# ina-foss/inaSpeechSegmenter

Measured on AMD Instinct MI355X. Metric: hours-of-audio segmented/sec (smn+gender, 16 kHz mono), higher is better.
Workload: dtype f32 (f16x3 split-operand MFMA, f32 accumulate; f64 FFT)

## Files before the change

inaspeechsegmenter_amd/_native.py:

```python
import ctypes as C
import os

import numpy as np

_HERE = os.path.dirname(os.path.abspath(__file__))
LIB_PATH = os.environ.get('ISS_LIB') or os.path.join(_HERE, 'libiss_hip.so')

PROG_COLS = 32
OP_CONV, OP_POOL, OP_SOFTMAX, OP_STATPOOL, OP_ACT, OP_ELT = 1, 2, 3, 4, 5, 6
(ELT_COPY, ELT_ADD, ELT_SUB, ELT_MUL, ELT_MAX, ELT_MIN, ELT_AVG, ELT_ZERO, ELT_PERMUTE) = range(9)
(C_OP, C_IN, C_OUT, C_RES, C_H, C_W, C_CIN, C_HO, C_WO, C_COUT, C_KH, C_KW, C_SH, C_SW, C_PT, C_PL,
 C_ACT, C_WOFF, C_BOFF, C_PSOFF, C_PTOFF, C_INMODE, C_POOLKIND, C_ORDER, C_FPOOLH, C_FPOOLW, C_DUALW, C_DUALB, C_ACTPARAM, C_ACTPARAM2, C_ACTPARAM3) = range(31)
PREC_BF16X3, PREC_F32, PREC_F16X3 = 0, 1, 2
K_ALIGN = 32
BUF_INPUT = -2
MAX_NETS = 8
RS_JOB = np.dtype([('src_offset', '<i8'), ('frames_in', '<i8'), ('channels', '<i4'), ('format', '<i4'), ('filter', '<i4'),
                   ('reserved', '<i4'), ('dst_offset', '<i8'), ('frames_out', '<i8')])
RS_FORMAT = {np.dtype(np.uint8): 0, np.dtype('<i2'): 1, np.dtype('<i4'): 2, np.dtype('<f4'): 3, np.dtype('<f8'): 4}
RS_I8, RS_ULAW, RS_ALAW, RS_SWAP = 8, 9, 10, 0x100
ADPCM_JOB = np.dtype([('src_offset', '<i8'), ('block_begin', '<i8'), ('nblocks', '<i8'), ('frames_total', '<i8'), ('channels', '<i4'),
                      ('block_align', '<i4'), ('output', '<i4'), ('filter', '<i4'), ('dst_offset', '<i8'), ('frames_out', '<i8')])
ADPCM_TO_SIGNAL, ADPCM_TO_STAGE = 0, 1
ADPCM_STATUS = {1: 'step index above 88', 2: 'predictor index above 6'}
# ... 66 lines not shown
    global _lib
    if _lib is not None:
        return _lib
    if not os.path.exists(LIB_PATH):
        raise NativeError(
            f"{LIB_PATH} is missing: the HIP extension has not been built. "
            "Run `python -c 'import __graft_entry__ as g; g.build()'` (needs hipcc). "
            "There is no CPU fallback for the feature/CNN path.")
    try:
        import torch
    except ImportError:
        pass
    L = C.CDLL(LIB_PATH)
    vp, i32, i64, u64 = C.c_void_p, C.c_int32, C.c_int64, C.c_uint64
    pf, pd, pi32, pi64, pu8, pi16 = (C.POINTER(C.c_float), C.POINTER(C.c_double), C.POINTER(C.c_int32),
                                     C.POINTER(C.c_int64), C.POINTER(C.c_uint8), C.POINTER(C.c_int16))
    sig = {
        'iss_create': (C.c_int, [C.c_int, C.POINTER(vp)]),
        'iss_destroy': (None, [vp]),
        'iss_last_error': (C.c_char_p, [vp]),
        'iss_version': (C.c_char_p, []),
        'iss_set_workspace_limit': (C.c_int, [vp, u64]),
        'iss_synchronize': (C.c_int, [vp]),
        'iss_sidekit_tables': (C.c_int, [vp, pd, pf]),
        'iss_signal_pcm16': (C.c_int, [vp, pi16, i64]),
        'iss_signal_f32': (C.c_int, [vp, pf, i64]),
        'iss_signal_pcm16_device': (C.c_int, [vp, vp, i64]),
        'iss_signal_pcm16_device_stream': (C.c_int, [vp, vp, i64, vp]),
        'iss_resample_filter': (C.c_int, [vp, i32, i32, pd, i64, pi32]),
        'iss_resample_pcm16': (C.c_int, [vp, vp, i64, vp, i32, i64]),
        'iss_resample_pcm16_windows': (C.c_int, [vp, vp, i64, vp, vp, i32, i64]),
        'iss_flac_decode_windows': (C.c_int, [vp, vp, i64, vp, i64, vp, vp, i32, i64, pi32]),
        'iss_adpcm_decode_windows': (C.c_int, [vp, vp, i64, vp, vp, i32, i64, i64, pi32]),
        'iss_msadpcm_decode_windows': (C.c_int, [vp, vp, i64, vp, vp, i32, i64, i64, pi32]),
        'iss_resample_pcm16_split': (C.c_int, [vp, vp, i64, vp, i32, i64, vp, vp, i64]),
        'iss_flac_decode_split': (C.c_int, [vp, vp, i64, vp, i64, vp, i32, i64, pi32, vp, vp, i64]),
        'iss_adpcm_decode_split': (C.c_int, [vp, vp, i64, vp, i32, i64, i64, pi32, vp, vp, i64]),
        'iss_msadpcm_decode_split': (C.c_int, [vp, vp, i64, vp, i32, i64, i64, pi32, vp, vp, i64]),
        'iss_resample_pcm16_windows_split': (C.c_int, [vp, vp, i64, vp, vp, i32, i64, vp, vp, i64]),
        'iss_flac_decode_windows_split': (C.c_int, [vp, vp, i64, vp, i64, vp, vp, i32, i64, pi32, vp, vp, i64]),
        'iss_adpcm_decode_windows_split': (C.c_int, [vp, vp, i64, vp, vp, i32, i64, i64, pi32, vp, vp, i64]),
        'iss_msadpcm_decode_windows_split': (C.c_int, [vp, vp, i64, vp, vp, i32, i64, i64, pi32, vp, vp, i64]),
        'iss_resample_split_geometry': (C.c_int, [vp, i32, i32, pi32, pi32]),
        'iss_resample_pcm16_mix': (C.c_int, [vp, vp, i64, vp, vp, i32, i64, vp, vp, i64, vp, i64]),
        'iss_flac_decode_mix': (C.c_int, [vp, vp, i64, vp, i64, vp, vp, i32, i64, pi32, vp, vp, i64, vp, i64]),
        'iss_adpcm_decode_mix': (C.c_int, [vp, vp, i64, vp, vp, i32, i64, i64, pi32, vp, vp, i64, vp, i64]),
        'iss_msadpcm_decode_mix': (C.c_int, [vp, vp, i64, vp, vp, i32, i64, i64, pi32, vp, vp, i64, vp, i64]),
        'iss_get_signal_pcm16': (C.c_int, [vp, pi16, i64, i64]),
        'iss_resample_stats': (C.c_int, [vp, pi64, pi64]),
        'iss_flac_index': (C.c_int, [vp, i64, i64, vp, vp, i64, pi64, pi64, C.c_char_p, i32]),
        'iss_flac_crc': (C.c_int, [vp, i64, pi32, pi32]),
        'iss_flac_decode_host': (C.c_int, [vp, i64, vp, i64, i32, i32, i64, vp, pi32]),
        'iss_flac_decode': (C.c_int, [vp, vp, i64, vp, i64, vp, i32, i64, pi32]),
        'iss_flac_get_stage': (C.c_int, [vp, i32, vp, i64]),
        'iss_flac_stats': (C.c_int, [vp, pi64, pi64]),
        'iss_adpcm_decode_host': (C.c_int, [vp, i64, i64, i32, i32, i64, pi16, pi32]),
        'iss_adpcm_decode': (C.c_int, [vp, vp, i64, vp, i32, i64, i64, pi32]),
        'iss_adpcm_get_stage': (C.c_int, [vp, i32, vp, i64]),
        'iss_adpcm_stats': (C.c_int, [vp, pi64, pi64]),
        'iss_msadpcm_decode_host': (C.c_int, [vp, i64, i64, i32, i32, i64, pi16, pi32]),
        'iss_msadpcm_decode': (C.c_int, [vp, vp, i64, vp, i32, i64, i64, pi32]),
        'iss_msadpcm_get_stage': (C.c_int, [vp, i32, vp, i64]),
        'iss_msadpcm_stats': (C.c_int, [vp, pi64, pi64]),
        'iss_host_alloc': (C.c_int, [vp, C.c_size_t, C.POINTER(vp)]),
        'iss_host_free': (C.c_int, [vp, vp]),
        'iss_cnn_probs_async': (C.c_int, [vp, C.c_int, pi32, i32, pf, pu8, pi64]),
        'iss_cnn_dead_stats': (C.c_int, [vp, pi64, pi64]),
        'iss_wait': (C.c_int, [vp, i64]),
        'iss_comm_unique_id': (C.c_int, [vp, pu8]),
        'iss_comm_init': (C.c_int, [vp, pu8, i32, i32]),
        'iss_comm_destroy': (C.c_int, [vp]),
        'iss_allgather_segments': (C.c_int, [vp, pi32, i32, i32, pi32, pi32]),
        'iss_comm_allreduce_max': (C.c_int, [vp, pd]),
        'iss_comm_info': (C.c_int, [vp, pi32, pi32, pi32, C.c_char_p, i32]),
        'iss_sidekit': (C.c_int, [vp, pi32]),
        'iss_get_loge': (C.c_int, [vp, pf]),
        'iss_get_mspec': (C.c_int, [vp, pf]),
        'iss_set_mspec': (C.c_int, [vp, pf, i32]),
        'iss_cnn_load': (C.c_int, [vp, C.c_int, pi32, i32, pf, i64, i32, pi64, i32, i32, i32, i32]),
        'iss_cnn_load_shared': (C.c_int, [vp, C.c_int, C.c_int, pi32, i32, i32, pi64, i32, i32, i32, i32]),
        'iss_cnn_probs': (C.c_int, [vp, C.c_int, pi32, i32, pf, pu8]),
        'iss_cnn_forward': (C.c_int, [vp, C.c_int, pf, i32, pf]),
        'iss_cnn_flops': (C.c_int, [vp, C.c_int, pd]),
        'iss_set_precision': (C.c_int, [vp, C.c_int]),
        'iss_set_precision_guard': (C.c_int, [vp, C.c_float]),
        'iss_cnn_precision_info': (C.c_int, [vp, C.c_int, pi32, pf, pi32, pi32, pf]),
        'iss_cnn_set_net_precision': (C.c_int, [vp, C.c_int, C.c_int]),
        'iss_vbx_tables': (C.c_int, [vp, pd, pd]),
        'iss_vbx_features': (C.c_int, [vp, pi32, pd, i64, pf, pi32]),
        'iss_vbx_set_dither': (C.c_int, [vp, pd, i64]),
        'iss_vbx_features_pcm16': (C.c_int, [vp, pi16, i64, pf, pi32]),
        'iss_vbx_features_batch_pcm16': (C.c_int, [vp, pi16, pi64, i32, pi32, pf]),
        'iss_vbx_features_resident': (C.c_int, [vp, pi64, pi64, i32, pi32, pf]),
        'iss_vbx_resident_stats': (C.c_int, [vp, pi64, pi64]),
        'iss_vbx_embed': (C.c_int, [vp, C.c_int, pi32, i32, pf]),
        'iss_prof_enable': (C.c_int, [vp, C.c_int]),
        'iss_prof_get': (C.c_int, [vp, C.c_int, pd, pi64, pd]),
        'iss_prof_reset': (C.c_int, [vp]),
        'iss_prof_get_row': (C.c_int, [vp, C.c_int, pd, pi64]),
        'iss_prof_get_instance': (C.c_int, [vp, C.c_int, C.c_char_p, i32, pd, pi64, pd]),
        'iss_set_diag': (C.c_int, [vp, C.c_uint32]),
        'iss_scribble': (C.c_int, [vp, C.c_uint32]),
        'iss_viterbi_f64': (C.c_int, [pd, i64, i32, pd, pi32]),
        'iss_viterbi_f32': (C.c_int, [pf, i64, i32, pd, pi32]),
        'iss_energy_viterbi': (C.c_int, [pf, i64, C.c_double, C.c_double, C.c_double, pd, pi32]),
        'iss_viterbi_segments_f32': (C.c_int, [pf, pi64, i64, i32, pd, pi32]),
    }
    for name, (res, args) in sig.items():
        fn = getattr(L, name)
        fn.restype = res
        fn.argtypes = args
    L._iss_symbols = tuple(sig)
    _lib = L
    return L


DIAG_BITS = {'no_shared_first': 0x001, 'no_flrows': 0x002, 'no_ws': 0x004, 'no_ws3': 0x008, 'no_direct1': 0x010,
             'no_nh2': 0x020, 'no_tr': 0x040, 'no_pw': 0x080, 'no_pws': 0x100, 'no_pws2': 0x200, 'no_wq': 0x400,
             'no_dual': 0x800, 'no_chain': 0x1000, 'no_ring': 0x2000, 'no_fsame': 0x4000, 'no_f32ws': 0x8000, 'no_ncb1': 0x10000, 'no_wsu3': 0x20000, 'no_gfused': 0x40000, 'no_hl': 0x80000,
             'no_skip_dead': 0x100000}


def diag_flags(names):
    flags = 0
    for nm in str(names).replace(' ', '').replace('+', ',').lower().split(','):
        if nm:
            flags |= DIAG_BITS[nm]
    return flags


def _ptr(a, ty):
    return a.ctypes.data_as(C.POINTER(ty))


def viterbi(emission, transition):
    L = lib()
    em = np.ascontiguousarray(emission)
    if em.dtype not in (np.float32, np.float64):
        em = em.astype(np.float64)
    tr = np.ascontiguousarray(transition, dtype=np.float64)
    T, K = em.shape
    out = np.empty(T, dtype=np.int32)
    if em.dtype == np.float32:
        rc = L.iss_viterbi_f32(_ptr(em, C.c_float), T, K, _ptr(tr, C.c_double), _ptr(out, C.c_int32))
    else:
        rc = L.iss_viterbi_f64(_ptr(em, C.c_double), T, K, _ptr(tr, C.c_double), _ptr(out, C.c_int32))
    if rc != 0:
        raise NativeError(f"iss_viterbi failed ({rc}): T={T} K={K}")
    return out


def viterbi_segments(emission, seg_len, transition):
    L = lib()
    em = np.ascontiguousarray(emission, dtype=np.float32)
    sl = np.ascontiguousarray(seg_len, dtype=np.int64)
    tr = np.ascontiguousarray(transition, dtype=np.float64)
    n, K = em.shape
    assert int(sl.sum()) == n
    out = np.empty(n, dtype=np.int32)
    rc = L.iss_viterbi_segments_f32(_ptr(em, C.c_float), _ptr(sl, C.c_int64), sl.size, K, _ptr(tr, C.c_double), _ptr(out, C.c_int32))
    if rc != 0:
        raise NativeError(f"iss_viterbi_segments_f32 failed ({rc}): n={n} K={K} segments={sl.size}")
    return out


_LOG_EPS = np.log(np.full(1, 1e-10))[0], np.log(np.full(1, 1 - 1e-10))[0]


def energy_viterbi(loge, threshold, transition):
    L = lib()
    x = np.ascontiguousarray(loge, dtype=np.float32)
    tr = np.ascontiguousarray(transition, dtype=np.float64)
    out = np.empty(x.size, dtype=np.int32)
    rc = L.iss_energy_viterbi(_ptr(x, C.c_float), x.size, float(threshold), float(_LOG_EPS[0]), float(_LOG_EPS[1]),
                              _ptr(tr, C.c_double), _ptr(out, C.c_int32))
    if rc != 0:
        raise NativeError(f"iss_energy_viterbi failed ({rc}): T={x.size}")
    return out


def flac_crc(buf):
    b = np.frombuffer(bytes(buf), dtype=np.uint8)
    c8, c16 = C.c_int32(), C.c_int32()
    if lib().iss_flac_crc(C.c_void_p(b.ctypes.data), b.size, C.byref(c8), C.byref(c16)) != 0:
        raise NativeError('iss_flac_crc failed')
    return c8.value, c16.value


def flac_index(buf, first_frame, info):
    L = lib()
    inf = np.ascontiguousarray(np.array(info, dtype=FLAC_INFO).reshape(1))
    cap = max(16, int(inf['total_samples'][0]) // max(1, int(inf['min_block'][0]) or 1) + 2) if inf['total_samples'][0] > 0 \
        else buf.size // 64 + 16
    err = C.create_string_buffer(256)
    n, off = C.c_int64(), C.c_int64()
    for _ in range(2):
        rows = np.zeros(cap, dtype=FLAC_FRAME)
        rc = L.iss_flac_index(C.c_void_p(buf.ctypes.data), buf.size, int(first_frame), C.c_void_p(inf.ctypes.data),
                              C.c_void_p(rows.ctypes.data), cap, C.byref(n), C.byref(off), err, 256)
        if rc != -5:
            break
        cap = buf.size // 9 + 16
    if rc != 0:
        raise ValueError(off.value, err.value.decode())
    return rows[:n.value].copy()


def flac_decode_host(buf, frames, channels, bps, frames_total):
    fr = np.ascontiguousarray(frames, dtype=FLAC_FRAME)
    out = np.empty((int(frames_total), int(channels)), dtype=np.int32 if bps > 16 else np.int16)
    st = np.zeros(len(fr), dtype=np.int32)
    rc = lib().iss_flac_decode_host(C.c_void_p(buf.ctypes.data), buf.size, C.c_void_p(fr.ctypes.data), len(fr), int(channels),
                                    int(bps), int(frames_total), C.c_void_p(out.ctypes.data), _ptr(st, C.c_int32))
    if rc != 0:
        raise NativeError(f'iss_flac_decode_host failed ({rc}): bad frame rows')
    return (out[:, 0] if channels == 1 else out), st


def adpcm_decode_host(buf, nblocks, channels, block_align, frames_total, fn='iss_adpcm_decode_host'):
    buf = np.ascontiguousarray(buf, dtype=np.uint8)
    out = np.empty((int(frames_total), int(channels)), dtype=np.int16)
    st = np.zeros(int(nblocks), dtype=np.int32)
    rc = getattr(lib(), fn)(C.c_void_p(buf.ctypes.data), buf.size, int(nblocks), int(channels), int(block_align),
                            int(frames_total), _ptr(out, C.c_int16), _ptr(st, C.c_int32))
    if rc != 0:
        raise NativeError(f'{fn} failed ({rc}): bad block geometry')
    return (out[:, 0] if channels == 1 else out), st


def msadpcm_decode_host(buf, nblocks, channels, block_align, frames_total):
    return adpcm_decode_host(buf, nblocks, channels, block_align, frames_total, 'iss_msadpcm_decode_host')


class Context:

    def __init__(self, device=0):
        self._L = lib()
        h = C.c_void_p()
        rc = self._L.iss_create(int(device), C.byref(h))
        if rc != 0:
            raise NativeError(f"iss_create(device={device}) failed ({rc}): "
                              f"{self._L.iss_last_error(None).decode()}")
        self._h = h
        self.device = device
        self.T = 0
        self._net_out = {}
        self._dither_n = 0
        self._pinned = {}
        self.comm_rank, self.comm_world = 0, 1
        self.precision = None
        self.workspace_limit = None
        self.diag = 0
        env = os.environ.get('ISS_DIAG', '')
        if env:
            self.set_diag(diag_flags(env))
        self.guard_threshold = None
        env = os.environ.get('ISS_PREC_GUARD', '')
        if env:
            self.set_precision_guard(float(env))

    def close(self):
        if getattr(self, '_h', None):
            for p in list(self._pinned.values()):
                self._L.iss_host_free(self._h, C.c_void_p(p))
            self._pinned.clear()
            self._L.iss_destroy(self._h)
            self._h = None

    def __del__(self):
        try:
            self.close()
        except Exception:
            pass

    def _ck(self, rc, what):
        if rc != 0:
            raise NativeError(f"{what} failed ({rc}): {self._L.iss_last_error(self._h).decode()}")

    def sidekit_tables(self, window, melbank):
        w = np.ascontiguousarray(window, dtype=np.float64)
        b = np.ascontiguousarray(melbank, dtype=np.float32)
        assert w.shape == (400,) and b.shape == (24, 257)
        self._ck(self._L.iss_sidekit_tables(self._h, _ptr(w, C.c_double), _ptr(b, C.c_float)), 'iss_sidekit_tables')

    def set_signal(self, sig):
        sig = np.ascontiguousarray(sig)
        if sig.dtype == np.int16:
            self._ck(self._L.iss_signal_pcm16(self._h, _ptr(sig, C.c_int16), sig.size), 'iss_signal_pcm16')
        elif sig.dtype == np.float32:
            self._ck(self._L.iss_signal_f32(self._h, _ptr(sig, C.c_float), sig.size), 'iss_signal_f32')
        else:
            raise TypeError(f"signal dtype {sig.dtype}: need int16 or float32")
        self._keep = sig

    def set_signal_device(self, dev_ptr, n, producer_stream=None):
        self._ck(self._L.iss_signal_pcm16_device_stream(self._h, C.c_void_p(int(dev_ptr)), int(n),
                                                        C.c_void_p(int(producer_stream)) if producer_stream else None),
                 'iss_signal_pcm16_device')

    def resample_filter(self, sr):
        from . import resample
        up, down, h = resample.plan(sr)
        fid = C.c_int32()
        self._ck(self._L.iss_resample_filter(self._h, up, down, _ptr(h, C.c_double), h.size, C.byref(fid)), 'iss_resample_filter')
        return fid.value, up, down

    def resample_job(self, x, sr, src_offset, dst_offset, fmt=None):
        fid, up, down = self.resample_filter(sr)
        n = x.shape[0]
        return (src_offset, n, 1 if x.ndim == 1 else x.shape[1], RS_FORMAT[x.dtype] if fmt is None else int(fmt), fid, 0,
                dst_offset, -(-n * up // down))

    def resample(self, src, jobs, n_signal=-1, windows=None, splits=None, mixes=None):
        src = np.ascontiguousarray(src, dtype=np.uint8)
        jb = np.ascontiguousarray(np.array(jobs, dtype=RS_JOB))
        self._decode_call('iss_resample_pcm16', (C.c_void_p(src.ctypes.data), src.size, C.c_void_p(jb.ctypes.data)),
                          (jb.size, int(n_signal)), windows, splits, mixes)
        self._keep_rs = src

    def _decode_call(self, base, lead, trail, windows, splits, mixes=None):
        name, args = base, lead + trail
        if mixes is not None:
            if splits is not None:
                raise ValueError('a call carries splits or mixes, not both')
            wn = None if windows is None else _window_rows(windows, trail[0])
            sets, rows, terms = _mix_rows(mixes, trail[0])
            args = lead + (None if wn is None else C.c_void_p(wn.ctypes.data),) + trail + (
                C.c_void_p(sets.ctypes.data), C.c_void_p(rows.ctypes.data), rows.size, C.c_void_p(terms.ctypes.data), terms.size)
            self._ck(getattr(self._L, base + '_mix')(self._h, *args), base + '_mix')
            return
        if windows is not None:
            wn = _window_rows(windows, trail[0])
            name, args = base + '_windows', lead + (C.c_void_p(wn.ctypes.data),) + trail
        if splits is not None:
            sp, sel = _split_rows(splits, trail[0])
            name, args = name + '_split', args + (C.c_void_p(sp.ctypes.data), C.c_void_p(sel.ctypes.data), sel.size)
        self._ck(getattr(self._L, name)(self._h, *args), name)

# ... 166 lines not shown
        self._ck(self._L.iss_wait(self._h, int(ticket)), 'iss_wait')

    def comm_unique_id(self):
        buf = np.zeros(128, dtype=np.uint8)
        self._ck(self._L.iss_comm_unique_id(self._h, _ptr(buf, C.c_uint8)), 'iss_comm_unique_id')
        return buf.tobytes()

    def comm_init(self, uid, rank, world):
        buf = np.frombuffer(bytes(uid), dtype=np.uint8).copy()
        assert buf.size == 128
        self._ck(self._L.iss_comm_init(self._h, _ptr(buf, C.c_uint8), int(rank), int(world)), 'iss_comm_init')
        self.comm_rank, self.comm_world = int(rank), int(world)

    def comm_destroy(self):
        self._ck(self._L.iss_comm_destroy(self._h), 'iss_comm_destroy')
        self.comm_rank, self.comm_world = 0, 1

    def allgather_segments(self, rows, capacity):
        world = self.comm_world
        out = np.zeros((world, capacity, 4), dtype=np.int32)
        counts = np.zeros(world, dtype=np.int32)
        if rows is None:
            rows, n = np.zeros((1, 4), np.int32), -1
        else:
            rows = np.ascontiguousarray(rows, dtype=np.int32).reshape(-1, 4)
            n = rows.shape[0]
        self._ck(self._L.iss_allgather_segments(self._h, _ptr(rows, C.c_int32), n, int(capacity),
                                                _ptr(out, C.c_int32), _ptr(counts, C.c_int32)), 'iss_allgather_segments')
        return out, counts

    def comm_info(self):
        w, r, v = C.c_int32(), C.c_int32(), C.c_int32()
        buf = C.create_string_buffer(512)
        self._ck(self._L.iss_comm_info(self._h, C.byref(w), C.byref(r), C.byref(v), buf, 512), 'iss_comm_info')
        return {'world': w.value, 'rank': r.value, 'version': v.value, 'lib': buf.value.decode(errors='replace')}

    def comm_allreduce_max(self, value):
        v = C.c_double(float(value))
        self._ck(self._L.iss_comm_allreduce_max(self._h, C.byref(v)), 'iss_comm_allreduce_max')
        return v.value

    def cnn_forward(self, net_id, x):
        x = np.ascontiguousarray(x, dtype=np.float32)
        n = x.shape[0]
        out = np.empty((n, self._net_out[net_id]), dtype=np.float32)
        self._ck(self._L.iss_cnn_forward(self._h, net_id, _ptr(x, C.c_float), n, _ptr(out, C.c_float)), 'iss_cnn_forward')
        return out

    def cnn_flops(self, net_id):
        f = C.c_double()
        self._ck(self._L.iss_cnn_flops(self._h, net_id, C.byref(f)), 'iss_cnn_flops')
        return f.value

    def set_precision(self, mode):
        self._ck(self._L.iss_set_precision(self._h, int(mode)), 'iss_set_precision')
        self.precision = int(mode)

    def set_precision_guard(self, threshold):
        self._ck(self._L.iss_set_precision_guard(self._h, float(threshold)), 'iss_set_precision_guard')
        self.guard_threshold = float(threshold)

    def cnn_precision_info(self, net_id):
        mode, slots, state, d, du = C.c_int32(0), C.c_int32(0), C.c_int32(0), C.c_float(0), C.c_float(0)
        self._ck(self._L.iss_cnn_precision_info(self._h, int(net_id), C.byref(mode), C.byref(d), C.byref(slots), C.byref(state), C.byref(du)),
                 'iss_cnn_precision_info')
        return {'mode': {PREC_F32: 'f32', PREC_F16X3: 'f16x3'}.get(mode.value, 'bf16x3'), 'max_dlogp': None if d.value < 0 else float(d.value),
                'max_dlogp_in_use': None if du.value < 0 else float(du.value),
                'slots': slots.value, 'state': ('pending', 'passed', 'escalated', 'fixed')[state.value]}

    def cnn_set_net_precision(self, net_id, mode):
        self._ck(self._L.iss_cnn_set_net_precision(self._h, int(net_id), int(mode)), 'iss_cnn_set_net_precision')

    def set_workspace_limit(self, nbytes):
        self._ck(self._L.iss_set_workspace_limit(self._h, int(nbytes)), 'iss_set_workspace_limit')
        self.workspace_limit = int(nbytes)

    def mirror_settings(self, other):
        if getattr(other, 'precision', None) is not None and other.precision != getattr(self, 'precision', None):
            self.set_precision(other.precision)
        if getattr(other, 'workspace_limit', None) is not None and other.workspace_limit != getattr(self, 'workspace_limit', None):
            self.set_workspace_limit(other.workspace_limit)
        if getattr(other, 'diag', 0) != getattr(self, 'diag', 0):
            self.set_diag(other.diag)
        if getattr(other, 'guard_threshold', None) is not None and other.guard_threshold != getattr(self, 'guard_threshold', None):
            self.set_precision_guard(other.guard_threshold)

    def set_diag(self, flags):
        flags = diag_flags(flags) if isinstance(flags, str) else int(flags)
        self._ck(self._L.iss_set_diag(self._h, flags), 'iss_set_diag')
        self.diag = flags

    def scribble(self, word):
        self._ck(self._L.iss_scribble(self._h, int(word) & 0xFFFFFFFF), 'iss_scribble')

    def synchronize(self):
        self._ck(self._L.iss_synchronize(self._h), 'iss_synchronize')

    def vbx_tables(self, window, melbank):
        w = np.ascontiguousarray(window, dtype=np.float64)
        b = np.ascontiguousarray(melbank, dtype=np.float64)
        assert w.shape == (400,) and b.shape == (257, 64)
        self._ck(self._L.iss_vbx_tables(self._h, _ptr(w, C.c_double), _ptr(b, C.c_double)), 'iss_vbx_tables')

    def vbx_features(self, sig_i32, dither_u):
        s = np.ascontiguousarray(sig_i32, dtype=np.int32)
        u = np.ascontiguousarray(dither_u, dtype=np.float64)
        assert s.shape == u.shape and s.ndim == 1
        T = (s.size + 320 - 400) // 160 + 1
        out = np.empty((T, 64), dtype=np.float32)
        t = C.c_int32()
        self._ck(self._L.iss_vbx_features(self._h, _ptr(s, C.c_int32), _ptr(u, C.c_double), s.size,
                                          _ptr(out, C.c_float), C.byref(t)), 'iss_vbx_features')
        self._dither_n = 0
        assert t.value == T
        return out

    def vbx_set_dither(self, dither_u):
        u = np.ascontiguousarray(dither_u, dtype=np.float64)
        self._ck(self._L.iss_vbx_set_dither(self._h, _ptr(u, C.c_double), u.size), 'iss_vbx_set_dither')
        self._dither_n = u.size

    def vbx_features_pcm16(self, pcm, to_host=True):
        s = np.ascontiguousarray(pcm, dtype=np.int16)
        T = (s.size + 320 - 400) // 160 + 1
        t = C.c_int32()
        if not to_host:
            self._ck(self._L.iss_vbx_features_pcm16(self._h, _ptr(s, C.c_int16), s.size, None, C.byref(t)), 'iss_vbx_features_pcm16')
            assert t.value == T
            return T
        out = np.empty((T, 64), dtype=np.float32)
        self._ck(self._L.iss_vbx_features_pcm16(self._h, _ptr(s, C.c_int16), s.size, _ptr(out, C.c_float), C.byref(t)),
                 'iss_vbx_features_pcm16')
        assert t.value == T
        return out

    def vbx_features_batch_pcm16(self, pcms, to_host=True):
        pcms = [np.asarray(p, dtype=np.int16) for p in pcms]
        soff = np.zeros(len(pcms) + 1, dtype=np.int64)
        soff[1:] = np.cumsum([p.size for p in pcms])
        s = np.ascontiguousarray(np.concatenate(pcms) if pcms else np.zeros(0, np.int16))
        foff = np.zeros(len(pcms) + 1, dtype=np.int32)
        T = int(sum((p.size + 320 - 400) // 160 + 1 for p in pcms))
        out = np.empty((T, 64), dtype=np.float32) if to_host else None
        self._ck(self._L.iss_vbx_features_batch_pcm16(self._h, _ptr(s, C.c_int16), _ptr(soff, C.c_int64), len(pcms),
                                                      _ptr(foff, C.c_int32), _ptr(out, C.c_float) if to_host else None),
                 'iss_vbx_features_batch_pcm16')
        return foff, out

    def vbx_features_resident(self, begins, counts, to_host=False):
        b = np.ascontiguousarray(begins, dtype=np.int64).reshape(-1)
        n = np.ascontiguousarray(counts, dtype=np.int64).reshape(-1)
        if b.size != n.size:
            raise ValueError(f'vbx_features_resident: {b.size} begins, {n.size} counts')
        foff = np.zeros(b.size + 1, dtype=np.int32)
        T = int(sum((int(k) + 320 - 400) // 160 + 1 for k in n if k >= 200))
        out = np.empty((T, 64), dtype=np.float32) if to_host else None
        self._ck(self._L.iss_vbx_features_resident(self._h, _ptr(b, C.c_int64), _ptr(n, C.c_int64), b.size, _ptr(foff, C.c_int32),
                                                   _ptr(out, C.c_float) if to_host else None), 'iss_vbx_features_resident')
        return foff, (out[:foff[-1]] if to_host else None)

    def vbx_resident_stats(self):
        return self._counters('iss_vbx_resident_stats')

    def vbx_embed(self, net_id, starts):
        st = np.ascontiguousarray(starts, dtype=np.int32)
        out = np.empty((st.size, self._net_out[net_id]), dtype=np.float32)
        self._ck(self._L.iss_vbx_embed(self._h, net_id, _ptr(st, C.c_int32), st.size, _ptr(out, C.c_float)), 'iss_vbx_embed')
        return out

    def prof_enable(self, on=True):
        self._ck(self._L.iss_prof_enable(self._h, 1 if on else 0), 'iss_prof_enable')

    def prof_reset(self):
# ... 24 lines not shown
```

inaspeechsegmenter_amd/csrc/cnn.hip:

```cpp
#include "conv_select.h"

using namespace issk;

namespace {

template <int MODE>
__global__ __launch_bounds__(256) void conv_igemm_kernel(const ConvArgs p) {
    __shared__ __attribute__((aligned(16))) float sA[2][BM * LDK];
    __shared__ __attribute__((aligned(16))) float sB[2][BN * LDK];

    const int tid = threadIdx.x, lane = tid & 63, wv = tid >> 6;
    unsigned mt, nt;
    gemm_tile_of_block(blockIdx.x, p.nblk, p.nblk_n, mt, nt);
    const long long m0 = (long long)mt * BM;
    const int n0 = (int)nt * BN;

    const int k4 = tid & 3;
    const int lr = tid >> 2;
    RowSrc rs[2];
#pragma unroll
    for (int j = 0; j < 2; ++j) rs[j] = row_source<MODE>(p, m0 + lr + 64 * j);
    const int bn = n0 + lr;
    const bool bok = bn < p.Cout;
    const float* wrow = p.w + (size_t)(bok ? bn : 0) * p.Kpad + k4 * 4;
// ... 743 lines not shown

__global__ void pool_kernel(const float* __restrict__ in, float* __restrict__ out, long long total, int H, int W,
                            int C, int Ho, int Wo, int kh, int kw, int sh, int sw, int pt, int pl, int kind) {
    const long long idx = (long long)blockIdx.x * blockDim.x + threadIdx.x;
    if (idx >= total) return;
    const int c = (int)(idx % C);
    long long t = idx / C;
    const int ox = (int)(t % Wo); t /= Wo;
    const int oy = (int)(t % Ho);
    const long long b = t / Ho;
    float acc = kind == 0 ? -INFINITY : 0.f;
    int cnt = 0;
    for (int ky = 0; ky < kh; ++ky) {
        const int iy = oy * sh - pt + ky;
        if ((unsigned)iy >= (unsigned)H) continue;
        for (int kx = 0; kx < kw; ++kx) {
            const int ix = ox * sw - pl + kx;
            if ((unsigned)ix >= (unsigned)W) continue;
            const float v = in[((b * H + iy) * W + ix) * C + c];
            acc = kind == 0 ? fmaxf(acc, v) : acc + v;
            ++cnt;
        }
    }
    out[idx] = kind == 0 ? acc : acc / (float)(cnt > 0 ? cnt : 1);
}


__global__ __launch_bounds__(256) void act_kernel(const float* in, float* out, long long total, int act, float alpha, float p2, float p3) {
    auto f = [&](float v) {
        if (act == 9) return v > p3 ? fminf(v, p2) : alpha * (v - p3);
        if (act == 8) return fminf(fmaxf(v, 0.f), alpha);
        if (act == 4) return v > 0.f ? v : alpha * (expf(v) - 1.f);
        if (act == 5) return v > 0.f ? v : alpha * v;
        if (act == 6) return 1.05070098f * (v > 0.f ? v : 1.67326324f * (expf(v) - 1.f));
        return v > 20.f ? v : log1pf(expf(v));
    };
    const long long n4 = total >> 2;
    for (long long i = blockIdx.x * 256ll + threadIdx.x; i < n4; i += (long long)gridDim.x * 256) {
        float4 v = reinterpret_cast<const float4*>(in)[i];
        v.x = f(v.x); v.y = f(v.y); v.z = f(v.z); v.w = f(v.w);
        reinterpret_cast<float4*>(out)[i] = v;
    }
    for (long long i = (n4 << 2) + blockIdx.x * 256ll + threadIdx.x; i < total; i += (long long)gridDim.x * 256) out[i] = f(in[i]);
}

__global__ __launch_bounds__(256) void elt_kernel(const float* in, const float* res, float* out, long long total, int kind,
                                                  int cin, int cout, int nch, int soff, int doff, int d0, int d1, int d2,
                                                  int s0, int s1, int s2, int relu) {
    auto bin = [&](float a, float b) {
        const float v = kind == ISS_ELT_ADD ? a + b : kind == ISS_ELT_SUB ? a - b : kind == ISS_ELT_MUL ? a * b :
                        kind == ISS_ELT_MAX ? fmaxf(a, b) : kind == ISS_ELT_MIN ? fminf(a, b) : (a + b) * 0.5f;
        return relu ? fmaxf(v, 0.f) : v;
    };
    if (kind >= ISS_ELT_ADD && kind <= ISS_ELT_AVG && (total & 3) == 0) {
        const long long n4 = total >> 2;
        for (long long i = blockIdx.x * 256ll + threadIdx.x; i < n4; i += (long long)gridDim.x * 256) {
            const float4 a = reinterpret_cast<const float4*>(in)[i], b = reinterpret_cast<const float4*>(res)[i];
            reinterpret_cast<float4*>(out)[i] = make_float4(bin(a.x, b.x), bin(a.y, b.y), bin(a.z, b.z), bin(a.w, b.w));
        }
        return;
    }
    for (long long i = blockIdx.x * 256ll + threadIdx.x; i < total; i += (long long)gridDim.x * 256) {
        if (kind >= ISS_ELT_ADD && kind <= ISS_ELT_AVG) {
            out[i] = bin(in[i], res[i]);
        } else if (kind == ISS_ELT_COPY || kind == ISS_ELT_ZERO) {
            const long long p = i / nch;
            const int ch = (int)(i - p * nch);
            out[p * cout + doff + ch] = kind == ISS_ELT_ZERO ? 0.f : in[p * cin + soff + ch];
        } else {
            const long long per = (long long)d0 * d1 * d2;
            const long long smp = i / per;
            long long r = i - smp * per;
            const int i2 = (int)(r % d2); r /= d2;
            const int i1 = (int)(r % d1);
            const int i0 = (int)(r / d1);
            out[i] = in[smp * per + (long long)i0 * s0 + (long long)i1 * s1 + (long long)i2 * s2];
        }
    }
}

__global__ void softmax_kernel(const float* __restrict__ in, float* __restrict__ out, long long rows, int C) {
    const long long r = (long long)blockIdx.x * blockDim.x + threadIdx.x;
    if (r >= rows) return;
    const float* x = in + r * C;
    float mx = x[0];
    for (int i = 1; i < C; ++i) mx = fmaxf(mx, x[i]);
    float s = 0.f;
    for (int i = 0; i < C; ++i) s += expf(x[i] - mx);
    for (int i = 0; i < C; ++i) out[r * C + i] = expf(x[i] - mx) / s;
}

__global__ void statpool_kernel(const float* __restrict__ in, float* __restrict__ out, long long total, int H, int W, int C) {
    const long long idx = (long long)blockIdx.x * blockDim.x + threadIdx.x;
    if (idx >= total) return;
    const int c = (int)(idx % C);
    long long t = idx / C;
    const int h = (int)(t % H);
    const long long b = t / H;
    const float* src = in + ((b * H + h) * (long long)W) * C + c;
    float s = 0.f, q = 0.f;
    for (int w = 0; w < W; ++w) { const float v = src[(long long)w * C]; s += v; q += v * v; }
    const float mean = s / W, meansq = q / W;
    float* o = out + b * (2LL * C * H);
    o[c * H + h] = mean;
    o[(long long)C * H + c * H + h] = sqrtf(meansq - mean * mean + 1e-10f);
}

__global__ void fill_half_kernel(float* p, long long n) {
    const long long i = (long long)blockIdx.x * blockDim.x + threadIdx.x;
    if (i < n) p[i] = 0.5f;
}

__global__ void mask_probs_kernel(float* probs, const uint8_t* finite, long long n, int C) {
    const long long i = (long long)blockIdx.x * blockDim.x + threadIdx.x;
    if (i < n * C && !finite[i / C]) probs[i] = 0.5f;
}

__global__ __launch_bounds__(256) void row_flags_kernel(const float* __restrict__ mspec, int T, uint8_t* __restrict__ flag) {
    const int t = blockIdx.x * 256 + threadIdx.x;
    if (t >= T) return;
    float v[24];
#pragma unroll
    for (int k = 0; k < 6; ++k) *reinterpret_cast<float4*>(v + 4 * k) = reinterpret_cast<const float4*>(mspec + (size_t)t * 24)[k];
    flag[t] = (uint8_t)iss_row_flag(v);
}

__global__ void scatter_probs_kernel(const float* __restrict__ res, const uint8_t* __restrict__ lfinite, const int32_t* __restrict__ map,
                                     long long n, int C, float* __restrict__ out, uint8_t* __restrict__ finite) {
    const long long i = (long long)blockIdx.x * blockDim.x + threadIdx.x;
    if (i >= n * C) return;
    const long long r = i / C;
    const int k = (int)(i - r * C);
    const long long m = map[r];
    const uint8_t f = lfinite[r];
    out[m * C + k] = f ? res[i] : 0.5f;
    if (k == 0) finite[m] = f;
}

inline int roundup(int a, int b) { return (a + b - 1) / b * b; }

inline uint16_t bf16_rne(float x) {
    uint32_t u;
    memcpy(&u, &x, 4);
    u += 0x7fffu + ((u >> 16) & 1u);
    return (uint16_t)(u >> 16);
}
inline float bf16_to_f32(uint16_t h) {
    uint32_t u = (uint32_t)h << 16;
    float x;
    memcpy(&x, &u, 4);
    return x;
}

}

IssParamArrays::~IssParamArrays() {
    for (void* p : {(void*)blob, (void*)wh, (void*)wl, (void*)wh16, (void*)wl16}) if (p) (void)hipFree(p);
}

int iss_cnn_free(iss_ctx* c, int id) {
    if (!c || id < 0 || id >= ISS_MAX_NETS) return ISS_EINVAL;
    IssNet& n = c->nets[id];
    if (n.shared_params) {
        n.shared_params.reset();
    } else {
        if (n.d_blob) (void)hipFree(n.d_blob);
        if (n.d_wh) (void)hipFree(n.d_wh);
        if (n.d_wl) (void)hipFree(n.d_wl);
        if (n.d_wh16) (void)hipFree(n.d_wh16);
        if (n.d_wl16) (void)hipFree(n.d_wl16);
    }
    for (auto& kv : n.dhl_wp) if (kv.second) (void)hipFree(kv.second);
// ... 212 lines not shown
    ISS_HIP(c, hipSetDevice(c->device));
    iss_cnn_free(c, id);
    IssNet& s = c->nets[src];
    IssNet& n = c->nets[id];
    std::vector<int32_t> ktab;
    int rc = cnn_set_program(c, n, "iss_cnn_load_shared", prog, nrows, s.blob_floats, nbuf, buf_elems, in_h, in_w, in_c, out_dim, ktab);
    if (rc) return rc;
    if (!s.shared_params) {
        s.shared_params = std::make_shared<IssParamArrays>();
        IssParamArrays& a = *s.shared_params;
        a.blob = s.d_blob; a.wh = s.d_wh; a.wl = s.d_wl; a.wh16 = s.d_wh16; a.wl16 = s.d_wl16;
    }
    n.shared_params = s.shared_params;
    n.d_blob = s.d_blob; n.d_wh = s.d_wh; n.d_wl = s.d_wl; n.d_wh16 = s.d_wh16; n.d_wl16 = s.d_wl16;
    n.f16_ok = s.f16_ok;
    if ((rc = cnn_upload_tables(c, n, nullptr, ktab))) return rc;
    n.loaded = true;
    return ISS_OK;
}

extern "C" int iss_set_precision(iss_ctx* c, int mode) {
    if (!c) return ISS_EINVAL;
    if (mode != ISS_PREC_BF16X3 && mode != ISS_PREC_F32 && mode != ISS_PREC_F16X3) return iss_fail(c, ISS_EINVAL, "iss_set_precision: unknown mode %d", mode);
    if (mode == c->precision) return ISS_OK;
    c->precision = mode;
    for (IssNet& n : c->nets) {
        if (!n.loaded || n.prec_by_caller) continue;
        n.prec_override = -1;
        n.guard_state = ISS_GUARD_PENDING;
        n.guard_dlogp = n.guard_dlogp_chosen = -1.f;
        n.guard_slots = 0;
    }
    return ISS_OK;
}

extern "C" int iss_set_precision_guard(iss_ctx* c, float threshold) {
    if (!c) return ISS_EINVAL;
    if (!(threshold == threshold)) return iss_fail(c, ISS_EINVAL, "iss_set_precision_guard: threshold is NaN");
    c->guard_threshold = threshold;
    return ISS_OK;
}

extern "C" int iss_cnn_set_net_precision(iss_ctx* c, int id, int mode) {
    if (!c || id < 0 || id >= ISS_MAX_NETS) return ISS_EINVAL;
    if (mode != -1 && mode != ISS_PREC_BF16X3 && mode != ISS_PREC_F32 && mode != ISS_PREC_F16X3) return iss_fail(c, ISS_EINVAL, "iss_cnn_set_net_precision: unknown mode %d", mode);
    if (!c->nets[id].loaded) return iss_fail(c, ISS_ESTATE, "net %d not loaded", id);
    c->nets[id].prec_override = mode;
    c->nets[id].prec_by_caller = mode != -1;
    c->nets[id].guard_state = mode == -1 ? ISS_GUARD_PENDING : ISS_GUARD_FIXED;
    return ISS_OK;
}

static bool net_reads_patches(const IssNet& n) {
    for (int r = 0; r < n.nrows; ++r)
        if (n.prog[(size_t)r * ISS_PROG_COLS + ISS_C_OP] == ISS_OP_CONV && n.prog[(size_t)r * ISS_PROG_COLS + ISS_C_INMODE] == 1) return true;
    return false;
}

static int effective_precision(const iss_ctx* c, const IssNet& n) {
    const int prec = n.prec_override >= 0 ? n.prec_override : c->precision;
    if (prec == ISS_PREC_F16X3 && !(n.f16_ok && n.d_wh16 != nullptr && net_reads_patches(n))) return ISS_PREC_BF16X3;
    return prec;
}

extern "C" int iss_cnn_precision_info(iss_ctx* c, int id, int32_t* mode, float* max_dlogp, int32_t* slots, int32_t* state, float* dlogp_in_use) {
    if (!c || id < 0 || id >= ISS_MAX_NETS) return ISS_EINVAL;
    const IssNet& n = c->nets[id];
    if (!n.loaded) return iss_fail(c, ISS_ESTATE, "net %d not loaded", id);
    if (mode) *mode = effective_precision(c, n);
    if (max_dlogp) *max_dlogp = n.guard_dlogp;
    if (slots) *slots = n.guard_slots;
    if (state) *state = n.guard_state;
    if (dlogp_in_use) *dlogp_in_use = n.guard_dlogp_chosen;
    return ISS_OK;
}

extern "C" int iss_set_diag(iss_ctx* c, uint32_t flags) {
    if (!c) return ISS_EINVAL;
    if (flags & ~(uint32_t)ISS_DIAG_ALL) return iss_fail(c, ISS_EINVAL, "iss_set_diag: unknown bits 0x%x", flags & ~(uint32_t)ISS_DIAG_ALL);
    c->diag = flags;
    return ISS_OK;
}

extern "C" int iss_cnn_flops(iss_ctx* c, int id, double* f) {
    if (!c || id < 0 || id >= ISS_MAX_NETS || !f) return ISS_EINVAL;
    if (!c->nets[id].loaded) return iss_fail(c, ISS_ESTATE, "net %d not loaded", id);
    *f = c->nets[id].flops_per_sample;
    return ISS_OK;
}

namespace {

struct PassIo { const int32_t* d_winrow; const float* d_stats; const uint8_t* d_fin; const float* d_input; };

int conv_args(iss_ctx* c, IssNet& n, const PassIo& io, int bc, const ConvChoice& ch, ConvArgs& a) {
    const int r = ch.row;
    const int32_t* R = &n.prog[(size_t)r * ISS_PROG_COLS];
    memset(&a, 0, sizeof(a));
    fill_geometry(a, R, bc);
    a.in = R[ISS_C_IN] == ISS_BUF_INPUT ? io.d_input : (const float*)c->act[R[ISS_C_IN]].p;
    a.w = n.d_blob + R[ISS_C_WOFF];
    a.bias = R[ISS_C_BOFF] >= 0 ? n.d_blob + R[ISS_C_BOFF] : nullptr;
    a.ps = R[ISS_C_PSOFF] >= 0 ? n.d_blob + R[ISS_C_PSOFF] : nullptr;
    a.pt = R[ISS_C_PTOFF] >= 0 ? n.d_blob + R[ISS_C_PTOFF] : nullptr;
    a.res = R[ISS_C_RES] >= 0 ? (const float*)c->act[R[ISS_C_RES]].p : nullptr;
    a.out = (float*)c->act[R[ISS_C_OUT]].p;
    a.ktab = n.d_ktab + n.ktab_off[r];
    a.wh = n.d_wh + R[ISS_C_WOFF]; a.wl = n.d_wl + R[ISS_C_WOFF];
    a.Kpad = n.kpad[r]; a.mode = ch.inst.mode; a.tmr = ch.tmr;
    if (ch.inst.kernel == ConvKernel::Dhl) return ISS_OK;
    if (R[ISS_C_INMODE] == 1) {
        if (!io.d_winrow) return iss_fail(c, ISS_ESTATE, "patch-mode network run without a window list");
        a.in = (const float*)c->mspec.p; a.win_row = io.d_winrow; a.stats = io.d_stats; a.finite = io.d_fin;
    } else if (R[ISS_C_INMODE] == 2) {
        if (!io.d_winrow || !c->vbx_out.p) return iss_fail(c, ISS_ESTATE, "window-mode network run without resident vbx features");
        a.in = (const float*)c->vbx_out.p; a.win_row = io.d_winrow;
    } else if (!a.in) return iss_fail(c, ISS_ESTATE, "network input missing");
    a.nblk = (unsigned)((a.M + BM - 1) / BM);
    set_fast_div(a, 0, a.pp); set_fast_div(a, 1, a.pw); set_fast_div(a, 2, a.Hq * a.Wq); set_fast_div(a, 3, a.Wq);
#ifdef ISS_EXPERIMENTS
    { static const int dbg = getenv("ISS_DBG") ? atoi(getenv("ISS_DBG")) : 0; a.dbg = dbg; }
#endif
    a.nblk_n = (unsigned)((a.Cout + BN - 1) / BN);
    if (ch.inst.kernel == ConvKernel::Pwc) {
        const int32_t* Q = &n.prog[(size_t)ch.partner * ISS_PROG_COLS];
        a.wh2 = n.d_wh + Q[ISS_C_WOFF]; a.wl2 = n.d_wl + Q[ISS_C_WOFF];
        a.bias2 = Q[ISS_C_BOFF] >= 0 ? n.d_blob + Q[ISS_C_BOFF] : nullptr;
        a.out2 = (float*)c->act[Q[ISS_C_OUT]].p;
        a.act2 = Q[ISS_C_ACT]; a.Cout2 = Q[ISS_C_COUT];
    } else if (ch.inst.kernel == ConvKernel::Pws2Dual) {
        const int32_t* P = &n.prog[(size_t)ch.partner * ISS_PROG_COLS];
        a.in2 = P[ISS_C_IN] == ISS_BUF_INPUT ? io.d_input : (const float*)c->act[P[ISS_C_IN]].p;
        a.Cin2 = P[ISS_C_CIN]; a.H2 = P[ISS_C_H]; a.W2 = P[ISS_C_W]; a.sh2 = P[ISS_C_SH]; a.sw2 = P[ISS_C_SW];
        const int64_t wo = (int64_t)R[ISS_C_DUALW] - 1;
        a.w = n.d_blob + wo; a.wh = n.d_wh + wo; a.wl = n.d_wl + wo;
        a.bias = n.d_blob + (R[ISS_C_DUALB] - 1); a.res = nullptr;
        a.Kpad = a.Cin + a.Cin2;
    }
    if (ch.inst.f16) { a.f16 = 1; a.wh = n.d_wh16 + R[ISS_C_WOFF]; a.wl = n.d_wl16 + R[ISS_C_WOFF]; }
    if (ch.inst.kernel == ConvKernel::Wq3h) { a.in_hl = 1; a.in_np = ch.in_np; }
    if (ch.out != OutLayout::F32) { a.out_hl = 1; a.out_np = ch.out_np; a.out_f16 = ch.generic_out && ch.out_f16 ? 1 : 0; }
    return ISS_OK;
}

int launch_shared_first_layer(iss_ctx* c, IssNet& n, const PassIo& io, int pend, int bc, int rmin, int rmax, ConvArgs& a, double* fl) {
    const int32_t* R1 = &n.prog[(size_t)pend * ISS_PROG_COLS];
    const bool fs1 = R1[ISS_C_HO] == R1[ISS_C_H];
    int ph1, pw1;
    fused_pool_of(R1, ph1, pw1);
    const bool pool1 = ph1 * pw1 != 1;
    const long long rrows = (long long)(rmax - rmin) + R1[ISS_C_HO];
    const long long rtot = rrows * R1[ISS_C_WO] * (R1[ISS_C_COUT] / 4);
    const int f_ne = fs1 ? R1[ISS_C_KH] - 1 : 0;
    const long long etot = (long long)bc * f_ne * R1[ISS_C_WO] * (R1[ISS_C_COUT] / 4);
    const int plane_rows = pool1 ? (int)(rrows / ph1) + 2 : 0;
    const long long ptot = pool1 ? (long long)ph1 * plane_rows * (R1[ISS_C_WO] / pw1) * (R1[ISS_C_COUT] / 4) : 0;
    { const int rc = iss_reserve(c, c->raw1, (size_t)(rtot + etot + ptot) * 16 + (pool1 ? (size_t)bc * 4 + 16 : 0)); if (rc) return rc; }
    float* Rraw = (float*)c->raw1.p;
    const float* mspec = (const float*)c->mspec.p;
    const float* w1 = n.d_blob + R1[ISS_C_WOFF];
    const size_t lds1 = (size_t)R1[ISS_C_KH] * R1[ISS_C_KW] * R1[ISS_C_COUT] * 4;
    iss_prof_begin(c, 2, 0);
    if (fs1) {
        const int pt1 = R1[ISS_C_PT], pl1 = R1[ISS_C_PL], pb1 = R1[ISS_C_KH] - 1 - pt1;
        const float* S = n.d_wsum + n.wsumx_off[pend];
        if (rtot >= (1ll << 31) || etot >= (1ll << 31)) return iss_fail(c, ISS_EINVAL, "internal: shared first layer over %lld + %lld items", rtot, etot);
        hipLaunchKernelGGL(first_layer_same_kernel, dim3((unsigned)std::min<long long>((rtot + 255) / 256, 4096)), dim3(256), lds1, c->stream,
                           mspec, (int)c->T, rmin, rtot, R1[ISS_C_WO], R1[ISS_C_COUT], R1[ISS_C_KH], R1[ISS_C_KW], pt1, pl1, w1, n.kpad[pend], Rraw);
        if (etot > 0)
            hipLaunchKernelGGL(first_layer_edge_kernel, dim3((unsigned)std::min<long long>((etot + 255) / 256, 8192)), dim3(256), lds1, c->stream,
                               mspec, io.d_winrow, io.d_stats, etot, R1[ISS_C_H], R1[ISS_C_WO], R1[ISS_C_COUT], R1[ISS_C_KH],
                               R1[ISS_C_KW], pt1, pb1, pl1, w1, n.kpad[pend], S, Rraw + (size_t)rtot * 4);
        a.f_padt = pt1; a.f_padb = pb1; a.f_erow0 = (int)rrows;
    } else {
        const dim3 rgrid((unsigned)std::min<long long>((rtot + 255) / 256, 4096));
        const bool no_rows = (c->diag & ISS_DIAG_NO_FLROWS) != 0;
// ... 1 lines not shown
                             rrows * (R1[ISS_C_COUT] / 4) < (1ll << 31);
        const dim3 rowgrid((unsigned)std::min<long long>((rrows * (R1[ISS_C_COUT] / 4) + 255) / 256, 4096));
        if (rows_ok && R1[ISS_C_WO] == 17)
            hipLaunchKernelGGL((first_layer_rows_kernel<4, 5, 17>), rowgrid, dim3(256), lds1, c->stream, mspec, rmin, (int)rrows, R1[ISS_C_COUT], w1, n.kpad[pend], Rraw);
        else if (rows_ok)
            hipLaunchKernelGGL((first_layer_rows_kernel<4, 5, 20>), rowgrid, dim3(256), lds1, c->stream, mspec, rmin, (int)rrows, R1[ISS_C_COUT], w1, n.kpad[pend], Rraw);
        else if (R1[ISS_C_KH] == 4 && R1[ISS_C_KW] == 5)
            hipLaunchKernelGGL((first_layer_raw_kernel<4, 5>), rgrid, dim3(256), lds1, c->stream, mspec, rmin, rtot, R1[ISS_C_WO], R1[ISS_C_COUT], 4, 5, w1, n.kpad[pend], Rraw);
        else
            hipLaunchKernelGGL((first_layer_raw_kernel<0, 0>), rgrid, dim3(256), lds1, c->stream, mspec, rmin, rtot, R1[ISS_C_WO], R1[ISS_C_COUT],
                               R1[ISS_C_KH], R1[ISS_C_KW], w1, n.kpad[pend], Rraw);
    }
    a.in = Rraw; a.win_row = io.d_winrow; a.f_rmin = rmin;
    if (pool1) {
        if (ptot >= (1ll << 40)) return iss_fail(c, ISS_EINVAL, "internal: pooled first layer over %lld items", ptot);
        float* P = Rraw + (size_t)(rtot + etot) * 4;
        int32_t* wr2 = reinterpret_cast<int32_t*>(P + (size_t)ptot * 4);
        hipLaunchKernelGGL(pool_rows_kernel, dim3((unsigned)std::min<long long>((ptot + 255) / 256, 8192)), dim3(256), 0, c->stream,
                           (const float*)Rraw, P, ptot, (int)rrows, R1[ISS_C_WO], R1[ISS_C_COUT], ph1, pw1, plane_rows);
        hipLaunchKernelGGL(winrow_pool_kernel, dim3((unsigned)((bc + 255) / 256)), dim3(256), 0, c->stream, io.d_winrow, wr2, bc, rmin, ph1, plane_rows);
        a.in = P; a.win_row = wr2; a.f_rmin = 0;
    }
    iss_prof_end(c);
    a.stats = io.d_stats; a.finite = io.d_fin;
    a.f_bias = n.d_blob + R1[ISS_C_BOFF];
    a.f_wsum = fs1 ? n.d_wsum + n.wsumx_off[pend] : n.d_wsum + n.wsum_off[pend];
    a.f_ps = R1[ISS_C_PSOFF] >= 0 ? n.d_blob + R1[ISS_C_PSOFF] : nullptr;
    a.f_pt = R1[ISS_C_PTOFF] >= 0 ? n.d_blob + R1[ISS_C_PTOFF] : nullptr;
    a.f_act = R1[ISS_C_ACT];
    *fl += 2.0 * R1[ISS_C_KH] * R1[ISS_C_KW] * (double)R1[ISS_C_COUT] * (double)bc * R1[ISS_C_HO] * R1[ISS_C_WO];
    return ISS_OK;
}

bool launch_direct1(const ConvArgs& a, dim3 grid, size_t lds, hipStream_t st, const ConvInst& i) {
#define ISS_DIRECT1_TRY(WINDOW_) ISS_LAUNCH_IF(i.kernel == ConvKernel::Direct1 && i.window == WINDOW_, conv1_direct3x3_kernel<WINDOW_>, grid, 256, lds)
    ISS_DIRECT1_TRY(true)
    ISS_DIRECT1_TRY(false)
#undef ISS_DIRECT1_TRY
    return false;
}
bool launch_patch1(const ConvArgs& a, dim3 grid, hipStream_t st, const ConvInst& i) {
#define ISS_PATCH1_TRY(TR_, F16_) \
    ISS_LAUNCH_IF(i.kernel == ConvKernel::Patch1 && i.tr == TR_ && i.f16 == F16_, (conv1_patch_x3_kernel<TR_, F16_>), grid, 256, 0)
    ISS_PATCH1_TRY(true, true)
    ISS_PATCH1_TRY(true, false)
    ISS_PATCH1_TRY(false, true)
    ISS_PATCH1_TRY(false, false)
#undef ISS_PATCH1_TRY
    return false;
}
constexpr int X3_NTN = 2;
bool launch_x3(const ConvArgs& a, dim3 grid, hipStream_t st, const ConvInst& i) {
#define ISS_X3_TRY(MODE_, TR_)                                                                                                      \
    ISS_LAUNCH_IF((i.kernel == ConvKernel::X3 || i.kernel == ConvKernel::Gather) && i.mode == MODE_ && i.tr == TR_, \
                  (conv_x3_kernel<MODE_, TR_, X3_NTN>), grid, 256, 0)
    ISS_X3_TRY(4, true)
    ISS_X3_TRY(4, false)
    ISS_X3_TRY(3, true)
    ISS_X3_TRY(3, false)
    ISS_X3_TRY(0, true)
    ISS_X3_TRY(0, false)
    ISS_X3_TRY(1, true)
    ISS_X3_TRY(1, false)
    ISS_X3_TRY(2, false)
#undef ISS_X3_TRY
    return false;
}
bool launch_pw(const ConvArgs& a, dim3 grid, hipStream_t st, const ConvInst& i) {
#define ISS_PW_TRY(F16_) ISS_LAUNCH_IF(i.kernel == ConvKernel::Pw && i.f16 == F16_, conv_x3_pw_kernel<F16_>, grid, 256, 0)
    ISS_PW_TRY(true)
    ISS_PW_TRY(false)
#undef ISS_PW_TRY
    return false;
}
bool launch_igemm(const ConvArgs& a, dim3 grid, hipStream_t st, const ConvInst& i) {
#define ISS_IGEMM_TRY(MODE_) ISS_LAUNCH_IF(i.kernel == ConvKernel::Igemm && i.mode == MODE_, conv_igemm_kernel<MODE_>, grid, 256, 0)
    ISS_IGEMM_TRY(0)
    ISS_IGEMM_TRY(1)
    ISS_IGEMM_TRY(2)
#undef ISS_IGEMM_TRY
    return false;
}

int launch_conv(iss_ctx* c, IssNet& n, const ConvChoice& ch, ConvArgs& a, double fl) {
    const int r = ch.row;
    const int32_t* R = &n.prog[(size_t)r * ISS_PROG_COLS];
    const ConvInst& i = ch.inst;
    hipStream_t st = c->stream;
    const dim3 grid(a.nblk, a.nblk_n);
    const unsigned ny = (unsigned)std::max(1, a.Cout / (2 * BN));
    const unsigned tiles = (unsigned)((a.M + WS_TM - 1) / WS_TM);
    const unsigned groups = (unsigned)((a.M + (long long)WS_TM * WS_G - 1) / ((long long)WS_TM * WS_G));
    const unsigned qtiles = ch.tmr > 0 ? (unsigned)((a.M + ch.tmr - 1) / ch.tmr) : 0;
    const dim3 nh2grid(std::min<unsigned>(tiles, std::max(1u, 256u / ny)), ny);
    const dim3 wgrid(std::min<unsigned>(groups, 256u), grid.y);
    bool ok = false;
    iss_prof_begin(c, 0, fl);
    iss_prof_tag(c, ch.tag), iss_prof_row(c, r), iss_prof_inst(c, "%s", inst_name(i).c_str());
    switch (i.kernel) {
    case ConvKernel::Dhl: {
        const int K = R[ISS_C_CIN];
        uint16_t*& wp = n.dhl_wp[{r, i.f16 ? 1 : 0}];
        if (!wp) {
            ISS_HIP(c, hipMalloc((void**)&wp, dhl_packed_elems(K, R[ISS_C_COUT]) * 2));
            iss_dhl_pack((i.f16 ? n.d_wh16 : n.d_wh) + R[ISS_C_WOFF], (i.f16 ? n.d_wl16 : n.d_wl) + R[ISS_C_WOFF], wp, R[ISS_C_COUT], n.kpad[r], K, st);
        }
        DhlArgs d;
        d.a = reinterpret_cast<const uint16_t*>(a.in); d.wp = wp; d.bias = a.bias; d.out = a.out;
        d.np = ch.in_np; d.M = (int)a.M; d.K = K; d.Cout = R[ISS_C_COUT]; d.act = R[ISS_C_ACT];
        ok = iss_dhl_launch(d, st, i);
        break;
    }
    case ConvKernel::Pwc: ok = iss_pwc_launch(a, st, i); break;
    case ConvKernel::Pws2Dual: case ConvKernel::Pws2Strided: case ConvKernel::Pws2: ok = iss_pws2_launch(a, st, i); break;
    case ConvKernel::Direct1: {
        const long long items = (long long)(a.M / ((long long)a.H * a.W)) * ((a.H + 7) / 8) * a.W * (a.Cout / 4);
        if (items >= (1ll << 32)) return iss_fail(c, ISS_EINVAL, "internal: direct first layer over %lld work items", items);
        ok = launch_direct1(a, dim3((unsigned)std::min<long long>((items + 255) / 256, 8192)), (size_t)9 * a.Cout * sizeof(float), st, i);
        break;
    }
    case ConvKernel::WsNh2F32: ok = iss_ws_launch_f32_nh2_3x3(a, nh2grid, st, i); break;
    case ConvKernel::WsNh2: ok = iss_ws_launch_nh2_3x3(a, nh2grid, st, i); break;
    case ConvKernel::Wq3: ok = iss_wq3_launch(a, dim3(std::min<unsigned>((qtiles + 1) / 2, std::max(1u, 256u / ny)), ny), st, i); break;
    case ConvKernel::Wq3h: ok = iss_wq3h_launch(a, dim3(std::min<unsigned>((qtiles + 1) / 2, std::max(1u, 256u / ny)), ny), st, i); break;
    case ConvKernel::WsPlainU: case ConvKernel::WsPlain: {
        const dim3 pgrid(std::min<unsigned>(groups, std::max(1u, 256u / grid.y)), grid.y);
        ok = iss_ws_launch_plain_3x3(a, pgrid, st, i);
        break;
    }
    case ConvKernel::WsF32Fused: ok = iss_ws_launch_f32_fused_5x3(a, wgrid, st, i); break;
    case ConvKernel::WsRing: ok = iss_ws_launch_ring(a, dim3(std::min<unsigned>(qtiles, 256u), grid.y), st, i); break;
    case ConvKernel::WsFs: ok = iss_ws_launch_fs(a, dim3(std::min<unsigned>(tiles, 256u), grid.y), st, i); break;
    case ConvKernel::WsNcb1: ok = iss_ws_launch_ncb1_5x3(a, wgrid, st, i); break;
    case ConvKernel::Wq: ok = iss_wq_launch_5x3(a, dim3(std::min<unsigned>((qtiles + 1) / 2, 256u), grid.y), st, i); break;
    case ConvKernel::Ws:
#define ISS_WS_CASE(KH_, KW_) if (i.kh == KH_ && i.kw == KW_) ok = iss_ws_launch_##KH_##x##KW_(a, wgrid, st, i);
        ISS_WS_SHAPES(ISS_WS_CASE)
#undef ISS_WS_CASE
        break;
    case ConvKernel::Fp: {
        const dim3 pgrid(std::min<unsigned>(a.nblk, 512u), grid.y / i.nh);
#define ISS_FP_CASE(KH_, KW_) if (i.kh == KH_ && i.kw == KW_) ok = iss_fp_launch_##KH_##x##KW_(a, pgrid, st, i);
        ISS_FP_SHAPES(ISS_FP_CASE)
#undef ISS_FP_CASE
        break;
    }
    case ConvKernel::Patch1: ok = launch_patch1(a, dim3(std::min<unsigned>(a.nblk, 512u), grid.y), st, i); break;
    case ConvKernel::Gather: case ConvKernel::X3:
        a.nblk_n = (unsigned)((a.Cout + 32 * X3_NTN - 1) / (32 * X3_NTN));
        ok = launch_x3(a, dim3(a.nblk * a.nblk_n), st, i);
        break;
    case ConvKernel::Pws: ok = iss_pws_launch(a, dim3(std::min<unsigned>(a.nblk * a.nblk_n, 512u)), st, i); break;
    case ConvKernel::Pw: ok = launch_pw(a, dim3(std::min<unsigned>(a.nblk * a.nblk_n, 768u)), st, i); break;
    case ConvKernel::Igemm: ok = launch_igemm(a, dim3(a.nblk * a.nblk_n), st, i); break;
    case ConvKernel::Declined: return iss_fail(c, ISS_EINVAL, "internal: row %d has no kernel", r);
    }
    if (!ok) return iss_fail(c, ISS_EINVAL, "internal: %s is not compiled", inst_name(i).c_str());
    iss_prof_end(c);
    return ISS_OK;
}

int run_conv(iss_ctx* c, IssNet& n, const ConvEnv& env, const PassIo& io, const ConvChoice& ch, int pend) {
    const int32_t* R = &n.prog[(size_t)ch.row * ISS_PROG_COLS];
    ConvArgs a;
    int rc = conv_args(c, n, io, env.bc, ch, a);
    if (rc) return rc;
    double fl = conv_flops(R, (double)a.M);
    if (ch.inst.kernel == ConvKernel::Dhl) fl = 2.0 * R[ISS_C_CIN] * (double)R[ISS_C_COUT] * (double)env.bc;
    if (ch.inst.kernel == ConvKernel::Pwc) fl += 2.0 * a.Cout * (double)a.Cout2 * (double)a.M;
    if (ch.inst.kernel == ConvKernel::Pws2Dual) fl += 2.0 * a.Cin2 * (double)a.Cout * (double)a.M;
    if (ch.first == FirstLayer::Fused || ch.first == FirstLayer::Gather)
        if ((rc = launch_shared_first_layer(c, n, io, pend, env.bc, env.rmin, env.rmax, a, &fl))) return rc;
    return launch_conv(c, n, ch, a, fl);
}

int run_program(iss_ctx* c, IssNet& n, int bc, const int32_t* d_winrow, const float* d_stats,
                const uint8_t* d_fin, const float* d_input, float** result, int rmin = 0, int rmax = -1,
                bool share_first = false) {
    const PassIo io{d_winrow, d_stats, d_fin, d_input};
    std::vector<ChlState> layout(std::max<size_t>(c->act.size(), (size_t)n.nbuf));
    ConvEnv env = make_env(n, bc, rmin, rmax, share_first, effective_precision(c, n), c->diag, d_winrow != nullptr, d_input != nullptr,
                           c->vbx_out.p != nullptr, layout.data());
    int pending = -1;
    for (int r = 0; r < n.nrows; ++r) {
        const int32_t* R = &n.prog[(size_t)r * ISS_PROG_COLS];
        const float* in = R[ISS_C_IN] == ISS_BUF_INPUT ? d_input : (const float*)c->act[R[ISS_C_IN]].p;
        float* out = (float*)c->act[R[ISS_C_OUT]].p;
        const int op = R[ISS_C_OP];
        ChlState out_layout;
        if (op == ISS_OP_CONV) {
            if (pending < 0 && can_defer(env, r)) { pending = r; *result = out; continue; }
            const ConvChoice ch = select_conv(env, r, pending);
            int rc = ISS_OK;
            if (ch.first == FirstLayer::Alone) rc = run_conv(c, n, env, io, select_row(env, pending, -1, -1, -1), -1);
            if (!rc) rc = run_conv(c, n, env, io, ch, pending);
            if (pending >= 0) layout[n.prog[(size_t)pending * ISS_PROG_COLS + ISS_C_OUT]] = ChlState{};
            pending = -1;
            if (rc) return rc;
            if (ch.rows == 1 && env.layout_of(R[ISS_C_IN]).np && !ch.in_np)
                return iss_fail(c, ISS_EINVAL, "internal: row %d reads a CHL tensor on a kernel that expects f32", r);
            if (ch.rows == 2) {
                layout[R[ISS_C_OUT]] = ChlState{};
                R = &n.prog[(size_t)++r * ISS_PROG_COLS];
                out = (float*)c->act[R[ISS_C_OUT]].p;
            }
            if (ch.out != OutLayout::F32) out_layout = ChlState{ch.out_np, ch.out_f16, ch.out == OutLayout::ChlDense};
        } else if (op == ISS_OP_POOL) {
            const long long total = (long long)bc * R[ISS_C_HO] * R[ISS_C_WO] * R[ISS_C_CIN];
            iss_prof_begin(c, 2, 0);
            hipLaunchKernelGGL(pool_kernel, dim3((unsigned)((total + 255) / 256)), dim3(256), 0, c->stream, in, out,
                               total, R[ISS_C_H], R[ISS_C_W], R[ISS_C_CIN], R[ISS_C_HO], R[ISS_C_WO], R[ISS_C_KH],
                               R[ISS_C_KW], R[ISS_C_SH], R[ISS_C_SW], R[ISS_C_PT], R[ISS_C_PL], R[ISS_C_POOLKIND]);
            iss_prof_end(c);
        } else if (op == ISS_OP_SOFTMAX) {
            const long long rows = (long long)bc * R[ISS_C_H] * R[ISS_C_W];
            iss_prof_begin(c, 2, 0);
            hipLaunchKernelGGL(softmax_kernel, dim3((unsigned)((rows + 255) / 256)), dim3(256), 0, c->stream, in, out,
                               rows, R[ISS_C_CIN]);
            iss_prof_end(c);
        } else if (op == ISS_OP_ACT) {
            const long long total = (long long)bc * R[ISS_C_H] * R[ISS_C_W] * R[ISS_C_CIN];
            float alpha, p2, p3;
            { const int32_t bits = R[ISS_C_ACTPARAM]; memcpy(&alpha, &bits, sizeof(float)); }
            { const int32_t bits = R[ISS_C_ACTPARAM2]; memcpy(&p2, &bits, sizeof(float)); }
            { const int32_t bits = R[ISS_C_ACTPARAM3]; memcpy(&p3, &bits, sizeof(float)); }
            iss_prof_begin(c, 2, 0);
            hipLaunchKernelGGL(act_kernel, dim3((unsigned)std::min<long long>((total + 1023) / 1024, 1 << 20)), dim3(256), 0, c->stream, in, out, total,
                               R[ISS_C_ACT], alpha, p2, p3);
            iss_prof_end(c);
        } else if (op == ISS_OP_ELT) {
            const int k = R[ISS_C_ACT];
            const long long hw = (long long)R[ISS_C_H] * R[ISS_C_W];
            const bool chan = k == ISS_ELT_COPY || k == ISS_ELT_ZERO;
            const long long total = (long long)bc * hw * (chan ? R[ISS_C_KH] : R[ISS_C_CIN]);
            const float* res = R[ISS_C_RES] >= 0 ? (const float*)c->act[R[ISS_C_RES]].p : nullptr;
            if (res && layout[R[ISS_C_RES]].np) return iss_fail(c, ISS_EINVAL, "internal: row %d reads a CHL tensor", r);
            int st[3] = {0, 0, 0};
            if (k == ISS_ELT_PERMUTE) {
                const int sin[3] = {R[ISS_C_W] * R[ISS_C_CIN], R[ISS_C_CIN], 1};
                st[0] = sin[R[ISS_C_KH]]; st[1] = sin[R[ISS_C_KW]]; st[2] = sin[R[ISS_C_SH]];
            }
            iss_prof_begin(c, 2, 0);
            hipLaunchKernelGGL(elt_kernel, dim3((unsigned)std::min<long long>((total + 255) / 256, 1 << 20)), dim3(256), 0, c->stream, in, res, out,
                               total, k, R[ISS_C_CIN], R[ISS_C_COUT], R[ISS_C_KH], R[ISS_C_PT], R[ISS_C_PL],
                               R[ISS_C_HO], R[ISS_C_WO], R[ISS_C_COUT], st[0], st[1], st[2], R[ISS_C_ORDER] == 1 ? 1 : 0);
            iss_prof_end(c);
        } else if (op == ISS_OP_STATPOOL) {
            const long long total = (long long)bc * R[ISS_C_H] * R[ISS_C_CIN];
            iss_prof_begin(c, 2, 0);
            hipLaunchKernelGGL(statpool_kernel, dim3((unsigned)((total + 255) / 256)), dim3(256), 0, c->stream, in, out,
                               total, R[ISS_C_H], R[ISS_C_W], R[ISS_C_CIN]);
            iss_prof_end(c);
        }
        ISS_HIP(c, hipGetLastError());
        *result = out;
        layout[R[ISS_C_OUT]] = out_layout;
        if (op != ISS_OP_CONV && R[ISS_C_IN] != ISS_BUF_INPUT && layout[R[ISS_C_IN]].np)
            return iss_fail(c, ISS_EINVAL, "internal: row %d reads a CHL tensor", r);
    }
    return ISS_OK;
}

int plan_chunk(iss_ctx* c, IssNet& n, int total, int* bc_out) {
    int64_t per = 0;
    for (auto e : n.buf_elems) per += e;
    int64_t bc = (int64_t)(c->ws_limit / (uint64_t)(per * sizeof(float)));
    if (bc < 1) bc = 1;
    if (bc > total) bc = total;
    int64_t emax = 1;
    for (auto e : n.buf_elems) emax = std::max<int64_t>(emax, e);
    bc = std::min<int64_t>(bc, ((1ll << 31) - 1) / emax);
    if (bc < 1) return iss_fail(c, ISS_EINVAL, "network activation of %lld floats per sample exceeds the 2^31 element limit", (long long)emax);
    if (bc > 8) bc -= bc % 8;
    if ((int)c->act.size() < n.nbuf) c->act.resize(n.nbuf);
    for (int i = 0; i < n.nbuf; ++i) {
        int rc = iss_reserve(c, c->act[i], (size_t)bc * n.buf_elems[i] * sizeof(float) + issk::ISS_ACT_SLACK);
        if (rc) return rc;
    }
    *bc_out = (int)bc;
    return ISS_OK;
}

}

static int cnn_probs_impl(iss_ctx* c, int id, const int32_t* win_row, int32_t nslots, float* probs_out,
                          uint8_t* finite_out, bool async, int64_t* ticket_out);

static int precision_guard(iss_ctx* c, int id, const int32_t* win_row, int32_t nslots) {
    IssNet& n = c->nets[id];
    const int eff = effective_precision(c, n);
    if (eff == ISS_PREC_F32) { n.guard_state = ISS_GUARD_FIXED; return ISS_OK; }
    if (!(c->guard_threshold > 0.f)) return ISS_OK;
    const int runs = nslots >= 256 ? 4 : 1, per = nslots >= 256 ? 64 : nslots;
    const size_t od = (size_t)n.out_dim;
    std::vector<float> pref((size_t)runs * per * od), pm((size_t)per * od);
    std::vector<uint8_t> fref((size_t)runs * per), fm(per);
    auto window_run = [&](int r) { return win_row + (runs == 1 ? 0 : (size_t)r * (nslots - per) / (runs - 1)); };
    int rc = ISS_OK, compared = 0;
    auto probe = [&](int mode, double& worst) {
        worst = 0.0; compared = 0;
        for (int r = 0; r < runs && rc == ISS_OK; ++r) {
            n.prec_override = mode;
            rc = cnn_probs_impl(c, id, window_run(r), per, pm.data(), fm.data(), false, nullptr);
            if (rc != ISS_OK) return;
            for (int i = 0; i < per; ++i) {
                if (!fm[i] || !fref[(size_t)r * per + i]) continue;
                ++compared;
                for (size_t k = 0; k < od; ++k) {
                    const float a = pm[(size_t)i * od + k], b = pref[((size_t)r * per + i) * od + k];
                    if (!(a == a)) { worst = 1e30; continue; }
                    if (!(a > 1e-30f) || !(b > 1e-30f)) continue;
                    worst = std::max(worst, std::fabs(std::log((double)a) - std::log((double)b)));
                }
            }
        }
    };
    c->in_guard = true;
    for (int r = 0; r < runs && rc == ISS_OK; ++r) {
        n.prec_override = ISS_PREC_F32;
        rc = cnn_probs_impl(c, id, window_run(r), per, pref.data() + (size_t)r * per * od, fref.data() + (size_t)r * per, false, nullptr);
    }
    double worst = 0.0;
    int chosen = eff;
    if (rc == ISS_OK) probe(eff, worst);
    const double first = worst;
    if (rc == ISS_OK && worst > (double)c->guard_threshold) {
        chosen = ISS_PREC_F32;
        const int other = eff == ISS_PREC_BF16X3 ? ISS_PREC_F16X3 : ISS_PREC_BF16X3;
        if (other == ISS_PREC_BF16X3 || n.f16_ok) {
            double w2 = 0.0;
            probe(other, w2);
            if (rc == ISS_OK && w2 <= (double)c->guard_threshold) { chosen = other; worst = w2; }
        }
    }
    c->in_guard = false;
    n.prec_override = -1;
    if (rc != ISS_OK) return rc;
    if (compared == 0) { n.guard_slots = 0; return ISS_OK; }
    n.guard_dlogp = (float)std::min(first, 1e30); n.guard_slots = compared;
    n.guard_dlogp_chosen = chosen == eff ? n.guard_dlogp : (chosen == ISS_PREC_F32 ? 0.f : (float)worst);
    if (chosen != eff) { n.prec_override = chosen; n.guard_state = ISS_GUARD_ESCALATED; }
    else n.guard_state = ISS_GUARD_PASSED;
// ... 9 lines not shown
    hipLaunchKernelGGL(row_flags_kernel, dim3((c->T + 255) / 256), dim3(256), 0, c->stream, (const float*)c->mspec.p, (int)c->T,
                       (uint8_t*)c->d_rowflag.p);
    iss_prof_end(c);
    ISS_HIP(c, hipGetLastError());
    ISS_HIP(c, hipMemcpyAsync(c->h_rowflag, c->d_rowflag.p, (size_t)c->T, hipMemcpyDeviceToHost, c->stream));
    ISS_HIP(c, hipStreamSynchronize(c->stream));
    c->bad_prefix.clear();
    c->flags_epoch = c->feat_epoch;
    return ISS_OK;
}

static const std::vector<int32_t>& bad_prefix(iss_ctx* c, int w) {
    std::vector<int32_t>& P = c->bad_prefix[w];
    if (P.size() != (size_t)c->T + 1) {
        P.resize((size_t)c->T + 1);
        P[0] = 0;
        for (int32_t t = 0; t < c->T; ++t) P[t + 1] = P[t] + (c->h_rowflag[t] < w ? 1 : 0);
    }
    return P;
}

extern "C" int iss_cnn_dead_stats(iss_ctx* c, int64_t* windows, int64_t* dead) {
    if (!c) return ISS_EINVAL;
    if (windows) *windows = c->win_total;
    if (dead) *dead = c->win_dead;
    return ISS_OK;
}

static int cnn_probs_impl(iss_ctx* c, int id, const int32_t* win_row, int32_t nslots, float* probs_out,
                          uint8_t* finite_out, bool async, int64_t* ticket_out) {
    if (!c) return ISS_EINVAL;
    if (ticket_out) *ticket_out = -1;
    if (id < 0 || id >= ISS_MAX_NETS || nslots < 0 || (nslots > 0 && (!win_row || !probs_out || !finite_out)))
        return iss_fail(c, ISS_EINVAL, "iss_cnn_probs: bad argument");
    IssNet& n = c->nets[id];
    if (!n.loaded) return iss_fail(c, ISS_ESTATE, "iss_cnn_probs: net %d not loaded", id);
    if (!c->have_feats) return iss_fail(c, ISS_ESTATE, "iss_cnn_probs: no mel spectrogram resident");
    if (n.in_h != 68 || n.in_c != 1 || n.in_w > 24) return iss_fail(c, ISS_EINVAL, "net %d is not a (68,h,1) patch network", id);
    if (nslots == 0) return ISS_OK;
    for (int i = 0; i < nslots; ++i)
        if (win_row[i] < 0 || win_row[i] + 68 > c->T)
            return iss_fail(c, ISS_EINVAL, "iss_cnn_probs: window %d (row %d) outside the %d resident frames", i, win_row[i], c->T);
    ISS_HIP(c, hipSetDevice(c->device));
    int rc;
    std::vector<int32_t> lm;
    int nlive = nslots;
    if (!(c->diag & ISS_DIAG_NO_SKIP_DEAD)) {
        if ((rc = ensure_row_flags(c))) return rc;
        const std::vector<int32_t>& P = bad_prefix(c, n.in_w);
        int dead = 0;
        for (int i = 0; i < nslots; ++i) dead += P[win_row[i] + 68] != P[win_row[i]];
        if (dead) {
            nlive = nslots - dead;
            lm.resize(2 * (size_t)nlive);
            for (int i = 0, j = 0; i < nslots; ++i)
                if (P[win_row[i] + 68] == P[win_row[i]]) { lm[j] = win_row[i]; lm[(size_t)nlive + j] = i; ++j; }
        }
        if (!c->in_guard) c->win_dead += dead;
    }
    if (!c->in_guard) c->win_total += nslots;
    const bool compact = nlive < nslots;
    const int32_t* rows = compact ? lm.data() : win_row;
    if (!c->in_guard && n.guard_state == ISS_GUARD_PENDING && nlive > 0 && (rc = precision_guard(c, id, rows, nlive))) return rc;
    const size_t nup = compact ? 2 * (size_t)nlive : (size_t)nslots;
    if ((rc = iss_reserve(c, c->d_winrow, (nup ? nup : 1) * 4))) return rc;
    if ((rc = iss_reserve(c, c->d_stats, (size_t)nslots * 8))) return rc;
    if ((rc = iss_reserve(c, c->d_finite, (size_t)nslots))) return rc;
    if (compact && (rc = iss_reserve(c, c->d_lfinite, (size_t)(nlive ? nlive : 1)))) return rc;
    if ((rc = iss_reserve(c, c->d_out, (size_t)nslots * n.out_dim * 4))) return rc;
    int bc = 0;
    if (nlive > 0 && (rc = plan_chunk(c, n, nlive, &bc))) return rc;
    if (nup == 0) {
    } else if (async || compact) {
        void* pinned; int slot;
        if ((rc = iss_stage_host(c, rows, nup * 4, &pinned, &slot))) return rc;
        ISS_HIP(c, hipMemcpyAsync(c->d_winrow.p, pinned, nup * 4, hipMemcpyHostToDevice, c->stream));
        iss_stage_mark(c, slot);
    } else {
        ISS_HIP(c, hipMemcpyAsync(c->d_winrow.p, win_row, (size_t)nslots * 4, hipMemcpyHostToDevice, c->stream));
    }
    const int32_t* d_map = (const int32_t*)c->d_winrow.p + nlive;
    uint8_t* d_fin = compact ? (uint8_t*)c->d_lfinite.p : (uint8_t*)c->d_finite.p;
    const long long tot = (long long)nslots * n.out_dim;
    if (compact) {
        iss_prof_begin(c, 2, 0);
        hipLaunchKernelGGL(fill_half_kernel, dim3((unsigned)((tot + 255) / 256)), dim3(256), 0, c->stream, (float*)c->d_out.p, tot);
        iss_prof_end(c);
        ISS_HIP(c, hipGetLastError());
        ISS_HIP(c, hipMemsetAsync(c->d_finite.p, 0, (size_t)nslots, c->stream));
    }
    if (nlive > 0) {
        iss_prof_begin(c, 2, 0);
        hipLaunchKernelGGL(patch_stats_kernel, dim3((nlive + 3) / 4), dim3(256), 0, c->stream, (const float*)c->mspec.p,
                           (const int32_t*)c->d_winrow.p, nlive, n.in_w, (float*)c->d_stats.p, d_fin);
        iss_prof_end(c);
        ISS_HIP(c, hipGetLastError());
    }
    bool share = !(c->diag & ISS_DIAG_NO_SHARED_FIRST);
    if (nlive > 0) {
        int gmin = rows[0], gmax = rows[0];
        for (int i = 1; i < nlive; ++i) { gmin = std::min(gmin, rows[i]); gmax = std::max(gmax, rows[i]); }
        if ((long long)(gmax - gmin + 68) * 4 > (long long)nlive * 68) share = false;
    }
    for (int s0 = 0; s0 < nlive; s0 += bc) {
        const int cur = std::min(bc, nlive - s0);
        float* res = nullptr;
        int rmin = rows[s0], rmax = rows[s0];
        for (int i = s0 + 1; i < s0 + cur; ++i) { rmin = std::min(rmin, rows[i]); rmax = std::max(rmax, rows[i]); }
        rc = run_program(c, n, cur, (const int32_t*)c->d_winrow.p + s0, (const float*)c->d_stats.p + 2 * (size_t)s0,
                         (const uint8_t*)d_fin + s0, nullptr, &res, rmin, rmax, share);
        if (rc) return rc;
        if (compact) {
            const long long ct = (long long)cur * n.out_dim;
            iss_prof_begin(c, 2, 0);
            hipLaunchKernelGGL(scatter_probs_kernel, dim3((unsigned)((ct + 255) / 256)), dim3(256), 0, c->stream, (const float*)res,
                               (const uint8_t*)d_fin + s0, d_map + s0, (long long)cur, n.out_dim, (float*)c->d_out.p, (uint8_t*)c->d_finite.p);
            iss_prof_end(c);
            ISS_HIP(c, hipGetLastError());
        } else {
            ISS_HIP(c, hipMemcpyAsync((float*)c->d_out.p + (size_t)s0 * n.out_dim, res, (size_t)cur * n.out_dim * 4,
                                      hipMemcpyDeviceToDevice, c->stream));
        }
    }
    if (!compact) {
        hipLaunchKernelGGL(mask_probs_kernel, dim3((unsigned)((tot + 255) / 256)), dim3(256), 0, c->stream,
                           (float*)c->d_out.p, (const uint8_t*)c->d_finite.p, (long long)nslots, n.out_dim);
        ISS_HIP(c, hipGetLastError());
    }
    ISS_HIP(c, hipMemcpyAsync(probs_out, c->d_out.p, (size_t)tot * 4, hipMemcpyDeviceToHost, c->stream));
    ISS_HIP(c, hipMemcpyAsync(finite_out, c->d_finite.p, (size_t)nslots, hipMemcpyDeviceToHost, c->stream));
    if (async) {
        hipEvent_t ev;
        if (!c->ev_pool.empty()) { ev = c->ev_pool.back(); c->ev_pool.pop_back(); }
        else ISS_HIP(c, hipEventCreate(&ev));
        ISS_HIP(c, hipEventRecord(ev, c->stream));
        c->ticket_ev.push_back(ev);
        if (ticket_out) *ticket_out = c->ticket_base + (int64_t)c->ticket_ev.size() - 1;
        return ISS_OK;
    }
    ISS_HIP(c, hipStreamSynchronize(c->stream));
    iss_prof_collect(c);
    return ISS_OK;
}

extern "C" int iss_cnn_probs(iss_ctx* c, int id, const int32_t* win_row, int32_t nslots, float* probs_out,
                             uint8_t* finite_out) {
    return cnn_probs_impl(c, id, win_row, nslots, probs_out, finite_out, false, nullptr);
}

extern "C" int iss_cnn_probs_async(iss_ctx* c, int id, const int32_t* win_row, int32_t nslots, float* probs_out,
                                   uint8_t* finite_out, int64_t* ticket_out) {
    return cnn_probs_impl(c, id, win_row, nslots, probs_out, finite_out, true, ticket_out);
}

extern "C" int iss_cnn_forward(iss_ctx* c, int id, const float* x, int32_t nsamp, float* out) {
    if (!c) return ISS_EINVAL;
    if (id < 0 || id >= ISS_MAX_NETS || nsamp < 0 || (nsamp > 0 && (!x || !out)))
        return iss_fail(c, ISS_EINVAL, "iss_cnn_forward: bad argument");
    IssNet& n = c->nets[id];
    if (!n.loaded) return iss_fail(c, ISS_ESTATE, "iss_cnn_forward: net %d not loaded", id);
    if (net_reads_patches(n)) return iss_fail(c, ISS_EINVAL, "iss_cnn_forward: net %d reads mspec patches; use iss_cnn_probs", id);
    if (nsamp == 0) return ISS_OK;
    ISS_HIP(c, hipSetDevice(c->device));
    const size_t in_elems = (size_t)n.in_h * n.in_w * n.in_c;
    int rc, bc = 0;
    if ((rc = plan_chunk(c, n, nsamp, &bc))) return rc;
    if ((rc = iss_reserve(c, c->d_in, (size_t)bc * in_elems * 4))) return rc;
    if ((rc = iss_reserve(c, c->d_out, (size_t)nsamp * n.out_dim * 4))) return rc;
    for (int s0 = 0; s0 < nsamp; s0 += bc) {
        const int cur = std::min(bc, nsamp - s0);
        ISS_HIP(c, hipMemcpyAsync(c->d_in.p, x + (size_t)s0 * in_elems, (size_t)cur * in_elems * 4, hipMemcpyHostToDevice, c->stream));
        float* res = nullptr;
        rc = run_program(c, n, cur, nullptr, nullptr, nullptr, (const float*)c->d_in.p, &res);
        if (rc) return rc;
        ISS_HIP(c, hipMemcpyAsync((float*)c->d_out.p + (size_t)s0 * n.out_dim, res, (size_t)cur * n.out_dim * 4,
                                  hipMemcpyDeviceToDevice, c->stream));
    }
    ISS_HIP(c, hipMemcpyAsync(out, c->d_out.p, (size_t)nsamp * n.out_dim * 4, hipMemcpyDeviceToHost, c->stream));
    ISS_HIP(c, hipStreamSynchronize(c->stream));
    iss_prof_collect(c);
    return ISS_OK;
}

extern "C" int iss_vbx_embed(iss_ctx* c, int id, const int32_t* starts, int32_t nwin, float* out) {
    if (!c) return ISS_EINVAL;
    if (id < 0 || id >= ISS_MAX_NETS || nwin < 0 || (nwin > 0 && (!starts || !out)))
        return iss_fail(c, ISS_EINVAL, "iss_vbx_embed: bad argument");
    IssNet& n = c->nets[id];
    if (!n.loaded) return iss_fail(c, ISS_ESTATE, "iss_vbx_embed: net %d not loaded", id);
    if (n.prog[ISS_C_OP] != ISS_OP_CONV || n.prog[ISS_C_INMODE] != 2)
        return iss_fail(c, ISS_EINVAL, "iss_vbx_embed: net %d does not start with a window-mode conv", id);
    if (c->vbx_T <= 0) return iss_fail(c, ISS_ESTATE, "iss_vbx_embed: no vbx features resident (iss_vbx_features*)");
    if (nwin == 0) return ISS_OK;
    for (int i = 0; i < nwin; ++i)
        if (starts[i] < 0 || starts[i] + n.in_w > c->vbx_T)
            return iss_fail(c, ISS_EINVAL, "iss_vbx_embed: window %d (frames %d..%d) outside the %d resident frames", i, starts[i],
                            starts[i] + n.in_w, c->vbx_T);
    ISS_HIP(c, hipSetDevice(c->device));
    int rc, bc = 0;
    if ((rc = iss_reserve(c, c->d_winrow, (size_t)nwin * 4))) return rc;
    if ((rc = iss_reserve(c, c->d_out, (size_t)nwin * n.out_dim * 4))) return rc;
    if ((rc = plan_chunk(c, n, nwin, &bc))) return rc;
    ISS_HIP(c, hipMemcpyAsync(c->d_winrow.p, starts, (size_t)nwin * 4, hipMemcpyHostToDevice, c->stream));
    for (int s0 = 0; s0 < nwin; s0 += bc) {
        const int cur = std::min(bc, nwin - s0);
        float* res = nullptr;
        rc = run_program(c, n, cur, (const int32_t*)c->d_winrow.p + s0, nullptr, nullptr, nullptr, &res);
        if (rc) return rc;
        ISS_HIP(c, hipMemcpyAsync((float*)c->d_out.p + (size_t)s0 * n.out_dim, res, (size_t)cur * n.out_dim * 4,
                                  hipMemcpyDeviceToDevice, c->stream));
    }
    ISS_HIP(c, hipMemcpyAsync(out, c->d_out.p, (size_t)nwin * n.out_dim * 4, hipMemcpyDeviceToHost, c->stream));
    ISS_HIP(c, hipStreamSynchronize(c->stream));
    iss_prof_collect(c);
    return ISS_OK;
}
```

inaspeechsegmenter_amd/csrc/cnn_dhl.hip:

```cpp
#include "conv_dhl.h"

namespace issk {
__global__ void dhl_pack_kernel(const uint16_t* __restrict__ wh, const uint16_t* __restrict__ wl, uint16_t* __restrict__ out,
                                int Cout, int Kpad, int K) {
    const long long per_tile = (long long)(K / 8) * 2 * DHL_BN * 8;
    const long long total = per_tile * dhl_col_tiles(Cout);
    for (long long i = blockIdx.x * 256ll + threadIdx.x; i < total; i += (long long)gridDim.x * 256) {
        const int ytile = (int)(i / per_tile);
        const long long j = i - (long long)ytile * per_tile;
        const int e = (int)(j & 7);
        long long t = j >> 3;
        const int n = ytile * DHL_BN + (int)(t % DHL_BN); t /= DHL_BN;
        const int part = (int)(t & 1);
        const int kg = (int)(t >> 1);
        const int k = kg * 8 + e;
        out[i] = n < Cout ? (part ? wl : wh)[(size_t)n * Kpad + k] : (uint16_t)0;
    }
}

void iss_dhl_pack(const uint16_t* wh, const uint16_t* wl, uint16_t* out, int Cout, int Kpad, int K, hipStream_t st) {
    const long long total = (long long)dhl_packed_elems(K, Cout);
    hipLaunchKernelGGL(dhl_pack_kernel, dim3((unsigned)std::min<long long>((total + 255) / 256, 4096)), dim3(256), 0, st, wh, wl, out, Cout, Kpad, K);
}
bool iss_dhl_launch(const DhlArgs& a, hipStream_t st, const ConvInst& i) {
    const dim3 grid((unsigned)((a.M + DHL_BM - 1) / DHL_BM), (unsigned)dhl_col_tiles(a.Cout));
#define ISS_DHL_TRY(F16_) ISS_LAUNCH_IF(i.kernel == ConvKernel::Dhl && i.f16 == F16_, (conv_dhl_kernel<F16_>), grid, ISS_DHL_NW * 64, 0)
    ISS_DHL_TRY(true)
    ISS_DHL_TRY(false)
#undef ISS_DHL_TRY
    return false;
}
}
```

inaspeechsegmenter_amd/csrc/conv_common.h:

```cpp
#pragma once
#include "iss_internal.h"
#include <cmath>
#include <cstring>
#include <algorithm>
#include <cstdlib>
#include <functional>
#include <type_traits>

namespace issk {


typedef float floatx16 __attribute__((ext_vector_type(16)));
typedef __bf16 bf16x8 __attribute__((ext_vector_type(8)));
typedef __bf16 bf16x4 __attribute__((ext_vector_type(4)));

constexpr int BM = 128;
constexpr int BN = 64;
constexpr int BK = 16;
constexpr int LDK = BK + 4;
constexpr int XBK = 32;
constexpr int XLD = XBK + 8;
constexpr int KALIGN = 32;

struct ConvArgs {
    const float* in;
    const float* w;
    const uint16_t* wh;
    const uint16_t* wl;
    const float* bias;
    const float* ps;
    const float* pt;
    const float* res;
    float* out;
    const int32_t* ktab;
    const int32_t* win_row;
    const float* stats;
    const uint8_t* finite;
    long long M;
    long long img_stride;
    int H, W, Cin, Cout;
    int Hq, Wq;
    int ph, pw, pp;
    int poolkind;
    int H_k, kw;
    int sh, sw, pt_, pl_;
    int row_stride, pix_stride;
    int act, Kpad, mode;
    const float* f_bias;
    const float* f_wsum;
    const float* f_ps;
    const float* f_pt;
    int f_act;
    int f_rmin;
    int f_padt, f_padb, f_erow0;
    unsigned dv_mul[4];
    int dv_sh[4];
    unsigned nblk;
    unsigned nblk_n;
    int dbg;
    int tmr;
    const float* in2;
    int Cin2, H2, W2, sh2, sw2;
    const uint16_t* wh2;
    const uint16_t* wl2;
    const float* bias2;
    float* out2;
    int act2, Cout2;
    int in_hl, out_hl;
    unsigned in_np, out_np;
    int f16;
    int out_f16;
};

enum class ConvKernel { Declined, Dhl, Pwc, Pws2Dual, Direct1, WsNh2F32, Wq3, Wq3h, WsNh2, WsPlainU, WsPlain, WsF32Fused, WsRing, WsFs, WsNcb1, Wq, Ws, Fp,
                        Patch1, Gather, Pws2Strided, Pws2, Pws, Pw, X3, Igemm };
struct ConvInst {
    ConvKernel kernel = ConvKernel::Declined;
    int kh = 0, kw = 0, mode = 0, epi = 0, nh = 1, kind = -1, c1 = 0, c3 = 0;
    bool padded = false, tr = false, fused = false, f16 = false, window = false, has_res = false, simple_pw = false;
    bool out_hl = false;
};
#define ISS_LAUNCH_IF(WHEN, KERNEL, GRID, THREADS, LDS) \
    if (WHEN) { hipLaunchKernelGGL(KERNEL, GRID, dim3(THREADS), LDS, st, a); return true; }
#define ISS_SHAPE_IS(KH_, KW_) if (kh == KH_ && kw == KW_) return true;

inline unsigned chl_npad(long long npix) { return (unsigned)((npix + 63) / 64 * 64 + 512); }
inline size_t chl_bytes(long long npix, int C) { return (size_t)chl_npad(npix) * 16u * 4u * (size_t)(C / 16); }
constexpr size_t ISS_ACT_SLACK = 8u << 20;
inline bool chl_fits(long long npix, int C) { return C % 16 == 0 && chl_bytes(npix, C) <= (size_t)npix * C * 4 + ISS_ACT_SLACK && chl_bytes(npix, C) < 0xFFF00000ull; }

inline void set_fast_div(ConvArgs& a, int slot, int d) {
    if (d <= 1) { a.dv_mul[slot] = 0; a.dv_sh[slot] = 0; return; }
    int l = 0;
    while ((1ll << l) < d) ++l;
    a.dv_mul[slot] = (unsigned)(((1ull << (31 + l)) / (unsigned long long)d) + 1ull);
    a.dv_sh[slot] = l - 1;
}
template <class P>
__device__ __forceinline__ int fast_div(const P& p, int slot, int n) {
    return p.dv_mul[slot] ? (int)(__umulhi((unsigned)n, p.dv_mul[slot]) >> p.dv_sh[slot]) : n;
}


__device__ __forceinline__ void map_row(const ConvArgs& p, long long m, int& b, int& oy, int& ox) {
    long long q = m;
    int dy = 0, dx = 0;
    if (p.pp > 1) {
        q = m / p.pp;
        const int j = (int)(m - q * p.pp);
        dy = j / p.pw; dx = j - dy * p.pw;
    }
    const int hw = p.Hq * p.Wq;
    b = (int)(q / hw);
    const int rem = (int)(q - (long long)b * hw);
    const int qy = rem / p.Wq, qx = rem - qy * p.Wq;
    oy = qy * p.ph + dy;
    ox = qx * p.pw + dx;
}

template <class P>
__device__ __forceinline__ void map_row32(const P& p, int m, int& b, int& oy, int& ox) {
    int q = m, dy = 0, dx = 0;
    if (p.pp > 1) {
        q = fast_div(p, 0, m);
        const int j = m - q * p.pp;
        dy = fast_div(p, 1, j); dx = j - dy * p.pw;
    }
    const int hw = p.Hq * p.Wq;
    b = fast_div(p, 2, q);
    const int rem = q - b * hw;
    const int qy = fast_div(p, 3, rem), qx = rem - qy * p.Wq;
    oy = qy * p.ph + dy;
    ox = qx * p.pw + dx;
}

__device__ __forceinline__ unsigned tile_of_block(unsigned bid, unsigned nblk) {
    const unsigned per = nblk >> 3;
    if (per == 0 || bid >= per * 8) return bid;
    return (bid & 7) * per + (bid >> 3);
}

__device__ __forceinline__ float apply_act(float v, int act) {
    if (act == 1) return fmaxf(v, 0.f);
    if (act == 2) return 1.f / (1.f + expf(-v));
    if (act == 3) return tanhf(v);
    return v;
}

__device__ __forceinline__ void chl_store(float* out, unsigned np, int f16, long long pix, int n, float x) {
    uint16_t* o = reinterpret_cast<uint16_t*>(out) + (((size_t)((n >> 4) * 4 + ((n >> 3) & 1) * 2) * np + (size_t)pix) * 8 + (size_t)(n & 7));
    uint16_t h, l;
    if (f16) {
        const _Float16 hh = (_Float16)x, ll = (_Float16)(x - (float)hh);
        h = __builtin_bit_cast(uint16_t, hh); l = __builtin_bit_cast(uint16_t, ll);
    } else {
        const __bf16 hh = (__bf16)x, ll = (__bf16)(x - (float)hh);
        h = __builtin_bit_cast(uint16_t, hh); l = __builtin_bit_cast(uint16_t, ll);
    }
    o[0] = h;
    o[(size_t)np * 8] = l;
}

template <int ACT, int PP, bool HAS_PS, bool HAS_RES, class P>
__device__ __forceinline__ void epilogue_impl(const P& p, const floatx16& acc, long long mrow0, int n, int lh) {
    if (n >= p.Cout) return;
    const float bias = p.bias ? p.bias[n] : 0.f;
    const float s = HAS_PS ? p.ps[n] : 1.f;
    const float sh = HAS_PS ? p.pt[n] : 0.f;
    if (PP > 1 && (ACT == 0 || ACT == 1) && !HAS_PS && !HAS_RES) {
        if (p.poolkind == 0) {
#pragma unroll
            for (int g = 0; g < 4; ++g) {
                const long long mb = mrow0 + 8 * g + 4 * lh;
                if (PP == 4) {
                    if (mb < p.M) {
                        float x = fmaxf(fmaxf(acc[4 * g], acc[4 * g + 1]), fmaxf(acc[4 * g + 2], acc[4 * g + 3])) + bias;
                        if (ACT == 1) x = fmaxf(x, 0.f);
                        if (p.out_np) chl_store(p.out, p.out_np, p.out_f16, mb >> 2, n, x);
                        else p.out[(size_t)(mb >> 2) * p.Cout + n] = x;
                    }
                } else {
#pragma unroll
                    for (int i = 0; i < 4; i += 2)
                        if (mb + i < p.M) {
                            float x = fmaxf(acc[4 * g + i], acc[4 * g + i + 1]) + bias;
                            if (ACT == 1) x = fmaxf(x, 0.f);
                            if (p.out_np) chl_store(p.out, p.out_np, p.out_f16, (mb + i) >> 1, n, x);
                            else p.out[(size_t)((mb + i) >> 1) * p.Cout + n] = x;
                        }
                }
            }
            return;
        }
    }
#pragma unroll
    for (int g = 0; g < 4; ++g) {
        const long long mb = mrow0 + 8 * g + 4 * lh;
        float v[4];
#pragma unroll
        for (int i = 0; i < 4; ++i) {
            float x = acc[4 * g + i] + bias;
            if (HAS_RES) { if (mb + i < p.M) x += p.res[(size_t)(mb + i) * p.Cout + n]; }
            if (ACT == 1) x = fmaxf(x, 0.f);
            else if (ACT == -1) x = apply_act(x, p.act);
            if (HAS_PS) x = x * s + sh;
            v[i] = x;
        }
        if (PP == 1) {
#pragma unroll
            for (int i = 0; i < 4; ++i)
                if (mb + i < p.M) p.out[(size_t)(mb + i) * p.Cout + n] = v[i];
        } else if (PP == 4) {
            if (mb < p.M) {
                const float r = p.poolkind == 0 ? fmaxf(fmaxf(v[0], v[1]), fmaxf(v[2], v[3]))
                                                : (v[0] + v[1] + v[2] + v[3]) * 0.25f;
                p.out[(size_t)(mb >> 2) * p.Cout + n] = r;
            }
        } else {
#pragma unroll
            for (int i = 0; i < 4; i += 2)
                if (mb + i < p.M) {
                    const float r = p.poolkind == 0 ? fmaxf(v[i], v[i + 1]) : (v[i] + v[i + 1]) * 0.5f;
                    p.out[(size_t)((mb + i) >> 1) * p.Cout + n] = r;
                }
        }
    }
}

template <int PP, class P>
// ... 198 lines not shown
```

inaspeechsegmenter_amd/csrc/conv_dhl.h:

```cpp
#pragma once
#include "conv_ws.h"

namespace issk {

constexpr int DHL_BM = 128, DHL_BN = 192, DHL_BK = 32;
constexpr int DHL_A = DHL_BM * DHL_BK * 4;
constexpr int DHL_B = DHL_BN * DHL_BK * 4;
constexpr int DHL_STAGE = DHL_A + DHL_B;

struct DhlArgs {
    const uint16_t* a;
    const uint16_t* wp;
    const float* bias;
    float* out;
    unsigned np;
    int M, K, Cout, act;
};

#ifndef ISS_DHL_NW
#define ISS_DHL_NW 8
#endif
template <bool F16, int NW = ISS_DHL_NW>
__global__ __launch_bounds__(NW * 64, 1) void conv_dhl_kernel(const DhlArgs p) {
    static_assert(NW == 4 || NW == 8, "");
    constexpr int NT = NW * 64;
    constexpr int RB = 8 / NW;
    constexpr int NA = 1024 / NT, NB = 1536 / NT;
    __shared__ __attribute__((aligned(4096))) unsigned char smem[2 * DHL_STAGE];
    const unsigned s0 = (unsigned)(size_t)smem;
    const int tid = threadIdx.x, lane = tid & 63;
    const int wv = __builtin_amdgcn_readfirstlane(tid >> 6);
    const int li = lane & 31, lh = lane >> 5;
    const int wr = wv >> 1, wc = wv & 1;
    const int m0 = (int)blockIdx.x * DHL_BM;
    const int n0 = (int)blockIdx.y * DHL_BN;
    const int nk = p.K / DHL_BK;
    const unsigned rowbytes = (unsigned)p.K * 4u;

    unsigned a_src[NA];
#pragma unroll
    for (int j = 0; j < NA; ++j) {
        const int i = tid + NT * j, row = i >> 3, slot = i & 7;
        a_src[j] = (unsigned)(m0 + row) * rowbytes + (unsigned)((slot ^ (row & 7)) * 16);
    }
    typedef unsigned u32x4 __attribute__((ext_vector_type(4)));
    typedef u32x4 __attribute__((address_space(3)))* LdsW16;
    struct Regs { u32x4 a[NA], b[NB]; };
    auto gather = [&](Regs& r, int kt) {
        const unsigned char* ab = reinterpret_cast<const unsigned char*>(p.a) + (size_t)kt * 128;
        const unsigned char* bb = reinterpret_cast<const unsigned char*>(p.wp) + ((size_t)blockIdx.y * nk + kt) * DHL_B;
#pragma unroll
        for (int j = 0; j < NA; ++j) r.a[j] = *reinterpret_cast<const u32x4*>(ab + a_src[j]);
#pragma unroll
        for (int j = 0; j < NB; ++j) r.b[j] = *reinterpret_cast<const u32x4*>(bb + (unsigned)((tid + NT * j) * 16));
    };
    auto stage = [&](Regs& r, unsigned buf) {
        const unsigned dst = s0 + buf * (unsigned)DHL_STAGE + (unsigned)(tid * 16);
#pragma unroll
        for (int j = 0; j < NA; ++j) *(LdsW16)(dst + (unsigned)(j * NT * 16)) = r.a[j];
#pragma unroll
        for (int j = 0; j < NB; ++j) *(LdsW16)(dst + (unsigned)(DHL_A + j * NT * 16)) = r.b[j];
    };

    floatx16 acc[RB][3];
#pragma unroll
    for (int r = 0; r < RB; ++r)
#pragma unroll
        for (int c = 0; c < 3; ++c)
#pragma unroll
            for (int i = 0; i < 16; ++i) acc[r][c][i] = 0.f;

    const unsigned a_rd = (unsigned)((wr * 32 * RB + li) * 128 + (((2 * lh) ^ (li & 7)) * 16));
    const unsigned b_rd = (unsigned)(DHL_A + (wc * 96 + li) * 16 + lh * 2 * 3072);
    struct Frag { bf16x8 ah[RB], al[RB], bh[3], bl[3]; };
    auto read_frags = [&](Frag& f, unsigned st, int ks) {
#pragma unroll
        for (int r = 0; r < RB; ++r) {
            f.ah[r] = *(LdsR16)(st + ((a_rd + (unsigned)(r * 32 * 128)) ^ (unsigned)(ks * 4 * 16)));
            f.al[r] = *(LdsR16)(st + ((a_rd + (unsigned)(r * 32 * 128)) ^ (unsigned)(ks * 4 * 16 + 16)));
        }
#pragma unroll
        for (int c = 0; c < 3; ++c) {
            f.bh[c] = *(LdsR16)(st + b_rd + (unsigned)(ks * 4 * 3072 + c * 32 * 16));
            f.bl[c] = *(LdsR16)(st + b_rd + (unsigned)(ks * 4 * 3072 + 3072 + c * 32 * 16));
        }
    };
    auto mfmas = [&](const Frag& f) {
#pragma unroll
        for (int term = 0; term < 3; ++term)
#pragma unroll
            for (int r = 0; r < RB; ++r)
#pragma unroll
                for (int c = 0; c < 3; ++c)
                    acc[r][c] = mfma_x3<F16>(term == 1 ? f.bl[c] : f.bh[c], term == 0 ? f.al[r] : f.ah[r], acc[r][c]);
    };

    Regs r0, r1;
    gather(r0, 0);
    gather(r1, nk > 1 ? 1 : 0);
    stage(r0, 0u);
    __syncthreads();
    int kt = 0;
    unsigned cur = 0;
#ifndef ISS_DHL_EXP
#define ISS_DHL_EXP 0
#endif
    Frag f0, f1;
    if (ISS_DHL_EXP & 8) { read_frags(f0, s0, 0); read_frags(f1, s0, 1); }
    auto step = [&](Regs& rload, Regs& rstage) {
        const unsigned st = s0 + cur * (unsigned)DHL_STAGE;
        if (!(ISS_DHL_EXP & 8)) read_frags(f0, st, 0);
        if (!(ISS_DHL_EXP & 16)) gather(rload, kt + 2 < nk ? kt + 2 : nk - 1);
        if (!(ISS_DHL_EXP & 8)) read_frags(f1, st, 1);
        __builtin_amdgcn_sched_barrier(0);
        mfmas(f0);
        __builtin_amdgcn_sched_barrier(0);
        if (!(ISS_DHL_EXP & 4)) stage(rstage, cur ^ 1u);
        __builtin_amdgcn_sched_barrier(0);
        mfmas(f1);
        __builtin_amdgcn_sched_barrier(0);
        if (!(ISS_DHL_EXP & 32)) __syncthreads();
        ++kt;
        cur ^= 1u;
    };
    while (true) {
        step(r0, r1);
        if (kt >= nk) break;
        step(r1, r0);
        if (kt >= nk) break;
    }
#pragma unroll
    for (int r = 0; r < RB; ++r) {
        const int m = m0 + (wr * RB + r) * 32 + li;
        if (m >= p.M) continue;
        float* orow = p.out + (size_t)m * p.Cout;
#pragma unroll
        for (int c = 0; c < 3; ++c)
#pragma unroll
            for (int g = 0; g < 4; ++g) {
                const int n = n0 + wc * 96 + c * 32 + 8 * g + 4 * lh;
                if (n >= p.Cout) continue;
                float4 v = make_float4(acc[r][c][4 * g], acc[r][c][4 * g + 1], acc[r][c][4 * g + 2], acc[r][c][4 * g + 3]);
                if (p.bias) { const float4 b4 = *reinterpret_cast<const float4*>(p.bias + n); v.x += b4.x; v.y += b4.y; v.z += b4.z; v.w += b4.w; }
                if (p.act == 1) { v.x = fmaxf(v.x, 0.f); v.y = fmaxf(v.y, 0.f); v.z = fmaxf(v.z, 0.f); v.w = fmaxf(v.w, 0.f); }
                *reinterpret_cast<float4*>(orow + n) = v;
            }
    }
}

inline bool dhl_supported(int K, int Cout, int act, bool has_ps, bool has_res) {
    return K % DHL_BK == 0 && K >= 2 * DHL_BK && Cout % 4 == 0 && Cout >= 32 && Cout <= 16 * DHL_BN && act <= 1 && !has_ps && !has_res;
}
__host__ __device__ inline int dhl_col_tiles(int Cout) { return (Cout + DHL_BN - 1) / DHL_BN; }
inline unsigned dhl_npad(long long windows) { return (unsigned)((windows + DHL_BM - 1) / DHL_BM * DHL_BM); }
inline size_t dhl_packed_elems(int K, int Cout = DHL_BN) { return (size_t)dhl_col_tiles(Cout) * (K / 8) * 2 * DHL_BN * 8; }
void iss_dhl_pack(const uint16_t* wh, const uint16_t* wl, uint16_t* out, int Cout, int Kpad, int K, hipStream_t st);
bool iss_dhl_launch(const DhlArgs& a, hipStream_t st, const ConvInst& i);

}
```

inaspeechsegmenter_amd/csrc/conv_select.h:

```cpp
#pragma once
#include <array>
#include <numeric>
#include "iss_internal.h"
#include "conv_common.h"
#include "conv_ws.h"
#include "conv_wq.h"
#include "conv_wq3.h"
#include "conv_wq3h.h"
#include "conv_dhl.h"
#include "conv_pwc.h"
#include "conv_pw.h"

namespace issk {

inline bool ws_recip_exact(int W, long long limit) {
    const long long m = (65536 + W - 1) / W;
    return limit * (m * W - 65536) < 65536 && limit * m < (1ll << 31);
}
inline bool ws_shape_compiled(int kh, int kw) { ISS_WS_SHAPES(ISS_SHAPE_IS) return false; }
inline bool fp_shape_compiled(int kh, int kw) { ISS_FP_SHAPES(ISS_SHAPE_IS) return false; }
#ifdef ISS_PW_NO_ASM_RING
constexpr bool asm_ring_ok = false;
#else
constexpr bool asm_ring_ok = true;
// ... 4 lines not shown
    pw = R[ISS_C_FPOOLW] > 1 ? R[ISS_C_FPOOLW] : 1;
}

inline bool fill_geometry(ConvArgs& a, const int32_t* R, int bc) {
    a.H = R[ISS_C_H]; a.W = R[ISS_C_W]; a.Cin = R[ISS_C_CIN]; a.Cout = R[ISS_C_COUT];
    fused_pool_of(R, a.ph, a.pw);
    a.pp = a.ph * a.pw;
    a.poolkind = R[ISS_C_POOLKIND];
    a.Hq = R[ISS_C_HO] / a.ph; a.Wq = R[ISS_C_WO] / a.pw;
    a.H_k = R[ISS_C_KH]; a.kw = R[ISS_C_KW];
    a.sh = R[ISS_C_SH]; a.sw = R[ISS_C_SW]; a.pt_ = R[ISS_C_PT]; a.pl_ = R[ISS_C_PL];
    a.act = R[ISS_C_ACT];
    a.M = (long long)bc * a.Hq * a.Wq * a.pp;
    if (R[ISS_C_INMODE] == 1) { a.row_stride = 24; a.pix_stride = 1; a.img_stride = 0; }
    else if (R[ISS_C_INMODE] == 2) { a.row_stride = 1; a.pix_stride = a.H; a.img_stride = 0; }
    else { a.row_stride = a.W * a.Cin; a.pix_stride = a.Cin; a.img_stride = (long long)a.H * a.W * a.Cin; }
    return a.pt_ != 0 || a.pl_ != 0 || (R[ISS_C_HO] - 1) * a.sh - a.pt_ + a.H_k > a.H || (R[ISS_C_WO] - 1) * a.sw - a.pl_ + a.kw > a.W;
}
inline double conv_flops(const int32_t* R, double M) { return 2.0 * R[ISS_C_KH] * R[ISS_C_KW] * R[ISS_C_CIN] * (double)R[ISS_C_COUT] * M; }

inline int footprint_pixels(const ConvArgs& a, int TM) {
    const long long rows_per_sample = (long long)a.Hq * a.Wq * a.pp;
    const long long lim_rows = std::lcm(rows_per_sample, (long long)TM);
    auto pix_of = [&](long long m, int ky, int kx) {
        long long q = m;
        int dy = 0, dx = 0;
        if (a.pp > 1) { q = m / a.pp; const int j = (int)(m - q * a.pp); dy = j / a.pw; dx = j - dy * a.pw; }
        const int hw = a.Hq * a.Wq;
        const long long b = q / hw;
        const int rem = (int)(q - b * hw);
        const int qy = rem / a.Wq, qx = rem - qy * a.Wq;
        const int oy = qy * a.ph + dy, ox = qx * a.pw + dx;
        return (b * a.H + (oy * a.sh - a.pt_ + ky)) * a.W + (ox * a.sw - a.pl_ + kx);
    };
    long long worst = 0;
    for (long long m0 = 0; m0 < lim_rows; m0 += TM) {
        const long long m_last = m0 + TM - 1;
        const long long lo = pix_of(m0, 0, 0), hi = pix_of(m_last, a.H_k - 1, a.kw - 1);
        worst = std::max<long long>(worst, hi - lo + 1);
        for (long long m = m0; m <= m_last; ++m)
            if (pix_of(m, 0, 0) < lo || pix_of(m, a.H_k - 1, a.kw - 1) > hi) return 0x7fffffff;
    }
    return (int)std::min<long long>(worst, 0x7fffffff);
}
inline int tile_span(IssNet& n, int r, const ConvArgs& a, int TM) {
    auto it = n.fp_pix.find({r, TM, 0, 0});
    if (it == n.fp_pix.end()) it = n.fp_pix.emplace(std::array<int, 4>{r, TM, 0, 0}, footprint_pixels(a, TM)).first;
    return it->second;
}
inline int tile_rows(IssNet& n, int r, const ConvArgs& a, int hi, int lo, int cap) {
    auto it = n.fp_pix.find({r, hi, lo, cap});
    if (it != n.fp_pix.end()) return it->second;
    int tmr = 0;
    for (int cand = hi; cand >= lo && !tmr; cand -= 4)
        if (footprint_pixels(a, cand) <= cap) tmr = cand;
    return n.fp_pix.emplace(std::array<int, 4>{r, hi, lo, cap}, tmr).first->second;
}

enum class FirstLayer { None, Fused, Gather, Alone };
enum class OutLayout { F32, Chl, ChlDense };
struct ChlState { unsigned np = 0; bool f16 = false, dense = false; };

struct ConvChoice {
    ConvInst inst;
    int row = -1, partner = -1, rows = 1;
    int tag = ISS_PROF_GATHER;
    int tmr = 0;
    FirstLayer first = FirstLayer::None;
    OutLayout out = OutLayout::F32;
    bool out_f16 = false;
    unsigned out_np = 0, in_np = 0;
    bool generic_out = false;
};

struct ConvEnv {
    IssNet& n;
    int bc, rmin, rmax;
    bool share_first;
    int prec;
    uint32_t diag;
    bool have_winrow, have_input, have_vbx;
    const ChlState* layout;
    double net_flops = 0.0;
    bool x3mode() const { return prec != ISS_PREC_F32; }
    bool f16mode() const { return prec == ISS_PREC_F16X3; }
    const int32_t* row(int r) const { return &n.prog[(size_t)r * ISS_PROG_COLS]; }
    ChlState layout_of(int buf) const { return layout && buf != ISS_BUF_INPUT ? layout[buf] : ChlState{}; }
};
inline ConvEnv make_env(IssNet& n, int bc, int rmin, int rmax, bool share_first, int prec, uint32_t diag, bool winrow, bool input, bool vbx, const ChlState* layout) {
    ConvEnv env{n, bc, rmin, rmax, share_first, prec, diag, winrow, input, vbx, layout};
    if (env.f16mode())
        for (int q = 0; q < n.nrows; ++q)
            if (env.row(q)[ISS_C_OP] == ISS_OP_CONV) env.net_flops += conv_flops(env.row(q), (double)env.row(q)[ISS_C_HO] * env.row(q)[ISS_C_WO]);
    return env;
}
inline bool sole_reader_is_next(const ConvEnv& env, int r) {
    const int ob = env.row(r)[ISS_C_OUT];
    for (int t = r + 2; t < env.n.nrows; ++t) {
        const int32_t* T = env.row(t);
        if (T[ISS_C_IN] == ob || T[ISS_C_RES] == ob) return false;
        if (T[ISS_C_OUT] == ob) break;
    }
    return true;
}

inline bool can_defer(const ConvEnv& env, int r) {
    const IssNet& n = env.n;
    if (r + 1 >= n.nrows || !env.share_first || env.rmax < env.rmin) return false;
    const bool x3mode = env.x3mode(), f32defer = !x3mode;
    if (f32defer && (env.diag & (ISS_DIAG_NO_WS | ISS_DIAG_NO_F32WS))) return false;
    const int32_t *R1 = env.row(r), *R2 = env.row(r + 1);
    int ph, pw;
    fused_pool_of(R1, ph, pw);
    const bool pool1 = ph * pw != 1;
    if (R1[ISS_C_OP] != ISS_OP_CONV || R1[ISS_C_INMODE] != 1 || R1[ISS_C_RES] >= 0 || R1[ISS_C_ACT] > 1) return false;
    if (pool1 && (R1[ISS_C_POOLKIND] != 0 || !x3mode || (env.diag & ISS_DIAG_NO_GFUSED))) return false;
    if (R1[ISS_C_CIN] != 1 || R1[ISS_C_SH] != 1 || R1[ISS_C_SW] != 1) return false;
    const bool valid1 = R1[ISS_C_PT] == 0 && R1[ISS_C_PL] == 0 && R1[ISS_C_HO] == R1[ISS_C_H] - R1[ISS_C_KH] + 1 &&
                        R1[ISS_C_WO] == R1[ISS_C_W] - R1[ISS_C_KW] + 1;
    const bool same_geo = !valid1 && R1[ISS_C_HO] == R1[ISS_C_H] && R1[ISS_C_WO] == R1[ISS_C_W] && R1[ISS_C_PT] <= R1[ISS_C_KH] - 1 &&
                          R1[ISS_C_PL] <= R1[ISS_C_KW] - 1 && R1[ISS_C_KH] <= R1[ISS_C_H] && n.wsumx_off[r] >= 0 && R1[ISS_C_PSOFF] < 0 &&
                          !(env.diag & ISS_DIAG_NO_FSAME);
    const bool same_ws = same_geo && R1[ISS_C_W] * R1[ISS_C_COUT] * 4 <= WS_STAB && !(env.diag & ISS_DIAG_NO_WS) &&
                         iss_ws_fs_compiled(R2[ISS_C_KH], R2[ISS_C_KW]);
    const bool same1 = same_ws || (same_geo && x3mode && !(env.diag & ISS_DIAG_NO_GFUSED));
    if (!valid1 && !same1) return false;
    if (pool1 && !valid1) return false;
    if (f32defer && (!valid1 || !iss_ws_f32_fused_compiled(R2[ISS_C_KH], R2[ISS_C_KW]) || R2[ISS_C_SH] != 1 || R2[ISS_C_SW] != 1 ||
                     R2[ISS_C_PT] != 0 || R2[ISS_C_PL] != 0 || R1[ISS_C_PSOFF] >= 0)) return false;
    if (R1[ISS_C_KH] * R1[ISS_C_KW] * R1[ISS_C_COUT] * 4 > 48 * 1024) return false;
    if (R1[ISS_C_BOFF] < 0 || (R1[ISS_C_PSOFF] >= 0) != (R1[ISS_C_PTOFF] >= 0) || R1[ISS_C_COUT] % 4 != 0 || n.wsum_off[r] < 0) return false;
    if (R2[ISS_C_OP] != ISS_OP_CONV || R2[ISS_C_INMODE] != 0 || R2[ISS_C_IN] != R1[ISS_C_OUT] || R2[ISS_C_RES] >= 0) return false;
    if (R2[ISS_C_CIN] != R1[ISS_C_COUT] || R2[ISS_C_CIN] % XBK != 0 || R2[ISS_C_H] != R1[ISS_C_HO] / ph || R2[ISS_C_W] != R1[ISS_C_WO] / pw) return false;
    const bool ring2 = valid1 && iss_ws_ring_compiled(R2[ISS_C_KH], R2[ISS_C_KW]) && !(env.diag & (ISS_DIAG_NO_RING | ISS_DIAG_NO_WS));
    const bool foot2 = R2[ISS_C_KH] * R2[ISS_C_KW] >= 8 && (fp_shape_compiled(R2[ISS_C_KH], R2[ISS_C_KW]) || ring2) &&
                       R2[ISS_C_H] * R2[ISS_C_W] >= FPIX + 32 && R2[ISS_C_W] <= 128 && (valid1 || same_ws) && !pool1;
    const bool gath2 = x3mode && (valid1 || same_geo) && R1[ISS_C_PSOFF] < 0 && !(env.diag & ISS_DIAG_NO_GFUSED);
    if (!foot2 && !gath2) return false;
    return sole_reader_is_next(env, r);
}
inline bool chain_pair(const ConvEnv& env, int r) {
    const IssNet& n = env.n;
    if (r + 1 >= n.nrows) return false;
    const int32_t *R1 = env.row(r), *R2 = env.row(r + 1);
    int ph, pw, ph2, pw2;
    fused_pool_of(R1, ph, pw), fused_pool_of(R2, ph2, pw2);
    auto plain1x1 = [](const int32_t* R) {
        return R[ISS_C_OP] == ISS_OP_CONV && R[ISS_C_KH] == 1 && R[ISS_C_KW] == 1 && R[ISS_C_SH] == 1 && R[ISS_C_SW] == 1 &&
               R[ISS_C_PT] == 0 && R[ISS_C_PL] == 0 && R[ISS_C_INMODE] == 0 && R[ISS_C_PSOFF] < 0 && R[ISS_C_BOFF] >= 0 &&
               R[ISS_C_HO] == R[ISS_C_H] && R[ISS_C_WO] == R[ISS_C_W];
    };
    return plain1x1(R1) && plain1x1(R2) && ph * pw == 1 && ph2 * pw2 == 1 && R1[ISS_C_DUALW] == 0 &&
           R1[ISS_C_RES] >= 0 && R1[ISS_C_RES] == R1[ISS_C_OUT] && R1[ISS_C_IN] != R1[ISS_C_OUT] && R1[ISS_C_IN] != ISS_BUF_INPUT &&
           R1[ISS_C_ACT] == 1 && R2[ISS_C_IN] == R1[ISS_C_OUT] && R2[ISS_C_RES] < 0 && R2[ISS_C_OUT] != R1[ISS_C_OUT] &&
           R2[ISS_C_OUT] != R1[ISS_C_IN] && R2[ISS_C_ACT] <= 1 && R2[ISS_C_CIN] == R1[ISS_C_COUT] && pwc_compiled(R1[ISS_C_CIN], R2[ISS_C_COUT]) &&
           R2[ISS_C_H] == R1[ISS_C_HO] && R2[ISS_C_W] == R1[ISS_C_WO] && n.kpad[r] == R1[ISS_C_CIN] && n.kpad[r + 1] == R2[ISS_C_CIN];
}
inline bool small_row_of(const ConvEnv& env, int r, int pend, bool* f16_dense_pw_out) {
    const int32_t* R = env.row(r);
    const double row_flops = conv_flops(R, (double)R[ISS_C_HO] * R[ISS_C_WO]);
    const bool small_cand = env.f16mode() && pend < 0 && row_flops < 0.005 * env.net_flops && row_flops < 2e6 &&
                            R[ISS_C_INMODE] == 0 && !can_defer(env, r);
    int ph, pw;
    fused_pool_of(R, ph, pw);
    *f16_dense_pw_out = small_cand && row_flops >= 2.5e5 && R[ISS_C_KH] == 1 && R[ISS_C_KW] == 1 && R[ISS_C_H] == 1 && R[ISS_C_W] == 1 &&
                        R[ISS_C_HO] == 1 && R[ISS_C_WO] == 1 && ph * pw == 1 && R[ISS_C_SH] == 1 && R[ISS_C_SW] == 1 && R[ISS_C_PT] == 0 &&
                        R[ISS_C_PL] == 0 && R[ISS_C_COUT] % 4 == 0 && R[ISS_C_CIN] % XBK == 0 && env.n.kpad[r] == R[ISS_C_CIN] && R[ISS_C_RES] < 0 &&
                        (env.diag & ISS_DIAG_NO_PW) == 0;
    return small_cand && !*f16_dense_pw_out;
}
inline bool epi_tr_simple(const ConvArgs& a) { return a.pp == 1 && a.Cout % 4 == 0 && epi_is_simple_tr(a); }
inline bool epi_pooled_relu(const ConvArgs& a) { return a.pp > 1 && epi_is_pool_relu(a); }

ConvChoice select_conv(const ConvEnv& env, int r, int pend);

inline bool want_hl_out(const ConvEnv& env, int r, long long npix) {
    if (!env.layout || (env.diag & ISS_DIAG_NO_HL) || r + 1 >= env.n.nrows) return false;
    const int32_t *R = env.row(r), *Q = env.row(r + 1);
    const int ob = R[ISS_C_OUT];
    if (Q[ISS_C_OP] != ISS_OP_CONV || Q[ISS_C_IN] != ob || Q[ISS_C_OUT] == ob || Q[ISS_C_CIN] != R[ISS_C_COUT] || (R[ISS_C_COUT] % (2 * BN) != 0 && R[ISS_C_COUT] != BN)) return false;
    if (npix != (long long)env.bc * Q[ISS_C_H] * Q[ISS_C_W] || !chl_fits(npix, R[ISS_C_COUT])) return false;
    ConvEnv f32in = env;
    f32in.layout = nullptr;
    return select_conv(f32in, r + 1, -1).inst.kernel == ConvKernel::Wq3 && sole_reader_is_next(env, r);
}
inline bool want_dhl_out(const ConvEnv& env, int r, int hq, int wq) {
    const IssNet& n = env.n;
    if (!env.layout || (env.diag & ISS_DIAG_NO_HL) || r + 1 >= n.nrows || !env.x3mode()) return false;
    const int32_t *R = env.row(r), *Q = env.row(r + 1);
    const int ob = R[ISS_C_OUT], bc = env.bc;
    const long long K = (long long)hq * wq * R[ISS_C_COUT];
    int qph, qpw;
    fused_pool_of(Q, qph, qpw);
    if (Q[ISS_C_OP] != ISS_OP_CONV || Q[ISS_C_IN] != ob || Q[ISS_C_OUT] == ob || Q[ISS_C_INMODE] != 0 || Q[ISS_C_RES] >= 0 || Q[ISS_C_DUALW] != 0) return false;
    if (Q[ISS_C_KH] != 1 || Q[ISS_C_KW] != 1 || Q[ISS_C_H] != 1 || Q[ISS_C_W] != 1 || Q[ISS_C_HO] != 1 || Q[ISS_C_WO] != 1 || qph * qpw != 1) return false;
    if (Q[ISS_C_CIN] != K || n.kpad[r + 1] != K || hq * wq < 2 || R[ISS_C_COUT] % 8 != 0) return false;
    if (!dhl_supported((int)K, Q[ISS_C_COUT], Q[ISS_C_ACT], Q[ISS_C_PSOFF] >= 0, false)) return false;
    const size_t bytes = (size_t)dhl_npad(bc) * (size_t)K * 4;
    if (bytes > (size_t)bc * K * 4 + ISS_ACT_SLACK || bytes >= 0xFFF00000ull || (long long)bc * hq * wq * (hq * wq) >= (1ll << 32)) return false;
    if ((long long)bc * Q[ISS_C_COUT] * 4 >= (1ll << 32)) return false;
    return sole_reader_is_next(env, r);
}

inline ConvChoice select_row(const ConvEnv& env, int r, int pend, int dual, int chain) {
    IssNet& n = env.n;
    const int32_t* R = env.row(r);
    const int32_t* Rp = pend >= 0 ? env.row(pend) : nullptr;
    const int bc = env.bc;
    const uint32_t diag = env.diag;
    static const float has = 0.f;
    ConvChoice ch;
    ConvInst& inst = ch.inst;
    ConvArgs a;
    memset(&a, 0, sizeof(a));
    const bool padded = fill_geometry(a, R, bc);
    a.bias = R[ISS_C_BOFF] >= 0 ? &has : nullptr; a.res = R[ISS_C_RES] >= 0 ? &has : nullptr;
    a.ps = R[ISS_C_PSOFF] >= 0 ? &has : nullptr; a.pt = R[ISS_C_PTOFF] >= 0 ? &has : nullptr;
    a.Kpad = n.kpad[r];
    const bool patch = R[ISS_C_INMODE] == 1, window = R[ISS_C_INMODE] == 2;
    auto present = [&](const int32_t* Q) { return Q[ISS_C_IN] != ISS_BUF_INPUT || env.have_input; };
    bool f16_dense_pw = false;
    const bool small_row = small_row_of(env, r, pend, &f16_dense_pw);
    const bool x3 = env.x3mode() && !small_row, f16mode = env.f16mode();
    const ChlState in_l = env.layout_of(R[ISS_C_IN]);
    ch.row = r; inst.kh = a.H_k; inst.kw = a.kw; inst.padded = padded; inst.window = window;
    if (in_l.np && in_l.dense) {
        inst.kernel = ConvKernel::Dhl; inst.f16 = in_l.f16; ch.in_np = in_l.np; ch.tag = ISS_PROF_PW;
        return ch;
    }
    a.mode = patch ? 2 : window ? 1 : ((a.Cin % (x3 ? XBK : 4) == 0) ? 0 : 1);
    inst.mode = a.mode;
    const double fl = conv_flops(R, (double)a.M);
    if (chain >= 0) {
        const int32_t* Q = env.row(chain);
        a.bias2 = Q[ISS_C_BOFF] >= 0 ? &has : nullptr;
        a.out = R[ISS_C_RES] == R[ISS_C_OUT] ? const_cast<float*>(a.res) : nullptr;
        a.act2 = Q[ISS_C_ACT]; a.Cout2 = Q[ISS_C_COUT];
        if (!x3 || a.mode != 0 || !present(R) || !pwc_supported(a)) return ch;
        inst.kernel = ConvKernel::Pwc; ch.partner = chain; ch.rows = 2; inst.c1 = a.Cin / 32; inst.c3 = a.Cout2 / 32; ch.tag = ISS_PROF_PW;
        return ch;
    }
    if (dual >= 0) {
        const int32_t* P = env.row(dual);
        a.Cin2 = P[ISS_C_CIN]; a.H2 = P[ISS_C_H]; a.W2 = P[ISS_C_W]; a.sh2 = P[ISS_C_SH]; a.sw2 = P[ISS_C_SW];
        a.bias = &has; a.res = nullptr;
        a.Kpad = a.Cin + a.Cin2;
        if (!x3 || a.mode != 0 || !present(R) || !present(P) || !pws2_dual_supported(a)) return ch;
        inst.kernel = ConvKernel::Pws2Dual; inst.simple_pw = true; ch.partner = dual; ch.rows = 2; ch.tag = ISS_PROF_PW;
        return ch;
    }
    const int taps = a.H_k * a.kw;
    const bool unit_stride = a.sh == 1 && a.sw == 1;
    bool fp = x3 && a.mode == 0 && fp_shape_compiled(a.H_k, a.kw) && a.M < (1ll << 31) && tile_span(n, r, a, BM) <= FPIX;
    const bool no_ws = (diag & ISS_DIAG_NO_WS) != 0;
    const bool fs1 = Rp && Rp[ISS_C_HO] == Rp[ISS_C_H];
    const bool pool1 = Rp && (Rp[ISS_C_FPOOLH] > 1 || Rp[ISS_C_FPOOLW] > 1);
    const bool affine1 = Rp && Rp[ISS_C_PSOFF] >= 0;
    bool ws = !no_ws && fp && Rp && taps >= 8 && taps <= WS_MAXNT && ws_shape_compiled(a.H_k, a.kw) &&
              a.Cin % F2_CH == 0 && a.H * a.W >= WS_PIX + 64 + (a.pt_ + 1) * a.W && ws_recip_exact(a.W, a.H * a.W + WS_PIX + a.W) &&
              tile_span(n, r, a, WS_TM) <= WS_PIX && !affine1;
    bool ws_ring = false;
    int tmr = 0;
    if (!no_ws && !(diag & ISS_DIAG_NO_RING) && Rp && !fs1 && x3 && a.mode == 0 && iss_ws_ring_compiled(a.H_k, a.kw) &&
        unit_stride && a.Cin % F2_CH == 0 && a.Cin >= 2 * F2_CH && a.M < (1ll << 31) &&
        ws_recip_exact(a.W, a.H * a.W + WS_PIX2 + a.W) && !affine1) {
        const int cap = std::min<long long>(WS_PIX2, (long long)a.H * a.W - 64 - (long long)(a.pt_ + 1) * a.W);
        tmr = tile_rows(n, r, a, WS_TM, 320, cap);
        ws_ring = tmr > 0 && a.M % 4 == 0;
        if (ws_ring) { ws = true; fp = true; } else tmr = 0;
    }
    const bool no_f32ws = (diag & ISS_DIAG_NO_F32WS) != 0;
    bool ws_f32 = !x3 && !no_ws && !no_f32ws && Rp && !fs1 && a.mode == 0 && iss_ws_f32_fused_compiled(a.H_k, a.kw) && !padded &&
                  unit_stride && epi_is_pool_relu(a) && a.Cin % F2_CH == 0 && a.Cin >= 2 * F2_CH && a.M < (1ll << 31) &&
                  a.H * a.W >= WS_PIX + 64 + a.W && ws_recip_exact(a.W, a.H * a.W + WS_PIX + a.W) && !affine1 && tile_span(n, r, a, WS_TM) <= WS_PIX;
    if (ws_f32) { ws = true; fp = true; }
    const bool fs_tr = a.pp == 1 && a.Cout % 4 == 0;
    const bool fs_tr_ok = fs_tr && a.H_k == 5 && a.kw == 3 && !padded && epi_is_simple_tr(a);
    const bool ws_fs = fs1 && ws && iss_ws_fs_compiled(a.H_k, a.kw) && (!fs_tr || fs_tr_ok) && unit_stride && a.W * a.Cin * 4 <= WS_STAB &&
                       a.Cin >= 2 * F2_CH && !(diag & ISS_DIAG_NO_FSAME);
    if (fs1 && !ws_fs) ws = false;
    const bool nh2_pad_pool = epi_pooled_relu(a);
    const bool nh2_pad_ok = epi_tr_simple(a) || nh2_pad_pool;
    const bool nh2_f32 = !x3 && !no_f32ws && !padded && (epi_tr_simple(a) || epi_pooled_relu(a));
    const bool plain3 = !no_ws && pend < 0 && a.mode == 0 && unit_stride && !a.res && a.Cin % F2_CH == 0 && a.M < (1ll << 31) &&
                        (long long)bc * a.img_stride * 4 < (1ll << 32);
    const bool ws_nh2 = plain3 && !(diag & ISS_DIAG_NO_WS3) && (x3 || nh2_f32) && (!padded || nh2_pad_ok) && a.Cout % (2 * BN) == 0 &&
                        iss_ws_nh2_compiled(a.H_k, a.kw) && tile_span(n, r, a, WS_TM) <= WS_PIX2;
    const bool ws_plain = plain3 && !fp && x3 && padded && a.pp == 1 && a.Cout % 4 == 0 && iss_ws_plain_compiled(a.H_k, a.kw) &&
                          tile_span(n, r, a, WS_TM) <= WS_PIX;
    const bool ws_plain_u = plain3 && !(diag & ISS_DIAG_NO_WSU3) && !ws_nh2 && x3 && !padded && iss_ws_plain_compiled(a.H_k, a.kw) &&
                            a.Cin >= 2 * F2_CH && (epi_tr_simple(a) || epi_pooled_relu(a)) && tile_span(n, r, a, WS_TM) <= WS_PIX;
    bool fused = false;
    if (Rp) {
        const long long edge_rows = fs1 ? (long long)bc * (Rp[ISS_C_KH] - 1) : 0;
        fused = !pool1 && fp && (ws || (!fs1 && !padded && taps >= 12)) && env.have_winrow &&
                ((long long)(env.rmax - env.rmin) + Rp[ISS_C_HO] + edge_rows) * Rp[ISS_C_WO] * Rp[ISS_C_COUT] * 4 < (1ll << 32);
        if (ws_ring && !fused) { ws = false; fp = false; ws_ring = false; tmr = 0; }
        if (ws_f32 && !fused) { ws = false; fp = false; ws_f32 = false; }
    }
    if (!fused && (long long)bc * a.img_stride >= (1ll << 32)) fp = false;
    bool gfused = false;
    if (Rp && !fused && x3 && a.mode == 0 && env.have_winrow && !(diag & ISS_DIAG_NO_GFUSED) && !(fs1 && (diag & ISS_DIAG_NO_FSAME))) {
        gfused = (fs1 || (Rp[ISS_C_PT] == 0 && Rp[ISS_C_PL] == 0)) && Rp[ISS_C_PSOFF] < 0 && Rp[ISS_C_ACT] <= 1 && a.M < (1ll << 31) &&
                 (!fs1 || n.wsumx_off[pend] >= 0);
        if (gfused && fp) {
            const double bytes1 = (double)bc * Rp[ISS_C_HO] * Rp[ISS_C_WO] * Rp[ISS_C_COUT] * 4.0;
            gfused = fl < 360.0 * bytes1;
        }
        if (gfused) fp = false;
    }
// ... 19 lines not shown
        }
        if (kind >= 0 && (ch.tmr = tile_rows(n, r, a, WQ3_TM, WQ3_TM - 64, WQ3_PIX)) <= 0) kind = -1;
        if (kind >= 0) {
            inst.kernel = in_l.np ? ConvKernel::Wq3h : ConvKernel::Wq3;
            inst.kind = kind; ch.in_np = in_l.np; inst.f16 = in_l.np && in_l.f16;
        } else {
            inst.kernel = ConvKernel::WsNh2; inst.nh = 2;
            inst.tr = (padded && !nh2_pad_pool) || (a.pp == 1 && a.Cout % 4 == 0);
            inst.epi = padded ? 1 : (inst.tr ? epi_is_simple_tr(a) : epi_is_pool_relu(a));
        }
    } else if (ws_plain_u) {
        inst.kernel = ConvKernel::WsPlainU; inst.tr = a.pp == 1; inst.epi = 1;
    } else if (ws_plain) {
        inst.kernel = ConvKernel::WsPlain; inst.epi = epi_is_simple_tr(a);
    } else if (ws && ws_f32) {
        inst.kernel = ConvKernel::WsF32Fused; inst.epi = 1;
    } else if (ws && ws_ring) {
        inst.kernel = ConvKernel::WsRing; inst.tr = false; inst.epi = epi_is_pool_relu_any(a);
    } else if (ws && ws_fs) {
        inst.kernel = ConvKernel::WsFs; inst.tr = fs_tr_ok; inst.epi = fs_tr_ok ? 1 : (int)epi_is_pool_relu_any(a);
    } else if (ws) {
        const bool rowmajor_pool = fused && !padded && !inst.tr && epi_is_pool_relu(a) && unit_stride && a.Cin >= 2 * F2_CH;
        if (!(diag & ISS_DIAG_NO_NCB1) && rowmajor_pool && !fs1 && a.Cout <= 32 && iss_ws_ncb1_compiled(a.H_k, a.kw)) {
            inst.kernel = ConvKernel::WsNcb1; inst.epi = 1;
        } else if (!(diag & ISS_DIAG_NO_WQ) && rowmajor_pool && a.pp == 4 && a.ph == 2 && iss_wq_compiled(a.H_k, a.kw) && a.M % 4 == 0 &&
                   (a.M / 4) * (long long)a.Cout * 4 < 0xFFF00000ll && a.Cout <= 256 && (ch.tmr = tile_rows(n, r, a, WS_TM, WS_TM - 32, WQ_PIX)) > 0) {
            inst.kernel = ConvKernel::Wq; inst.f16 = f16mode;
        } else {
            inst.kernel = ConvKernel::Ws; inst.epi = inst.tr ? epi_is_simple_tr(a) : epi_is_pool_relu_any(a);
        }
    } else if (fp) {
        inst.kernel = ConvKernel::Fp;
        inst.nh = (!fused && !(diag & ISS_DIAG_NO_NH2) && iss_fp_has_nh2(a.H_k, a.kw) && a.Cout % (2 * BN) == 0) ? 2 : 1;
        inst.tr = !(diag & ISS_DIAG_NO_TR) && inst.tr;
    } else if (x3 && patch && taps <= XBK && a.M < (1ll << 31)) {
        inst.kernel = ConvKernel::Patch1; ch.tag = ISS_PROF_PATCH1; inst.tr = inst.tr && !a.res; inst.f16 = f16mode;
    } else if (x3 && gfused) {
        inst.kernel = ConvKernel::Gather;
    } else if (x3) {
        const bool pointwise = !(diag & ISS_DIAG_NO_PW) && a.mode == 0 && inst.tr && taps == 1 && unit_stride && a.pt_ == 0 &&
                               a.pl_ == 0 && R[ISS_C_HO] == a.H && R[ISS_C_WO] == a.W && a.Kpad == a.Cin;
        if (pointwise) ch.tag = ISS_PROF_PW;
        const bool no_pws = !asm_ring_ok || (diag & ISS_DIAG_NO_PWS) != 0;
        const bool no_pws2 = (diag & ISS_DIAG_NO_PWS2) != 0;
        const bool pws_ok = !no_pws && a.Kpad <= 2048 && !f16_dense_pw;
        const bool pw_strided = pws_ok && !no_pws2 && a.mode == 0 && inst.tr && taps == 1 && (a.sh > 1 || a.sw > 1) && a.pt_ == 0 &&
                                a.pl_ == 0 && a.Kpad == a.Cin && pws2_strided_supported(a, R[ISS_C_HO], R[ISS_C_WO]);
        inst.simple_pw = a.act <= 1 && !a.ps; inst.has_res = a.res != nullptr;
        if (pw_strided) { inst.kernel = ConvKernel::Pws2Strided; ch.tag = ISS_PROF_PW; }
        else if (pointwise && pws_ok && !no_pws2 && pws2_supported(a)) inst.kernel = ConvKernel::Pws2;
        else if (pointwise && pws_ok && pws_supported(a)) inst.kernel = ConvKernel::Pws;
        else if (pointwise) { inst.kernel = ConvKernel::Pw; inst.f16 = f16mode; }
        else { inst.kernel = ConvKernel::X3; inst.tr = inst.tr && a.mode != 2; }
    } else {
        inst.kernel = ConvKernel::Igemm;
    }
    if (inst.kernel == ConvKernel::Wq) {
        if (a.Cout % BN == 0 && want_hl_out(env, r, a.M / 4)) { ch.out = OutLayout::Chl; ch.out_np = chl_npad(a.M / 4); ch.out_f16 = inst.f16; }
        inst.out_hl = ch.out != OutLayout::F32;
    } else if (inst.kernel == ConvKernel::Wq3h) {
        if (inst.kind == 0 && want_hl_out(env, r, a.M)) { ch.out = OutLayout::Chl; ch.out_np = chl_npad(a.M); }
        if (inst.kind == 1 && want_dhl_out(env, r, a.Hq, a.Wq)) { ch.out = OutLayout::ChlDense; ch.out_np = dhl_npad(bc); }
        inst.out_hl = ch.out != OutLayout::F32;
        ch.out_f16 = inst.out_hl && inst.f16;
    } else if (inst.kernel != ConvKernel::Wq3 && x3 && !patch && epi_is_pool_relu(a) && a.Cout % 16 == 0 && want_hl_out(env, r, a.M / a.pp)) {
        ch.out = OutLayout::Chl; ch.out_np = chl_npad(a.M / a.pp); ch.out_f16 = f16mode; ch.generic_out = true;
    }
    return ch;
}

inline ConvChoice select_conv(const ConvEnv& env, int r, int pend) {
    const bool pair = asm_ring_ok && pend < 0 && env.x3mode() && !(env.diag & (ISS_DIAG_NO_PW | ISS_DIAG_NO_PWS | ISS_DIAG_NO_PWS2));
    if (pair && !(env.diag & ISS_DIAG_NO_CHAIN) && chain_pair(env, r)) {
        const ConvChoice ch = select_row(env, r, -1, -1, r + 1);
        if (ch.inst.kernel != ConvKernel::Declined) return ch;
    }
    if (pair && !(env.diag & ISS_DIAG_NO_DUAL) && r + 1 < env.n.nrows && env.row(r + 1)[ISS_C_DUALW] > 0) {
        const ConvChoice ch = select_row(env, r + 1, -1, r, -1);
        if (ch.inst.kernel != ConvKernel::Declined) return ch;
    }
    return select_row(env, r, pend, -1, -1);
}

inline std::string inst_name(const ConvInst& c) {
    auto B = [](bool b) { return b ? "true" : "false"; };
    char s[160];
    auto ws = [&](const char* form) {
        snprintf(s, sizeof s, "conv_x3_ws_kernel<%d,%d,%s,%s,%s,%d,%d%s>", c.kh, c.kw, B(c.padded), B(c.tr), B(c.fused), c.nh, c.epi, form);
    };
    switch (c.kernel) {
    case ConvKernel::Dhl: snprintf(s, sizeof s, "conv_dhl_kernel<%s,%d>", B(c.f16), ISS_DHL_NW); break;
    case ConvKernel::Pwc: snprintf(s, sizeof s, "conv_x3_pwc_kernel<%d,%d>", c.c1, c.c3); break;
    case ConvKernel::Pws2Dual: snprintf(s, sizeof s, "conv_x3_pws2_kernel<%s,false,dual>", B(c.simple_pw)); break;
    case ConvKernel::Direct1: snprintf(s, sizeof s, "conv1_direct3x3_kernel<%s>", B(c.window)); break;
    case ConvKernel::Wq3: snprintf(s, sizeof s, "conv_x3_wq3_kernel<%d>", c.kind); break;
    case ConvKernel::Wq3h: snprintf(s, sizeof s, "conv_x3_wq3h_kernel<%d,%s,%s>", c.kind, B(c.out_hl), B(c.f16)); break;
    case ConvKernel::WsNh2: case ConvKernel::WsPlain: case ConvKernel::Ws: ws(""); break;
    case ConvKernel::WsNh2F32: case ConvKernel::WsF32Fused: ws(",f32"); break;
    case ConvKernel::WsPlainU: ws(",plain"); break;
    case ConvKernel::WsRing: ws(",ring"); break;
    case ConvKernel::WsFs: ws(",fs"); break;
    case ConvKernel::WsNcb1: ws(",ncb1"); break;
    case ConvKernel::Wq: snprintf(s, sizeof s, "conv_x3_wq_kernel<%d,%d,%s,%s>", c.kh, c.kw, B(c.out_hl), B(c.f16)); break;
    case ConvKernel::Fp: snprintf(s, sizeof s, "conv_x3_fp_kernel<%d,%d,%s,%s,%s,%d>", c.kh, c.kw, B(c.padded), B(c.tr), B(c.fused), c.nh); break;
    case ConvKernel::Patch1: snprintf(s, sizeof s, "conv1_patch_x3_kernel<%s,%s>", B(c.tr), B(c.f16)); break;
    case ConvKernel::Gather: case ConvKernel::X3: snprintf(s, sizeof s, "conv_x3_kernel<%d,%s,2>", c.mode, B(c.tr)); break;
    case ConvKernel::Pws2Strided: snprintf(s, sizeof s, "conv_x3_pws2_kernel<%s,true>", B(c.simple_pw)); break;
    case ConvKernel::Pws2: snprintf(s, sizeof s, "conv_x3_pws2_kernel<%s,false>", B(c.simple_pw)); break;
    case ConvKernel::Pws: snprintf(s, sizeof s, "conv_x3_pws_kernel<%s,%s>", B(c.has_res), B(c.simple_pw)); break;
    case ConvKernel::Pw: snprintf(s, sizeof s, "conv_x3_pw_kernel<%s>", B(c.f16)); break;
    case ConvKernel::Igemm: snprintf(s, sizeof s, "conv_igemm_kernel<%d>", c.mode); break;
    case ConvKernel::Declined: s[0] = 0; break;
    }
    return s;
}

}
```

inaspeechsegmenter_amd/csrc/iss_internal.h:

```cpp
#pragma once
#include <hip/hip_runtime.h>
#include <array>
#include <cstdint>
#include <cstdio>
#include <cstdarg>
#include <string>
#include <vector>
#include <unordered_map>
#include <map>
#include <memory>
#include "../../include/iss.h"

struct DevBuf {
    void* p = nullptr;
    size_t cap = 0;
};

struct ConvOp;

struct IssCounters { int64_t launches = 0, units = 0; };
struct IssCodec {
    const char* name;
    DevBuf src, rows, status, stage;
    std::vector<int64_t> stage_off, stage_bytes;
// ... 2 lines not shown

struct IssParamArrays {
    float* blob = nullptr;
    uint16_t *wh = nullptr, *wl = nullptr, *wh16 = nullptr, *wl16 = nullptr;
    ~IssParamArrays();
};

struct IssNet {
    bool loaded = false;
    std::vector<int32_t> prog;
    int nrows = 0;
    float* d_blob = nullptr;
    uint16_t* d_wh = nullptr;
    uint16_t* d_wl = nullptr;
    uint16_t* d_wh16 = nullptr;
    uint16_t* d_wl16 = nullptr;
    bool f16_ok = false;
    std::shared_ptr<IssParamArrays> shared_params;
    std::map<std::pair<int, int>, uint16_t*> dhl_wp;
    float* d_wsum = nullptr;
    std::vector<int64_t> wsum_off;
    std::vector<int64_t> wsumx_off;
    int64_t blob_floats = 0;
    std::vector<int64_t> w_dev_off;
    std::vector<int32_t> kpad;
    int32_t* d_ktab = nullptr;
    std::vector<int64_t> ktab_off;
    int nbuf = 0;
    std::vector<int64_t> buf_elems;
    int in_h = 0, in_w = 0, in_c = 0, out_dim = 0;
    double flops_per_sample = 0;
    std::map<std::array<int, 4>, int> fp_pix;
    int prec_override = -1;
    bool prec_by_caller = false;
    int guard_state = 0;
    float guard_dlogp = -1.f;
    float guard_dlogp_chosen = -1.f;
    int guard_slots = 0;
};

struct iss_ctx {
    int device = -1;
    hipStream_t stream = nullptr;
    std::string err;

    bool sk_tables = false;
    double* d_window = nullptr;
    float* d_melw = nullptr;
    int32_t* d_mellim = nullptr;
    double* d_tw = nullptr;

    DevBuf sig;
    const void* sig_ptr = nullptr;
    int sig_kind = 0;
    int64_t sig_n = 0;

    struct RsFilter { int32_t up = 1, down = 1, hl = 0; int64_t ntaps = 1; double* d_taps = nullptr; };
    std::vector<RsFilter> rs_filters;
    std::map<std::pair<int32_t, int32_t>, int32_t> rs_filter_id;
    DevBuf rs_src, rs_jobs;
    IssCounters rs_count;

    IssCodec flac{"flac"}, adpcm{"adpcm"}, msadpcm{"msadpcm"};

    DevBuf mspec, loge;
    int32_t T = 0;
    bool have_feats = false;
    uint64_t feat_epoch = 1;

    uint64_t flags_epoch = 0;
    DevBuf d_rowflag;
    uint8_t* h_rowflag = nullptr;
    size_t h_rowflag_cap = 0;
    std::map<int, std::vector<int32_t>> bad_prefix;
    DevBuf d_lfinite;
    int64_t win_total = 0, win_dead = 0;

    IssNet nets[ISS_MAX_NETS];
    uint64_t ws_limit = 24ull << 30;
    int precision = ISS_PREC_F16X3;
    float guard_threshold = 5e-4f;
    bool in_guard = false;
    uint32_t diag = 0;
    std::vector<DevBuf> act;
    DevBuf d_winrow, d_stats, d_finite, d_out, d_in;
    DevBuf raw1;

    bool vbx_tables = false;
    double* d_vbx_window = nullptr;
    double* d_vbx_melw = nullptr;
    int32_t* d_vbx_mellim = nullptr;
    DevBuf vbx_sig, vbx_dither, vbx_fb, vbx_out;
    DevBuf vbx_meta;
    int32_t vbx_T = 0;
    int64_t vbx_dither_n = 0;
    IssCounters vbx_res_count;

    struct Staging { void* p = nullptr; size_t cap = 0; hipEvent_t done = nullptr; bool busy = false; };
    std::vector<Staging> staging;
    std::vector<hipEvent_t> ticket_ev;
    int64_t ticket_base = 1;
    hipEvent_t order_ev = nullptr;

    void* comm = nullptr;
    int comm_rank = 0, comm_world = 1;
    DevBuf comm_send, comm_recv;

    bool prof = false;
    double prof_ms[ISS_PROF_KINDS] = {};
    int64_t prof_launch[ISS_PROF_KINDS] = {};
    double prof_flops[ISS_PROF_KINDS] = {};
    double prof_row_ms[ISS_PROF_ROWS] = {};
    int64_t prof_row_launch[ISS_PROF_ROWS] = {};
    struct Pending { hipEvent_t a, b; int kind; int sub; int row; double flops; std::string inst; };
    std::vector<Pending> pending;
    struct Inst { std::string name; double ms = 0; int64_t launches = 0; double flops = 0; };
    std::vector<Inst> prof_inst;
    std::vector<hipEvent_t> ev_pool;
};

int iss_fail(iss_ctx* c, int code, const char* fmt, ...);
int iss_reserve(iss_ctx* c, DevBuf& b, size_t bytes);
void iss_set_signal(iss_ctx* c, const void* ptr, int kind, int64_t n);
int iss_stage_host(iss_ctx* c, const void* src, size_t bytes, void** pinned_out, int* slot_out);
void iss_stage_mark(iss_ctx* c, int slot);
int iss_rowflag_host(iss_ctx* c, size_t rows);

__host__ __device__ inline int iss_row_flag(const float* row) {
    for (int k = 0; k < 24; ++k) {
        const float v = row[k];
        if (!(v - v == 0.f)) return k;
    }
    return 24;
}

#define ISS_HIP(c, call)                                                                  \
    do {                                                                                  \
        hipError_t e__ = (call);                                                          \
        if (e__ != hipSuccess)                                                            \
            return iss_fail((c), ISS_EHIP, "%s failed: %s (%s:%d)", #call,                \
                            hipGetErrorString(e__), __FILE__, __LINE__);                  \
    } while (0)

void iss_prof_begin(iss_ctx* c, int kind, double flops);
void iss_prof_tag(iss_ctx* c, int sub);
void iss_prof_row(iss_ctx* c, int row);
void iss_prof_inst(iss_ctx* c, const char* fmt, ...);
void iss_prof_end(iss_ctx* c);
void iss_prof_collect(iss_ctx* c);

struct RsJobDev {
    int64_t src_off, n_in, dst_off, n_out, tile_base;
    const double* taps;
    int32_t ch, fmt, up, down, hl, tile, lds_tab, pad;
};
struct RsWinDev { int64_t in_begin, frames_total, out_begin, out_end; };
struct RsSplitDev { int64_t dst_stride, ntiles; int32_t sel_begin, sel_count, group, stride, ident, pad; };
struct RsMixDev { int64_t dst_stride, ntiles; int32_t mix_begin, mix_count, group, stride; };
struct RsMixRow { int32_t term_begin, term_count; double divisor; };
struct RsTermDev { int32_t channel, pad; double weight; };
static_assert(sizeof(RsMixRow) == 16 && sizeof(RsTermDev) == 16, "one array of 16-byte rows");
struct IssMixTables { const iss_mixset* sets; const iss_mix* mixes; int64_t nmixes; const iss_mix_term* terms; int64_t nterms; };
struct IssRsPlan {
    std::vector<RsJobDev> dj;
    std::vector<RsWinDev> dw;
    std::vector<RsSplitDev> ds;
// ... 15 lines not shown
```

include/iss.h:

```cpp
#ifndef ISS_H
#define ISS_H

#include <stdint.h>
#include <stddef.h>

#ifdef __cplusplus
extern "C" {
#endif

#define ISS_OK        0
#define ISS_EINVAL   -1
#define ISS_ENODEV   -2
#define ISS_EHIP     -3
#define ISS_ESTATE   -4
#define ISS_ENOMEM   -5
#define ISS_ETIMEOUT -6

typedef struct iss_ctx iss_ctx;

int         iss_create(int device_id, iss_ctx** out);
void        iss_destroy(iss_ctx* ctx);
const char* iss_last_error(const iss_ctx* ctx);
const char* iss_version(void);
int         iss_set_workspace_limit(iss_ctx* ctx, uint64_t bytes);
// ... 202 lines not shown
#define ISS_PROG_COLS  32

enum {
    ISS_OP_CONV     = 1,
    ISS_OP_POOL     = 2,
    ISS_OP_SOFTMAX  = 3,
    ISS_OP_STATPOOL = 4,
    ISS_OP_ACT      = 5,
    ISS_OP_ELT      = 6,
};
enum { ISS_ELT_COPY = 0, ISS_ELT_ADD = 1, ISS_ELT_SUB = 2, ISS_ELT_MUL = 3, ISS_ELT_MAX = 4, ISS_ELT_MIN = 5, ISS_ELT_AVG = 6,
       ISS_ELT_ZERO = 7, ISS_ELT_PERMUTE = 8 };
enum {
    ISS_C_OP = 0, ISS_C_IN, ISS_C_OUT, ISS_C_RES,
    ISS_C_H, ISS_C_W, ISS_C_CIN, ISS_C_HO, ISS_C_WO, ISS_C_COUT,
    ISS_C_KH, ISS_C_KW, ISS_C_SH, ISS_C_SW, ISS_C_PT, ISS_C_PL,
    ISS_C_ACT,
    ISS_C_WOFF, ISS_C_BOFF,
    ISS_C_PSOFF, ISS_C_PTOFF,
    ISS_C_INMODE,
    ISS_C_POOLKIND,
    ISS_C_ORDER,
    ISS_C_FPOOLH, ISS_C_FPOOLW,
    ISS_C_DUALW, ISS_C_DUALB,
    ISS_C_ACTPARAM,
    ISS_C_ACTPARAM2, ISS_C_ACTPARAM3,
};
#define ISS_BUF_INPUT  (-2)

int iss_cnn_load(iss_ctx* ctx, int net_id, const int32_t* prog, int32_t nrows,
                 const float* blob, int64_t blob_floats,
                 int32_t nbuf, const int64_t* buf_elems,
                 int32_t in_h, int32_t in_w, int32_t in_c, int32_t out_dim);
int iss_cnn_load_shared(iss_ctx* ctx, int net_id, int src_id, const int32_t* prog, int32_t nrows,
                        int32_t nbuf, const int64_t* buf_elems,
                        int32_t in_h, int32_t in_w, int32_t in_c, int32_t out_dim);

int iss_cnn_probs(iss_ctx* ctx, int net_id, const int32_t* win_row, int32_t n,
                  float* probs_out , uint8_t* finite_out );

int iss_cnn_probs_async(iss_ctx* ctx, int net_id, const int32_t* win_row, int32_t n,
                        float* probs_out , uint8_t* finite_out , int64_t* ticket_out);
int iss_cnn_dead_stats(iss_ctx* ctx, int64_t* windows, int64_t* dead);
int iss_wait(iss_ctx* ctx, int64_t ticket);

int iss_cnn_forward(iss_ctx* ctx, int net_id, const float* x, int32_t n, float* out );

#define ISS_PREC_BF16X3 0
#define ISS_PREC_F32    1
#define ISS_PREC_F16X3  2
int iss_set_precision(iss_ctx* ctx, int mode);

#define ISS_GUARD_PENDING   0
#define ISS_GUARD_PASSED    1
#define ISS_GUARD_ESCALATED 2
#define ISS_GUARD_FIXED     3
int iss_set_precision_guard(iss_ctx* ctx, float threshold);
int iss_cnn_precision_info(iss_ctx* ctx, int id, int32_t* mode, float* max_dlogp, int32_t* slots, int32_t* state, float* dlogp_in_use);
int iss_cnn_set_net_precision(iss_ctx* ctx, int id, int mode);

#define ISS_DIAG_NO_SHARED_FIRST 0x001u
#define ISS_DIAG_NO_FLROWS       0x002u
#define ISS_DIAG_NO_WS           0x004u
#define ISS_DIAG_NO_WS3          0x008u
#define ISS_DIAG_NO_DIRECT1      0x010u
#define ISS_DIAG_NO_NH2          0x020u
#define ISS_DIAG_NO_TR           0x040u
#define ISS_DIAG_NO_PW           0x080u
#define ISS_DIAG_NO_PWS          0x100u
#define ISS_DIAG_NO_PWS2         0x200u
#define ISS_DIAG_NO_WQ           0x400u
#define ISS_DIAG_NO_DUAL         0x800u
#define ISS_DIAG_NO_CHAIN        0x1000u
#define ISS_DIAG_NO_RING         0x2000u
#define ISS_DIAG_NO_FSAME        0x4000u
#define ISS_DIAG_NO_F32WS        0x8000u
#define ISS_DIAG_NO_NCB1         0x10000u
#define ISS_DIAG_NO_WSU3         0x20000u
#define ISS_DIAG_NO_GFUSED       0x40000u
#define ISS_DIAG_NO_HL           0x80000u
#define ISS_DIAG_NO_SKIP_DEAD    0x100000u
#define ISS_DIAG_ALL             0x1fffffu
int iss_set_diag(iss_ctx* ctx, uint32_t flags);

int iss_cnn_flops(iss_ctx* ctx, int net_id, double* flops_per_sample);

int iss_vbx_tables(iss_ctx* ctx, const double* window400, const double* melbank_257x64);
int iss_vbx_features(iss_ctx* ctx, const int32_t* sig_i32, const double* dither_u, int64_t n,
                     float* fea_out , int32_t* T_out);
int iss_vbx_set_dither(iss_ctx* ctx, const double* dither_u, int64_t n);
int iss_vbx_features_pcm16(iss_ctx* ctx, const int16_t* pcm, int64_t n,
                           float* fea_out , int32_t* T_out);
int iss_vbx_features_batch_pcm16(iss_ctx* ctx, const int16_t* pcm, const int64_t* sample_off, int32_t nfiles,
                                 int32_t* frame_off_out, float* fea_out );
int iss_vbx_features_resident(iss_ctx* ctx, const int64_t* sample_begin, const int64_t* sample_count, int32_t nparts,
                              int32_t* frame_off_out, float* fea_out );
int iss_vbx_resident_stats(iss_ctx* ctx, int64_t* launches, int64_t* parts);
int iss_vbx_embed(iss_ctx* ctx, int net_id, const int32_t* starts, int32_t n, float* out );

#define ISS_COMM_ID_BYTES 128
int iss_comm_unique_id(iss_ctx* ctx, uint8_t id_out[ISS_COMM_ID_BYTES]);
int iss_comm_init(iss_ctx* ctx, const uint8_t id[ISS_COMM_ID_BYTES], int32_t rank, int32_t world);
int iss_comm_destroy(iss_ctx* ctx);
int iss_allgather_segments(iss_ctx* ctx, const int32_t* local_rows, int32_t n_local, int32_t capacity,
                           int32_t* all_rows, int32_t* counts );
int iss_comm_allreduce_max(iss_ctx* ctx, double* value);
int iss_comm_info(iss_ctx* ctx, int32_t* world, int32_t* rank, int32_t* version, char* lib_path, int32_t lib_path_len);

#define ISS_PROF_GEMM      0
#define ISS_PROF_FRONTEND  1
#define ISS_PROF_OTHER     2
#define ISS_PROF_WS        3
#define ISS_PROF_FP        4
#define ISS_PROF_PW        5
#define ISS_PROF_GATHER    6
#define ISS_PROF_PATCH1    7
#define ISS_PROF_F32       8
#define ISS_PROF_KINDS     9
int iss_prof_enable(iss_ctx* ctx, int on);
int iss_prof_get(iss_ctx* ctx, int kind, double* ms, int64_t* launches, double* flops);
int iss_prof_reset(iss_ctx* ctx);
#define ISS_PROF_ROWS      512
int iss_prof_get_row(iss_ctx* ctx, int row, double* ms, int64_t* launches);
int iss_prof_get_instance(iss_ctx* ctx, int index, char* name_out, int32_t name_len, double* ms, int64_t* launches, double* flops);

int iss_scribble(iss_ctx* ctx, uint32_t word);

int iss_viterbi_f64(const double* emission, int64_t T, int32_t K, const double* transition,
                    int32_t* states_out);
int iss_viterbi_f32(const float* emission, int64_t T, int32_t K, const double* transition,
                    int32_t* states_out);
int iss_viterbi_segments_f32(const float* emission, const int64_t* seg_len, int64_t nseg, int32_t K,
                             const double* transition, int32_t* states_out);
int iss_energy_viterbi(const float* loge, int64_t T, double threshold, double log_eps, double log_1m_eps,
                       const double* transition, int32_t* states_out);

#ifdef __cplusplus
}
#endif
#endif
```

Before: 7.243.

## Fuse dense classifier head and softmax into DHL conv kernel epilogue

When the last pointwise conv is followed by two 1x1 dense layers and a softmax, the DHL kernel now runs those layers with f32 MFMA in LDS and writes the masked probabilities straight to the output slots. This removes the separate dense-layer launches, the softmax and mask/scatter kernels, and the intermediate buffers between them. When host output buffers are mapped, results are written directly to pinned host memory, which also drops the device-to-host copies. The cost is more LDS and registers per DHL block, plus host-side filling of dead slots. Switches allow turning the fused head or the direct host write off.

```diff
diff --git a/inaspeechsegmenter_amd/_native.py b/inaspeechsegmenter_amd/_native.py
--- a/inaspeechsegmenter_amd/_native.py
+++ b/inaspeechsegmenter_amd/_native.py
@@ -172,6 +172,7 @@
         'iss_cnn_probs': (C.c_int, [vp, C.c_int, pi32, i32, pf, pu8]),
         'iss_cnn_forward': (C.c_int, [vp, C.c_int, pf, i32, pf]),
         'iss_cnn_flops': (C.c_int, [vp, C.c_int, pd]),
+        'iss_cnn_head_plan': (C.c_int, [pi32, i32, i32, pi64, i32, i32, i32, i32, C.c_int, C.c_uint32, i32, pi32]),
         'iss_set_precision': (C.c_int, [vp, C.c_int]),
         'iss_set_precision_guard': (C.c_int, [vp, C.c_float]),
         'iss_cnn_precision_info': (C.c_int, [vp, C.c_int, pi32, pf, pi32, pi32, pf]),
@@ -190,6 +191,7 @@
         'iss_prof_get_row': (C.c_int, [vp, C.c_int, pd, pi64]),
         'iss_prof_get_instance': (C.c_int, [vp, C.c_int, C.c_char_p, i32, pd, pi64, pd]),
         'iss_set_diag': (C.c_int, [vp, C.c_uint32]),
+        'iss_set_head_switches': (C.c_int, [vp, C.c_uint32]),
         'iss_scribble': (C.c_int, [vp, C.c_uint32]),
         'iss_viterbi_f64': (C.c_int, [pd, i64, i32, pd, pi32]),
         'iss_viterbi_f32': (C.c_int, [pf, i64, i32, pd, pi32]),
@@ -209,14 +211,26 @@
              'no_nh2': 0x020, 'no_tr': 0x040, 'no_pw': 0x080, 'no_pws': 0x100, 'no_pws2': 0x200, 'no_wq': 0x400,
              'no_dual': 0x800, 'no_chain': 0x1000, 'no_ring': 0x2000, 'no_fsame': 0x4000, 'no_f32ws': 0x8000, 'no_ncb1': 0x10000, 'no_wsu3': 0x20000, 'no_gfused': 0x40000, 'no_hl': 0x80000,
              'no_skip_dead': 0x100000}
+HEAD_SWITCHES = {'no_head': 0x1, 'no_host_out': 0x2}
+
+
+def _switch_names(names):
+    return [nm for nm in str(names).replace(' ', '').replace('+', ',').lower().split(',') if nm]
 
 
 def diag_flags(names):
     flags = 0
-    for nm in str(names).replace(' ', '').replace('+', ',').lower().split(','):
-        if nm:
-            flags |= DIAG_BITS[nm]
+    for nm in _switch_names(names):
+        flags |= DIAG_BITS[nm]
     return flags
+
+
+def split_switches(names):
+    nm = _switch_names(names)
+    head = 0
+    for k in nm:
+        head |= HEAD_SWITCHES.get(k, 0)
+    return diag_flags(','.join(k for k in nm if k not in HEAD_SWITCHES)), head
 
 
 def _ptr(a, ty):
@@ -267,6 +281,19 @@
     if rc != 0:
         raise NativeError(f"iss_energy_viterbi failed ({rc}): T={x.size}")
     return out
+
+
+def cnn_head_plan(compiled, windows, prec=PREC_F16X3, diag=0):
+    prog = np.ascontiguousarray(compiled.prog, dtype=np.int32)
+    be = np.ascontiguousarray(compiled.buf_elems, dtype=np.int64)
+    h, w, c = compiled.in_shape
+    flags = diag_flags(diag) if isinstance(diag, str) else int(diag)
+    row = C.c_int32(-1)
+    got = lib().iss_cnn_head_plan(_ptr(prog, C.c_int32), prog.shape[0], be.size, _ptr(be, C.c_int64), h, w, c, compiled.out_dim,
+                                  int(prec), flags, int(windows), C.byref(row))
+    if got < 0:
+        raise NativeError(f'iss_cnn_head_plan failed ({got})')
+    return row.value, got
 
 
 def flac_crc(buf):
@@ -341,9 +368,12 @@
         self.precision = None
         self.workspace_limit = None
         self.diag = 0
+        self.head_switches = 0
         env = os.environ.get('ISS_DIAG', '')
         if env:
-            self.set_diag(diag_flags(env))
+            diag, head = split_switches(env)
+            self.set_diag(diag)
+            self.set_head_switches(head)
         self.guard_threshold = None
         env = os.environ.get('ISS_PREC_GUARD', '')
         if env:
@@ -676,6 +706,8 @@
             self.set_workspace_limit(other.workspace_limit)
         if getattr(other, 'diag', 0) != getattr(self, 'diag', 0):
             self.set_diag(other.diag)
+        if getattr(other, 'head_switches', 0) != getattr(self, 'head_switches', 0):
+            self.set_head_switches(other.head_switches)
         if getattr(other, 'guard_threshold', None) is not None and other.guard_threshold != getattr(self, 'guard_threshold', None):
             self.set_precision_guard(other.guard_threshold)
 
@@ -683,6 +715,11 @@
         flags = diag_flags(flags) if isinstance(flags, str) else int(flags)
         self._ck(self._L.iss_set_diag(self._h, flags), 'iss_set_diag')
         self.diag = flags
+
+    def set_head_switches(self, flags):
+        flags = split_switches(flags)[1] if isinstance(flags, str) else int(flags)
+        self._ck(self._L.iss_set_head_switches(self._h, flags), 'iss_set_head_switches')
+        self.head_switches = flags
 
     def scribble(self, word):
         self._ck(self._L.iss_scribble(self._h, int(word) & 0xFFFFFFFF), 'iss_scribble')
diff --git a/inaspeechsegmenter_amd/csrc/cnn.hip b/inaspeechsegmenter_amd/csrc/cnn.hip
--- a/inaspeechsegmenter_amd/csrc/cnn.hip
+++ b/inaspeechsegmenter_amd/csrc/cnn.hip
@@ -849,12 +849,7 @@
 __global__ void softmax_kernel(const float* __restrict__ in, float* __restrict__ out, long long rows, int C) {
     const long long r = (long long)blockIdx.x * blockDim.x + threadIdx.x;
     if (r >= rows) return;
-    const float* x = in + r * C;
-    float mx = x[0];
-    for (int i = 1; i < C; ++i) mx = fmaxf(mx, x[i]);
-    float s = 0.f;
-    for (int i = 0; i < C; ++i) s += expf(x[i] - mx);
-    for (int i = 0; i < C; ++i) out[r * C + i] = expf(x[i] - mx) / s;
+    softmax_row(in + r * C, out + r * C, C);
 }
 
 __global__ void statpool_kernel(const float* __restrict__ in, float* __restrict__ out, long long total, int H, int W, int C) {
@@ -1233,6 +1228,13 @@
     return ISS_OK;
 }
 
+extern "C" int iss_set_head_switches(iss_ctx* c, uint32_t flags) {
+    if (!c) return ISS_EINVAL;
+    if (flags & ~(uint32_t)(ISS_HEAD_OFF | ISS_HEAD_NO_HOST_OUT)) return iss_fail(c, ISS_EINVAL, "iss_set_head_switches: unknown bits 0x%x", flags);
+    c->head_switches = flags;
+    return ISS_OK;
+}
+
 extern "C" int iss_cnn_flops(iss_ctx* c, int id, double* f) {
     if (!c || id < 0 || id >= ISS_MAX_NETS || !f) return ISS_EINVAL;
     if (!c->nets[id].loaded) return iss_fail(c, ISS_ESTATE, "net %d not loaded", id);
@@ -1242,7 +1244,8 @@
 
 namespace {
 
-struct PassIo { const int32_t* d_winrow; const float* d_stats; const uint8_t* d_fin; const float* d_input; };
+struct HeadOut { float* probs; uint8_t* fin_out; const int32_t* map; };
+struct PassIo { const int32_t* d_winrow; const float* d_stats; const uint8_t* d_fin; const float* d_input; const HeadOut* head; };
 
 int conv_args(iss_ctx* c, IssNet& n, const PassIo& io, int bc, const ConvChoice& ch, ConvArgs& a) {
     const int r = ch.row;
@@ -1410,7 +1413,7 @@
     return false;
 }
 
-int launch_conv(iss_ctx* c, IssNet& n, const ConvChoice& ch, ConvArgs& a, double fl) {
+int launch_conv(iss_ctx* c, IssNet& n, const PassIo& io, const ConvChoice& ch, ConvArgs& a, double fl) {
     const int r = ch.row;
     const int32_t* R = &n.prog[(size_t)r * ISS_PROG_COLS];
     const ConvInst& i = ch.inst;
@@ -1433,7 +1436,14 @@
             ISS_HIP(c, hipMalloc((void**)&wp, dhl_packed_elems(K, R[ISS_C_COUT]) * 2));
             iss_dhl_pack((i.f16 ? n.d_wh16 : n.d_wh) + R[ISS_C_WOFF], (i.f16 ? n.d_wl16 : n.d_wl) + R[ISS_C_WOFF], wp, R[ISS_C_COUT], n.kpad[r], K, st);
         }
-        DhlArgs d;
+        DhlArgs d{};
+        if (i.head) {
+            const int32_t *Q = R + ISS_PROG_COLS, *P = Q + ISS_PROG_COLS;
+            if (!io.head || !io.head->probs || !io.d_fin) return iss_fail(c, ISS_EINVAL, "internal: row %d runs the head without a place for its result", r);
+            d.w2 = n.d_blob + Q[ISS_C_WOFF]; d.b2 = Q[ISS_C_BOFF] >= 0 ? n.d_blob + Q[ISS_C_BOFF] : nullptr; d.act2 = Q[ISS_C_ACT];
+            d.w3 = n.d_blob + P[ISS_C_WOFF]; d.b3 = P[ISS_C_BOFF] >= 0 ? n.d_blob + P[ISS_C_BOFF] : nullptr; d.C = P[ISS_C_COUT];
+            d.fin = io.d_fin; d.map = io.head->map; d.probs = io.head->probs; d.fin_out = io.head->fin_out;
+        }
         d.a = reinterpret_cast<const uint16_t*>(a.in); d.wp = wp; d.bias = a.bias; d.out = a.out;
         d.np = ch.in_np; d.M = (int)a.M; d.K = K; d.Cout = R[ISS_C_COUT]; d.act = R[ISS_C_ACT];
         ok = iss_dhl_launch(d, st, i);
@@ -1495,20 +1505,22 @@
     if (rc) return rc;
     double fl = conv_flops(R, (double)a.M);
     if (ch.inst.kernel == ConvKernel::Dhl) fl = 2.0 * R[ISS_C_CIN] * (double)R[ISS_C_COUT] * (double)env.bc;
+    if (ch.inst.head) fl += 2.0 * ((double)DHL_BN * DHL_H2 + (double)DHL_H2 * n.out_dim) * (double)env.bc;
     if (ch.inst.kernel == ConvKernel::Pwc) fl += 2.0 * a.Cout * (double)a.Cout2 * (double)a.M;
     if (ch.inst.kernel == ConvKernel::Pws2Dual) fl += 2.0 * a.Cin2 * (double)a.Cout * (double)a.M;
     if (ch.first == FirstLayer::Fused || ch.first == FirstLayer::Gather)
         if ((rc = launch_shared_first_layer(c, n, io, pend, env.bc, env.rmin, env.rmax, a, &fl))) return rc;
-    return launch_conv(c, n, ch, a, fl);
+    return launch_conv(c, n, io, ch, a, fl);
 }
 
 int run_program(iss_ctx* c, IssNet& n, int bc, const int32_t* d_winrow, const float* d_stats,
                 const uint8_t* d_fin, const float* d_input, float** result, int rmin = 0, int rmax = -1,
-                bool share_first = false) {
-    const PassIo io{d_winrow, d_stats, d_fin, d_input};
+                bool share_first = false, const HeadOut* head = nullptr) {
+    const PassIo io{d_winrow, d_stats, d_fin, d_input, head};
     std::vector<ChlState> layout(std::max<size_t>(c->act.size(), (size_t)n.nbuf));
     ConvEnv env = make_env(n, bc, rmin, rmax, share_first, effective_precision(c, n), c->diag, d_winrow != nullptr, d_input != nullptr,
                            c->vbx_out.p != nullptr, layout.data());
+    env.head = head != nullptr;
     int pending = -1;
     for (int r = 0; r < n.nrows; ++r) {
         const int32_t* R = &n.prog[(size_t)r * ISS_PROG_COLS];
@@ -1525,6 +1537,11 @@
             if (pending >= 0) layout[n.prog[(size_t)pending * ISS_PROG_COLS + ISS_C_OUT]] = ChlState{};
             pending = -1;
             if (rc) return rc;
+            if (ch.inst.head) {
+                ISS_HIP(c, hipGetLastError());
+                *result = nullptr;
+                return ISS_OK;
+            }
             if (ch.rows == 1 && env.layout_of(R[ISS_C_IN]).np && !ch.in_np)
                 return iss_fail(c, ISS_EINVAL, "internal: row %d reads a CHL tensor on a kernel that expects f32", r);
             if (ch.rows == 2) {
@@ -1586,6 +1603,7 @@
         if (op != ISS_OP_CONV && R[ISS_C_IN] != ISS_BUF_INPUT && layout[R[ISS_C_IN]].np)
             return iss_fail(c, ISS_EINVAL, "internal: row %d reads a CHL tensor", r);
     }
+    if (head) return iss_fail(c, ISS_EINVAL, "internal: no launch of this pass ran the head (pass_head_rows said one would)");
     return ISS_OK;
 }
 
@@ -1761,7 +1779,44 @@
     const int32_t* d_map = (const int32_t*)c->d_winrow.p + nlive;
     uint8_t* d_fin = compact ? (uint8_t*)c->d_lfinite.p : (uint8_t*)c->d_finite.p;
     const long long tot = (long long)nslots * n.out_dim;
-    if (compact) {
+    bool share = !(c->diag & ISS_DIAG_NO_SHARED_FIRST);
+    if (nlive > 0) {
+        int gmin = rows[0], gmax = rows[0];
+        for (int i = 1; i < nlive; ++i) { gmin = std::min(gmin, rows[i]); gmax = std::max(gmax, rows[i]); }
+        if ((long long)(gmax - gmin + 68) * 4 > (long long)nlive * 68) share = false;
+    }
+    struct Pass { int s0, cur, rmin, rmax; };
+    std::vector<Pass> passes;
+    for (int s0 = 0; s0 < nlive; s0 += bc) {
+        Pass ps{s0, std::min(bc, nlive - s0), rows[s0], rows[s0]};
+        for (int i = s0 + 1; i < s0 + ps.cur; ++i) { ps.rmin = std::min(ps.rmin, rows[i]); ps.rmax = std::max(ps.rmax, rows[i]); }
+        passes.push_back(ps);
+    }
+    bool head = async && !passes.empty() && !(c->head_switches & ISS_HEAD_OFF);
+    for (size_t i = 0; i < passes.size() && head; ++i) {
+        int hrow;
+        head = pass_head_rows(n, passes[i].cur, passes[i].rmin, passes[i].rmax, share, effective_precision(c, n), c->diag, c->vbx_out.p != nullptr, &hrow) > 0;
+    }
+    float* out_probs = (float*)c->d_out.p;
+    uint8_t* out_fin = (uint8_t*)c->d_finite.p;
+    bool direct = false;
+    if (head && !(c->head_switches & ISS_HEAD_NO_HOST_OUT)) {
+        void *dp = nullptr, *df = nullptr;
+        if (hipHostGetDevicePointer(&dp, probs_out, 0) == hipSuccess && hipHostGetDevicePointer(&df, finite_out, 0) == hipSuccess && dp && df) {
+            direct = true; out_probs = (float*)dp; out_fin = (uint8_t*)df;
+        } else {
+            (void)hipGetLastError();
+        }
+    }
+    if (direct && compact) {
+        std::vector<uint8_t> live((size_t)nslots, 0);
+        for (int j = 0; j < nlive; ++j) live[lm[(size_t)nlive + j]] = 1;
+        for (int i = 0; i < nslots; ++i)
+            if (!live[i]) {
+                for (int k = 0; k < n.out_dim; ++k) probs_out[(size_t)i * n.out_dim + k] = 0.5f;
+                finite_out[i] = 0;
+            }
+    } else if (compact) {
         iss_prof_begin(c, 2, 0);
         hipLaunchKernelGGL(fill_half_kernel, dim3((unsigned)((tot + 255) / 256)), dim3(256), 0, c->stream, (float*)c->d_out.p, tot);
         iss_prof_end(c);
@@ -1775,20 +1830,15 @@
         iss_prof_end(c);
         ISS_HIP(c, hipGetLastError());
     }
-    bool share = !(c->diag & ISS_DIAG_NO_SHARED_FIRST);
-    if (nlive > 0) {
-        int gmin = rows[0], gmax = rows[0];
-        for (int i = 1; i < nlive; ++i) { gmin = std::min(gmin, rows[i]); gmax = std::max(gmax, rows[i]); }
-        if ((long long)(gmax - gmin + 68) * 4 > (long long)nlive * 68) share = false;
-    }
-    for (int s0 = 0; s0 < nlive; s0 += bc) {
-        const int cur = std::min(bc, nlive - s0);
+    for (const Pass& ps : passes) {
+        const int s0 = ps.s0, cur = ps.cur;
         float* res = nullptr;
-        int rmin = rows[s0], rmax = rows[s0];
-        for (int i = s0 + 1; i < s0 + cur; ++i) { rmin = std::min(rmin, rows[i]); rmax = std::max(rmax, rows[i]); }
+        const HeadOut ho = compact ? HeadOut{out_probs, out_fin, d_map + s0}
+                                   : HeadOut{out_probs + (size_t)s0 * n.out_dim, direct ? out_fin + s0 : nullptr, nullptr};
         rc = run_program(c, n, cur, (const int32_t*)c->d_winrow.p + s0, (const float*)c->d_stats.p + 2 * (size_t)s0,
-                         (const uint8_t*)d_fin + s0, nullptr, &res, rmin, rmax, share);
+                         (const uint8_t*)d_fin + s0, nullptr, &res, ps.rmin, ps.rmax, share, head ? &ho : nullptr);
         if (rc) return rc;
+        if (head) continue;
         if (compact) {
             const long long ct = (long long)cur * n.out_dim;
             iss_prof_begin(c, 2, 0);
@@ -1801,13 +1851,15 @@
                                       hipMemcpyDeviceToDevice, c->stream));
         }
     }
-    if (!compact) {
+    if (!compact && !head) {
         hipLaunchKernelGGL(mask_probs_kernel, dim3((unsigned)((tot + 255) / 256)), dim3(256), 0, c->stream,
                            (float*)c->d_out.p, (const uint8_t*)c->d_finite.p, (long long)nslots, n.out_dim);
         ISS_HIP(c, hipGetLastError());
     }
-    ISS_HIP(c, hipMemcpyAsync(probs_out, c->d_out.p, (size_t)tot * 4, hipMemcpyDeviceToHost, c->stream));
-    ISS_HIP(c, hipMemcpyAsync(finite_out, c->d_finite.p, (size_t)nslots, hipMemcpyDeviceToHost, c->stream));
+    if (!direct) {
+        ISS_HIP(c, hipMemcpyAsync(probs_out, c->d_out.p, (size_t)tot * 4, hipMemcpyDeviceToHost, c->stream));
+        ISS_HIP(c, hipMemcpyAsync(finite_out, c->d_finite.p, (size_t)nslots, hipMemcpyDeviceToHost, c->stream));
+    }
     if (async) {
         hipEvent_t ev;
         if (!c->ev_pool.empty()) { ev = c->ev_pool.back(); c->ev_pool.pop_back(); }
@@ -1820,6 +1872,26 @@
     ISS_HIP(c, hipStreamSynchronize(c->stream));
     iss_prof_collect(c);
     return ISS_OK;
+}
+
+extern "C" int iss_cnn_head_plan(const int32_t* prog, int32_t nrows, int32_t nbuf, const int64_t* buf_elems, int32_t in_h, int32_t in_w,
+                                 int32_t in_c, int32_t out_dim, int prec, uint32_t diag, int32_t windows, int32_t* row_out) {
+    if (!prog || nrows <= 0 || nbuf <= 0 || !buf_elems || windows <= 0 || !row_out || prec < 0 || prec > ISS_PREC_F16X3) return ISS_EINVAL;
+    IssNet n;
+    std::vector<int32_t> ktab;
+    int rc = cnn_set_program(nullptr, n, "iss_cnn_head_plan", prog, nrows, INT64_MAX / 2, nbuf, buf_elems, in_h, in_w, in_c, out_dim, ktab);
+    if (rc) return rc < 0 ? rc : -rc;
+    n.wsum_off.assign(nrows, -1);
+    n.wsumx_off.assign(nrows, -1);
+    for (int r = 0; r < nrows; ++r) {
+        const int32_t* R = &n.prog[(size_t)r * ISS_PROG_COLS];
+        if (R[ISS_C_OP] != ISS_OP_CONV || R[ISS_C_INMODE] != 1) continue;
+        n.wsum_off[r] = 0;
+        if ((R[ISS_C_PT] != 0 || R[ISS_C_PL] != 0 || R[ISS_C_WO] == R[ISS_C_W]) && R[ISS_C_CIN] == 1 && R[ISS_C_SW] == 1) n.wsumx_off[r] = 0;
+    }
+    const int rmax = 2 * (windows - 1);
+    const bool share = !(diag & ISS_DIAG_NO_SHARED_FIRST) && (long long)(rmax + 68) * 4 <= (long long)windows * 68;
+    return pass_head_rows(n, windows, 0, rmax, share, prec, diag, false, row_out);
 }
 
 extern "C" int iss_cnn_probs(iss_ctx* c, int id, const int32_t* win_row, int32_t nslots, float* probs_out,
diff --git a/inaspeechsegmenter_amd/csrc/cnn_dhl.hip b/inaspeechsegmenter_amd/csrc/cnn_dhl.hip
--- a/inaspeechsegmenter_amd/csrc/cnn_dhl.hip
+++ b/inaspeechsegmenter_amd/csrc/cnn_dhl.hip
@@ -24,9 +24,13 @@
 }
 bool iss_dhl_launch(const DhlArgs& a, hipStream_t st, const ConvInst& i) {
     const dim3 grid((unsigned)((a.M + DHL_BM - 1) / DHL_BM), (unsigned)dhl_col_tiles(a.Cout));
-#define ISS_DHL_TRY(F16_) ISS_LAUNCH_IF(i.kernel == ConvKernel::Dhl && i.f16 == F16_, (conv_dhl_kernel<F16_>), grid, ISS_DHL_NW * 64, 0)
-    ISS_DHL_TRY(true)
-    ISS_DHL_TRY(false)
+#define ISS_DHL_TRY(F16_, HEAD_) \
+    ISS_LAUNCH_IF(i.kernel == ConvKernel::Dhl && i.f16 == F16_ && i.head == HEAD_, (conv_dhl_kernel<F16_, ISS_DHL_NW, HEAD_>), grid, ISS_DHL_NW * 64, 0)
+    ISS_DHL_TRY(true, false)
+    ISS_DHL_TRY(false, false)
+#if ISS_DHL_NW == 8
+    ISS_DHL_TRY(true, true)
+#endif
 #undef ISS_DHL_TRY
     return false;
 }
diff --git a/inaspeechsegmenter_amd/csrc/conv_common.h b/inaspeechsegmenter_amd/csrc/conv_common.h
--- a/inaspeechsegmenter_amd/csrc/conv_common.h
+++ b/inaspeechsegmenter_amd/csrc/conv_common.h
@@ -79,6 +79,7 @@
     int kh = 0, kw = 0, mode = 0, epi = 0, nh = 1, kind = -1, c1 = 0, c3 = 0;
     bool padded = false, tr = false, fused = false, f16 = false, window = false, has_res = false, simple_pw = false;
     bool out_hl = false;
+    bool head = false;
 };
 #define ISS_LAUNCH_IF(WHEN, KERNEL, GRID, THREADS, LDS) \
     if (WHEN) { hipLaunchKernelGGL(KERNEL, GRID, dim3(THREADS), LDS, st, a); return true; }
@@ -145,6 +146,14 @@
     if (act == 2) return 1.f / (1.f + expf(-v));
     if (act == 3) return tanhf(v);
     return v;
+}
+
+__device__ __forceinline__ void softmax_row(const float* x, float* out, int C) {
+    float mx = x[0];
+    for (int i = 1; i < C; ++i) mx = fmaxf(mx, x[i]);
+    float s = 0.f;
+    for (int i = 0; i < C; ++i) s += expf(x[i] - mx);
+    for (int i = 0; i < C; ++i) out[i] = expf(x[i] - mx) / s;
 }
 
 __device__ __forceinline__ void chl_store(float* out, unsigned np, int f16, long long pix, int n, float x) {
diff --git a/inaspeechsegmenter_amd/csrc/conv_dhl.h b/inaspeechsegmenter_amd/csrc/conv_dhl.h
--- a/inaspeechsegmenter_amd/csrc/conv_dhl.h
+++ b/inaspeechsegmenter_amd/csrc/conv_dhl.h
@@ -15,18 +15,32 @@
     float* out;
     unsigned np;
     int M, K, Cout, act;
+    const float* w2;
+    const float* b2;
+    const float* w3;
+    const float* b3;
+    const uint8_t* fin;
+    const int32_t* map;
+    float* probs;
+    uint8_t* fin_out;
+    int act2, C;
 };
+constexpr int DHL_H2 = 128;
+constexpr int DHL_CMAX = 8;
+constexpr int DHL_HLD = DHL_BN + 4;
+constexpr int DHL_HEAD_LDS = DHL_BM * DHL_HLD * 4 + 2 * DHL_BM * DHL_CMAX * 4;
 
 #ifndef ISS_DHL_NW
 #define ISS_DHL_NW 8
 #endif
-template <bool F16, int NW = ISS_DHL_NW>
+template <bool F16, int NW = ISS_DHL_NW, bool HEAD = false>
 __global__ __launch_bounds__(NW * 64, 1) void conv_dhl_kernel(const DhlArgs p) {
     static_assert(NW == 4 || NW == 8, "");
+    static_assert(!HEAD || NW == 8, "the head is written for the 4 x 2 wave grid");
     constexpr int NT = NW * 64;
     constexpr int RB = 8 / NW;
     constexpr int NA = 1024 / NT, NB = 1536 / NT;
-    __shared__ __attribute__((aligned(4096))) unsigned char smem[2 * DHL_STAGE];
+    __shared__ __attribute__((aligned(4096))) unsigned char smem[HEAD ? (DHL_HEAD_LDS > 2 * DHL_STAGE ? DHL_HEAD_LDS : 2 * DHL_STAGE) : 2 * DHL_STAGE];
     const unsigned s0 = (unsigned)(size_t)smem;
     const int tid = threadIdx.x, lane = tid & 63;
     const int wv = __builtin_amdgcn_readfirstlane(tid >> 6);
@@ -129,6 +143,83 @@
         step(r1, r0);
         if (kt >= nk) break;
     }
+    if constexpr (HEAD) {
+        float* hs = reinterpret_cast<float*>(smem);
+        float* lg = hs + DHL_BM * DHL_HLD;
+        __syncthreads();
+#pragma unroll
+        for (int r = 0; r < RB; ++r) {
+            float* hrow = hs + ((wr * RB + r) * 32 + li) * DHL_HLD;
+#pragma unroll
+            for (int c = 0; c < 3; ++c)
+#pragma unroll
+                for (int g = 0; g < 4; ++g) {
+                    const int n = wc * 96 + c * 32 + 8 * g + 4 * lh;
+                    float4 v = make_float4(acc[r][c][4 * g], acc[r][c][4 * g + 1], acc[r][c][4 * g + 2], acc[r][c][4 * g + 3]);
+                    if (p.bias) { const float4 b4 = *reinterpret_cast<const float4*>(p.bias + n); v.x += b4.x; v.y += b4.y; v.z += b4.z; v.w += b4.w; }
+                    if (p.act == 1) { v.x = fmaxf(v.x, 0.f); v.y = fmaxf(v.y, 0.f); v.z = fmaxf(v.z, 0.f); v.w = fmaxf(v.w, 0.f); }
+                    *reinterpret_cast<float4*>(hrow + n) = v;
+                }
+        }
+        __syncthreads();
+        const float* arow = hs + (wr * 32 + li) * DHL_HLD + lh * 4;
+        auto tile_k = [&](floatx16& c0, floatx16& c1, const float* w0, const float* w1, int K, bool two) {
+            for (int k = 0; k < K; k += 8) {
+                const float4 a = *reinterpret_cast<const float4*>(arow + k);
+                const float4 b0 = *reinterpret_cast<const float4*>(w0 + k);
+                c0 = __builtin_amdgcn_mfma_f32_32x32x2f32(a.x, b0.x, c0, 0, 0, 0);
+                c0 = __builtin_amdgcn_mfma_f32_32x32x2f32(a.y, b0.y, c0, 0, 0, 0);
+                c0 = __builtin_amdgcn_mfma_f32_32x32x2f32(a.z, b0.z, c0, 0, 0, 0);
+                c0 = __builtin_amdgcn_mfma_f32_32x32x2f32(a.w, b0.w, c0, 0, 0, 0);
+                if (two) {
+                    const float4 b1 = *reinterpret_cast<const float4*>(w1 + k);
+                    c1 = __builtin_amdgcn_mfma_f32_32x32x2f32(a.x, b1.x, c1, 0, 0, 0);
+                    c1 = __builtin_amdgcn_mfma_f32_32x32x2f32(a.y, b1.y, c1, 0, 0, 0);
+                    c1 = __builtin_amdgcn_mfma_f32_32x32x2f32(a.z, b1.z, c1, 0, 0, 0);
+                    c1 = __builtin_amdgcn_mfma_f32_32x32x2f32(a.w, b1.w, c1, 0, 0, 0);
+                }
+            }
+        };
+        floatx16 c0, c1;
+#pragma unroll
+        for (int i = 0; i < 16; ++i) { c0[i] = 0.f; c1[i] = 0.f; }
+        const int n2 = wc * 64 + li;
+        tile_k(c0, c1, p.w2 + (size_t)n2 * DHL_BN + lh * 4, p.w2 + (size_t)(n2 + 32) * DHL_BN + lh * 4, DHL_BN, true);
+        __syncthreads();
+        {
+            const float bia0 = p.b2 ? p.b2[n2] : 0.f, bia1 = p.b2 ? p.b2[n2 + 32] : 0.f;
+#pragma unroll
+            for (int i = 0; i < 16; ++i) {
+                float* o = hs + (wr * 32 + 8 * (i >> 2) + 4 * lh + (i & 3)) * DHL_HLD + n2;
+                float x0 = c0[i] + bia0, x1 = c1[i] + bia1;
+                if (p.act2 == 1) { x0 = fmaxf(x0, 0.f); x1 = fmaxf(x1, 0.f); }
+                o[0] = x0; o[32] = x1;
+            }
+        }
+        __syncthreads();
+        if (wc == 0) {
+#pragma unroll
+            for (int i = 0; i < 16; ++i) c0[i] = 0.f;
+            const int cls = li < p.C ? li : 0;
+            tile_k(c0, c1, p.w3 + (size_t)cls * DHL_H2 + lh * 4, nullptr, DHL_H2, false);
+            if (li < p.C) {
+                const float bia = p.b3 ? p.b3[li] : 0.f;
+#pragma unroll
+                for (int i = 0; i < 16; ++i) lg[(wr * 32 + 8 * (i >> 2) + 4 * lh + (i & 3)) * DHL_CMAX + li] = c0[i] + bia;
+            }
+        }
+        __syncthreads();
+        if (tid < DHL_BM && m0 + tid < p.M) {
+            const int m = m0 + tid;
+            const float* pr = lg + DHL_BM * DHL_CMAX + tid * DHL_CMAX;
+            softmax_row(lg + tid * DHL_CMAX, lg + DHL_BM * DHL_CMAX + tid * DHL_CMAX, p.C);
+            const uint8_t f = p.fin[m];
+            const size_t slot = p.map ? (size_t)p.map[m] : (size_t)m;
+            for (int i = 0; i < p.C; ++i) p.probs[slot * p.C + i] = f ? pr[i] : 0.5f;
+            if (p.fin_out) p.fin_out[slot] = f;
+        }
+        return;
+    }
 #pragma unroll
     for (int r = 0; r < RB; ++r) {
         const int m = m0 + (wr * RB + r) * 32 + li;
diff --git a/inaspeechsegmenter_amd/csrc/conv_select.h b/inaspeechsegmenter_amd/csrc/conv_select.h
--- a/inaspeechsegmenter_amd/csrc/conv_select.h
+++ b/inaspeechsegmenter_amd/csrc/conv_select.h
@@ -110,6 +110,7 @@
     bool have_winrow, have_input, have_vbx;
     const ChlState* layout;
     double net_flops = 0.0;
+    bool head = false;
     bool x3mode() const { return prec != ISS_PREC_F32; }
     bool f16mode() const { return prec == ISS_PREC_F16X3; }
     const int32_t* row(int r) const { return &n.prog[(size_t)r * ISS_PROG_COLS]; }
@@ -230,6 +231,31 @@
     return sole_reader_is_next(env, r);
 }
 
+inline int head_rows(const ConvEnv& env, int r, bool f16) {
+    const IssNet& n = env.n;
+    if (!env.head || ISS_DHL_NW != 8 || !f16 || r + 4 != n.nrows) return 0;
+    const int32_t *R = env.row(r), *Q = env.row(r + 1), *P = env.row(r + 2), *S = env.row(r + 3);
+    if (R[ISS_C_COUT] != DHL_BN || R[ISS_C_ACT] > 1) return 0;
+    ConvEnv f32in = env;
+    f32in.layout = nullptr;
+    auto dense_f32 = [&](int q, const int32_t* prev, int cin, int maxact) {
+        const int32_t* D = env.row(q);
+        int ph, pw;
+        if (D[ISS_C_OP] != ISS_OP_CONV) return false;
+        fused_pool_of(D, ph, pw);
+        if (D[ISS_C_IN] != prev[ISS_C_OUT] || D[ISS_C_OUT] == D[ISS_C_IN] || D[ISS_C_INMODE] != 0 || D[ISS_C_RES] >= 0 || D[ISS_C_DUALW] != 0 ||
+            D[ISS_C_PSOFF] >= 0 || D[ISS_C_PTOFF] >= 0 || D[ISS_C_ACT] > maxact || ph * pw != 1) return false;
+        if (D[ISS_C_KH] != 1 || D[ISS_C_KW] != 1 || D[ISS_C_H] != 1 || D[ISS_C_W] != 1 || D[ISS_C_HO] != 1 || D[ISS_C_WO] != 1 || D[ISS_C_SH] != 1 ||
+            D[ISS_C_SW] != 1 || D[ISS_C_PT] != 0 || D[ISS_C_PL] != 0 || D[ISS_C_CIN] != cin || n.kpad[q] != cin) return false;
+        const ConvChoice ch = select_conv(f32in, q, -1);
+        return ch.inst.kernel == ConvKernel::Igemm && ch.inst.mode == 0 && ch.rows == 1 && ch.row == q && sole_reader_is_next(env, q - 1);
+    };
+    if (!dense_f32(r + 1, R, DHL_BN, 1) || Q[ISS_C_COUT] != DHL_H2) return 0;
+    if (!dense_f32(r + 2, Q, DHL_H2, 0) || P[ISS_C_COUT] > DHL_CMAX || P[ISS_C_COUT] != n.out_dim) return 0;
+    if (S[ISS_C_OP] != ISS_OP_SOFTMAX || S[ISS_C_IN] != P[ISS_C_OUT] || S[ISS_C_H] != 1 || S[ISS_C_W] != 1 || S[ISS_C_CIN] != P[ISS_C_COUT]) return 0;
+    return 3;
+}
+
 inline ConvChoice select_row(const ConvEnv& env, int r, int pend, int dual, int chain) {
     IssNet& n = env.n;
     const int32_t* R = env.row(r);
@@ -254,6 +280,8 @@
     ch.row = r; inst.kh = a.H_k; inst.kw = a.kw; inst.padded = padded; inst.window = window;
     if (in_l.np && in_l.dense) {
         inst.kernel = ConvKernel::Dhl; inst.f16 = in_l.f16; ch.in_np = in_l.np; ch.tag = ISS_PROF_PW;
+        const int hr = head_rows(env, r, inst.f16);
+        inst.head = hr > 0; ch.rows = 1 + hr;
         return ch;
     }
     a.mode = patch ? 2 : window ? 1 : ((a.Cin % (x3 ? XBK : 4) == 0) ? 0 : 1);
@@ -439,6 +467,29 @@
     return select_row(env, r, pend, -1, -1);
 }
 
+inline int pass_head_rows(IssNet& n, int bc, int rmin, int rmax, bool share_first, int prec, uint32_t diag, bool have_vbx, int* row) {
+    std::vector<ChlState> layout((size_t)std::max(n.nbuf, 1));
+    ConvEnv env = make_env(n, bc, rmin, rmax, share_first, prec, diag, true, false, have_vbx, layout.data());
+    env.head = true;
+    int pending = -1;
+    *row = -1;
+    for (int r = 0; r < n.nrows; ++r) {
+        const int32_t* R = env.row(r);
+        ChlState out_layout;
+        if (R[ISS_C_OP] == ISS_OP_CONV) {
+            if (pending < 0 && can_defer(env, r)) { pending = r; continue; }
+            const ConvChoice ch = select_conv(env, r, pending);
+            if (pending >= 0) layout[env.row(pending)[ISS_C_OUT]] = ChlState{};
+            pending = -1;
+            if (ch.inst.head) { *row = r; return ch.rows - 1; }
+            if (ch.rows == 2) { layout[R[ISS_C_OUT]] = ChlState{}; R = env.row(++r); }
+            if (ch.out != OutLayout::F32) out_layout = ChlState{ch.out_np, ch.out_f16, ch.out == OutLayout::ChlDense};
+        }
+        layout[R[ISS_C_OUT]] = out_layout;
+    }
+    return 0;
+}
+
 inline std::string inst_name(const ConvInst& c) {
     auto B = [](bool b) { return b ? "true" : "false"; };
     char s[160];
diff --git a/inaspeechsegmenter_amd/csrc/iss_internal.h b/inaspeechsegmenter_amd/csrc/iss_internal.h
--- a/inaspeechsegmenter_amd/csrc/iss_internal.h
+++ b/inaspeechsegmenter_amd/csrc/iss_internal.h
@@ -108,6 +108,7 @@
     float guard_threshold = 5e-4f;
     bool in_guard = false;
     uint32_t diag = 0;
+    uint32_t head_switches = 0;
     std::vector<DevBuf> act;
     DevBuf d_winrow, d_stats, d_finite, d_out, d_in;
     DevBuf raw1;
diff --git a/include/iss.h b/include/iss.h
--- a/include/iss.h
+++ b/include/iss.h
@@ -308,8 +308,14 @@
 #define ISS_DIAG_NO_SKIP_DEAD    0x100000u
 #define ISS_DIAG_ALL             0x1fffffu
 int iss_set_diag(iss_ctx* ctx, uint32_t flags);
+#define ISS_HEAD_OFF             0x1u
+#define ISS_HEAD_NO_HOST_OUT     0x2u
+int iss_set_head_switches(iss_ctx* ctx, uint32_t flags);
 
 int iss_cnn_flops(iss_ctx* ctx, int net_id, double* flops_per_sample);
+
+int iss_cnn_head_plan(const int32_t* prog, int32_t nrows, int32_t nbuf, const int64_t* buf_elems, int32_t in_h, int32_t in_w,
+                      int32_t in_c, int32_t out_dim, int prec, uint32_t diag, int32_t windows, int32_t* row_out);
 
 int iss_vbx_tables(iss_ctx* ctx, const double* window400, const double* melbank_257x64);
 int iss_vbx_features(iss_ctx* ctx, const int32_t* sig_i32, const double* dither_u, int64_t n,
```

Measured after the change: 7.233 (median of 2 runs). About the same (-0.1%).
